# youmi-zym/TemporalStereo

Hardware: AMD Instinct MI355X
Metric: stereo pairs/sec, FlyingThings3D 540x960 D=192 (aggregation hot path) (higher is better)
Workload: dtype f32

## Files before the change

include/ts_hip.h:

```cpp
#ifndef TS_HIP_H
#define TS_HIP_H

#include <stddef.h>
#include <stdint.h>

#ifdef __cplusplus
extern "C" {
#endif

#define TS_OK 0
#define TS_ERR_NULL (-1)
#define TS_ERR_SHAPE (-2)
#define TS_ERR_UNSUPPORTED (-3)
#define TS_ERR_ALIGN (-4)

int ts_version(void);
const char* ts_last_error_string(void);

size_t ts_block_cost_workspace_bytes(int B, int C, int H, int W, int D, int scales);

int ts_block_cost_int_fwd(const float* left, const float* right, float* out, void* workspace,
                          int B, int C, int H, int W, int D, int scales, void* stream);

int ts_block_cost_sampled_fwd(const float* left, const float* right, const float* disp, float* out,
                              void* workspace, int B, int C, int H, int W, int D, int scales,
                              void* stream);

int ts_block_cost_sampled_warped_fwd(const float* left, const float* right, const float* disp, float* out,
                                     void* workspace, int B, int C, int H, int W, int D, int scales,
                                     void* stream);

int ts_block_cost_sampled_corr_fwd(const float* left, const float* right, const float* disp, float* out,
                                   void* workspace, int B, int C, int H, int W, int D, int scales,
                                   void* stream);

int ts_block_cost_corr_split_supported(int C, int Csplit);
int ts_block_cost_sampled_corr_split_fwd(const float* left, const float* left2, const float* right, const float* right2,
                                         const float* disp, float* out, void* workspace, int B, int C, int Csplit, int H, int W,
                                         int D, int scales, long long left_bstride, long long left2_bstride,
                                         long long right_bstride, long long right2_bstride, void* stream);
int ts_conv3d_hw_split_supported(int B, int Cin, int Csplit, int Cout, int D, int H, int W, int stride, int dilation,
                                 int transposed);
int ts_conv3d_hw_split_fwd(const float* x, const float* x2, const float* w_t, const float* scale, const float* shift, float* y,
                           int B, int Cin, int Csplit, int Cout, int D, int H, int W, int stride, int dilation,
                           int transposed, int act, float act_param,
                           long long in_bstride, long long in_cstride, long long in2_bstride, long long in2_cstride,
                           long long out_bstride, long long out_cstride, const float* addend, long long addend_bstride,
                           void* workspace, size_t workspace_bytes, void* stream);
int ts_conv3d_d_split_supported(int Cin, int Csplit);
int ts_conv3d_d_split_fwd(const float* x, const float* x2, const float* w_t, const float* scale, const float* shift, float* y,
                          int B, int Cin, int Csplit, int Cout, int Din, int H, int W, int k, int stride, int dilation,
                          int padding, int transposed, int act, float act_param,
                          long long in_bstride, long long in_cstride, long long in2_bstride, long long in2_cstride,
                          long long out_bstride, long long out_cstride, void* stream);
int ts_conv3d_hw_x6_split_supported(int Cin, int Csplit, int Cout, int W, int dilation);
int ts_conv3d_hw_x6_split_fwd(const float* x, const float* x2, const void* w6, const float* scale, const float* shift, float* y,
                              int B, int Cin, int Csplit, int Cout, int D, int H, int W, int dilation, int act, float act_param,
                              long long in_bstride, long long in_cstride, long long in2_bstride, long long in2_cstride,
                              long long out_bstride, long long out_cstride, const float* addend, long long addend_bstride,
                              void* workspace, size_t workspace_bytes, void* stream);

int ts_cat_fms_fwd(const float* left, const float* right, const float* disp, float* out, int B, int C, int H, int W, int D,
                   void* stream);
int ts_inverse_warp_3d_fwd(const float* img, const float* disp, float* out, int B, int C, int H, int W, int D, void* stream);
size_t ts_dif_fms_workspace_bytes(void);
int ts_dif_fms_fwd(const float* left, const float* right, const float* disp, float* out, void* workspace, int B, int C,
                   int H, int W, int D, void* stream);

int ts_correlation_fwd(const float* left, const float* right, float* out, int B, int C, int H, int W, int patch_h, int patch_w,
                       int keep, void* stream);
int ts_correlation_bwd(const float* left, const float* right, const float* out, const float* grad_out, float* grad_left,
                       float* grad_right, int B, int C, int H, int W, int patch_h, int patch_w, int keep, void* stream);

size_t ts_block_cost_bwd_workspace_bytes(int B, int C, int H, int W, int D, int scales);

int ts_block_cost_int_bwd(const float* left, const float* right, const float* grad_out,
                          float* grad_left, float* grad_right, void* workspace,
                          int B, int C, int H, int W, int D, int scales, void* stream);

int ts_block_cost_sampled_bwd(const float* left, const float* right, const float* disp,
                              const float* grad_out, float* grad_left, float* grad_right,
                              float* grad_disp, void* workspace,
                              int B, int C, int H, int W, int D, int scales, void* stream);
int ts_block_cost_sampled_warped_bwd(const float* left, const float* right, const float* disp,
                                     const float* grad_out, float* grad_left, float* grad_right,
                                     float* grad_disp, void* workspace,
                                     int B, int C, int H, int W, int D, int scales, void* stream);

size_t ts_bn_workspace_bytes(int B, int C, long long N);
int ts_bn_sync_merge(const float* gathered, int world, int C, float* mean, float* var, float* running_mean,
                     float* running_var, float momentum, float* inv_count, void* stream);
long long ts_bn_set_small_elems(long long n);
int ts_channel_sum_fwd(const float* x, float* out, void* workspace, int B, int C, long long N, long long bstride, long long cstride,
                       void* stream);
int ts_bn_train_fwd(const float* x, float* mean, float* var, float* running_mean, float* running_var, float momentum,
                    long long* num_batches_tracked, const float* gamma, const float* beta, float* out, void* workspace,
                    int B, int C, long long N, long long x_bstride, long long x_cstride, long long out_bstride,
                    long long out_cstride, float eps, int act, void* stream);
int ts_bn_train_bwd(const float* x, const float* dy, const float* mean, const float* var, const float* gamma, const float* beta,
                    float* sum_dz, float* sum_dz_xhat, float* dx, void* workspace, int B, int C, long long N,
                    long long x_bstride, long long x_cstride, long long dy_bstride, long long dy_cstride, float eps, int act,
                    float count, void* stream);
int ts_bn_stats_fwd(const float* x, float* mean, float* var, float* running_mean, float* running_var, float momentum,
                    long long* num_batches_tracked, void* workspace, int B, int C, long long N, long long bstride,
                    long long cstride, void* stream);
int ts_bn_apply_act_fwd(const float* x, const float* mean, const float* var, const float* gamma, const float* beta, float* out,
                        int B, int C, long long N, long long x_bstride, long long x_cstride, long long out_bstride,
                        long long out_cstride, float eps, int act, void* stream);
int ts_bn_act_bwd_reduce(const float* x, const float* dy, const float* mean, const float* var, const float* gamma,
                         const float* beta, float* sum_dz, float* sum_dz_xhat, void* workspace, int B, int C, long long N,
                         long long x_bstride, long long x_cstride, long long dy_bstride, long long dy_cstride, float eps, int act,
                         void* stream);
int ts_bn_act_bwd_apply(const float* x, const float* dy, const float* mean, const float* var, const float* gamma,
                        const float* beta, const float* sum_dz, const float* sum_dz_xhat, float* dx, int B, int C, long long N,
                        long long x_bstride, long long x_cstride, long long dy_bstride, long long dy_cstride, float eps, int act,
                        int train, float count, void* stream);

size_t ts_wasserstein_loss_workspace_bytes(int B, int H, int W);
int ts_wasserstein_loss_fwd(const float* cost, const float* offset, const float* sample, const float* gt, float* loss,
                            float* gt_scaled, void* workspace, int B, int D, int H, int W, int Hg, int Wg, float max_disp,
                            float start_disp, int sparse, void* stream);
int ts_wasserstein_loss_bwd(const float* cost, const float* offset, const float* sample, const float* gt_scaled,
                            const float* grad_loss, float* grad_cost, float* grad_offset, int B, int D, int H, int W, int Wg,
                            float max_disp, float start_disp, void* stream);
size_t ts_disp_smooth_l1_workspace_bytes(int B, int Hg, int Wg);
int ts_disp_smooth_l1_fwd(const float* est, const float* gt, float* loss_count, void* workspace, int B, int h, int w, int Hg,
                          int Wg, float max_disp, float start_disp, void* stream);
int ts_disp_smooth_l1_bwd(const float* est, const float* gt, const float* grad_loss, const float* loss_count, float* grad_est,
                          int B, int h, int w, int Hg, int Wg, float max_disp, float start_disp, void* stream);

size_t ts_disp_metrics_workspace_bytes(int B, int Hg, int Wg);
int ts_disp_metrics_fwd(const float* est0, const float* est1, const float* est2, const float* est3, int n_est, int h0, int w0,
                        int h1, int w1, int h2, int w2, int h3, int w3, const float* gt, const float* gt_right, int B, int Hg,
                        int Wg, float lb, float ub, int flags, float* out, void* workspace, void* stream);

#define TS_RENDER_EST_COLOR 1
#define TS_RENDER_GT_COLOR 2
#define TS_RENDER_ERR_CLASS 4
#define TS_RENDER_ERR_JET 8
#define TS_RENDER_U16 16
#define TS_RENDER_UINT8 32
#define TS_RENDER_CHW 64
#define TS_RENDER_BAR 128
#define TS_RENDER_CLIP 256
#define TS_RENDER_MAX_SHARED 512
#define TS_RENDER_MAX_GIVEN 1024
#define TS_RENDER_STATS_FLOATS 32
size_t ts_disp_render_workspace_bytes(int B, int Hg, int Wg);
int ts_disp_render_fwd(const float* est, const float* gt, const float* max_disp, const float* jet, int B, int h, int w, int Hg,
                       int Wg, int flags, float scale16, void* disp_color, void* err_class, void* err_jet, void* disp_u16,
                       float* stats, void* workspace, void* stream);

#define TS_FLOW_SPARSE 1
#define TS_FLOW_EST_HWC 2
#define TS_FLOW_GT_HWC 4
#define TS_FLOW_RENDER_EST_COLOR 1
#define TS_FLOW_RENDER_GT_COLOR 2
#define TS_FLOW_RENDER_ERR_CLASS 4
#define TS_FLOW_RENDER_STATS 8
#define TS_FLOW_RENDER_UINT8 16
#define TS_FLOW_RENDER_CHW 32
#define TS_FLOW_RENDER_MAX_SHARED 64
#define TS_FLOW_RENDER_MAX_GIVEN 128
#define TS_FLOW_RENDER_EST_HWC 256
#define TS_FLOW_RENDER_GT_HWC 512
#define TS_FLOW_STATS_FLOATS 16
#define TS_FLOW_U16_CHW 1
size_t ts_flow_metrics_workspace_bytes(int B, int Hg, int Wg);
int ts_flow_metrics_fwd(const float* est0, const float* est1, const float* est2, const float* est3, int n_est, int h0, int w0,
                        int h1, int w1, int h2, int w2, int h3, int w3, const float* gt, int B, int Hg, int Wg, float lb, float ub,
                        int flags, float* out, void* workspace, void* stream);
size_t ts_flow_render_workspace_bytes(int B, int Hg, int Wg);
int ts_flow_render_fwd(const float* est, const float* gt, const float* gt_val, const float* max_rad, const float* wheel, int B,
                       int h, int w, int Hg, int Wg, int flags, void* flow_color, void* err_class, float* stats, void* workspace,
                       void* stream);
int ts_flow_u16_decode_fwd(const void* raw, int B, int H, int W, int flags, float* flow, void* valid, void* stream);

#define TS_PREPARE_CHW 1
int ts_frames_prepare_fwd(const void* left, const void* right, int B, int Hs, int Ws, int flags, float mean0, float mean1,
                          float mean2, float std0, float std1, float std2, int H, int W, const int* crop, float* color_l,
                          float* color_r, long long color_stride, float* color_aug_l, float* color_aug_r,
                          long long color_aug_stride, void* stream);
int ts_intrinsics_pyramid_fwd(const void* K_norm, int is_fp64, int B, int kh, int kw, int S, float* K, float* inv_K, void* stream);
int ts_disp_u16_decode_fwd(const void* raw, int B, int H, int W, float scale, float* disp, void* valid, void* stream);

#define TS_AUGMENT_ROW_INTS 96
#define TS_AUGMENT_MAX_RECTS 4
#define TS_AUGMENT_GAMMA 1
size_t ts_frames_augment_workspace_bytes(int B, int Hs, int Ws);
int ts_frames_augment_fwd(const void* left, const void* right, int B, int Hs, int Ws, int flags, float mean0, float mean1,
                          float mean2, float std0, float std1, float std2, int H, int W, const int* table, float* color_l,
                          float* color_r, long long color_stride, float* color_aug_l, float* color_aug_r,
                          long long color_aug_stride, void* workspace, size_t workspace_bytes, void* stream);
int ts_disp_u16_window_fwd(const void* raw, int B, int Hs, int Ws, int H, int W, const int* table, float scale, float* disp,
                           void* valid, void* stream);

int ts_topk_softargmax_fwd(const float* cost, const float* sample, const float* offset, float* disp,
                           float* topk_disp, float* topk_cost, int* topk_index,
                           int B, int D, int H, int W, int k, void* stream);

int ts_topk_softargmax_bwd(const float* topk_disp, const float* topk_cost, const int* topk_index,
                           const float* disp, const float* grad_disp, const float* grad_topk_disp,
                           const float* grad_topk_cost, float* grad_cost, float* grad_sample,
                           int B, int D, int H, int W, int k, void* stream);

int ts_softargmin_fwd(const float* cost, const float* sample, float* disp, float temperature,
                      int normalize, int B, int D, int H, int W, void* stream);
// ... 255 lines not shown
```

temporalstereo_amd/_lib.py:

```python
import ctypes
import os
import threading

_HERE = os.path.dirname(os.path.abspath(__file__))
LIB_PATH = os.path.join(_HERE, "libts_hip.so")

_lock = threading.Lock()
_lib = None

c_f32p = ctypes.c_void_p
c_ptr = ctypes.c_void_p
c_int = ctypes.c_int
c_size = ctypes.c_size_t
c_float = ctypes.c_float

SIGNATURES = {
    "ts_version": (c_int, []),
    "ts_last_error_string": (ctypes.c_char_p, []),
    "ts_block_cost_workspace_bytes": (c_size, [c_int] * 6),
    "ts_block_cost_int_fwd": (c_int, [c_f32p, c_f32p, c_f32p, c_ptr] + [c_int] * 6 + [c_ptr]),
    "ts_block_cost_sampled_fwd": (c_int, [c_f32p, c_f32p, c_f32p, c_f32p, c_ptr] + [c_int] * 6 + [c_ptr]),
    "ts_block_cost_sampled_warped_fwd": (c_int, [c_f32p, c_f32p, c_f32p, c_f32p, c_ptr] + [c_int] * 6 + [c_ptr]),
    "ts_block_cost_sampled_corr_fwd": (c_int, [c_f32p, c_f32p, c_f32p, c_f32p, c_ptr] + [c_int] * 6 + [c_ptr]),
    "ts_block_cost_corr_split_supported": (c_int, [c_int] * 2),
    "ts_block_cost_sampled_corr_split_fwd": (c_int, [c_f32p] * 6 + [c_ptr] + [c_int] * 7 + [ctypes.c_longlong] * 4 + [c_ptr]),
    "ts_conv3d_hw_split_supported": (c_int, [c_int] * 10),
    "ts_conv3d_hw_split_fwd": (c_int, [c_f32p] * 6 + [c_int] * 11 + [c_float] + [ctypes.c_longlong] * 6 +
                               [c_f32p, ctypes.c_longlong, c_ptr, c_size, c_ptr]),
    "ts_conv3d_d_split_supported": (c_int, [c_int] * 2),
    "ts_conv3d_d_split_fwd": (c_int, [c_f32p] * 6 + [c_int] * 13 + [c_float] + [ctypes.c_longlong] * 6 + [c_ptr]),
    "ts_conv3d_hw_x6_split_supported": (c_int, [c_int] * 5),
    "ts_conv3d_hw_x6_split_fwd": (c_int, [c_f32p, c_f32p, c_ptr, c_f32p, c_f32p, c_f32p] + [c_int] * 9 + [c_float] + [ctypes.c_longlong] * 6 +
                                  [c_f32p, ctypes.c_longlong, c_ptr, c_size, c_ptr]),
    "ts_conv3d_hw_warp_workspace_bytes": (c_size, [c_int] * 5),
    "ts_conv3d_hw_warp_fwd": (c_int, [c_f32p] * 8 + [c_int] * 8 + [c_float] + [ctypes.c_longlong] * 5 + [c_ptr, c_size, c_ptr]),
    "ts_cat_fms_fwd": (c_int, [c_f32p] * 4 + [c_int] * 5 + [c_ptr]),
    "ts_inverse_warp_3d_fwd": (c_int, [c_f32p] * 3 + [c_int] * 5 + [c_ptr]),
    "ts_dif_fms_workspace_bytes": (c_size, []),
    "ts_dif_fms_fwd": (c_int, [c_f32p] * 4 + [c_ptr] + [c_int] * 5 + [c_ptr]),
    "ts_correlation_fwd": (c_int, [c_f32p] * 3 + [c_int] * 7 + [c_ptr]),
    "ts_correlation_bwd": (c_int, [c_f32p] * 6 + [c_int] * 7 + [c_ptr]),
    "ts_block_cost_bwd_workspace_bytes": (c_size, [c_int] * 6),
    "ts_block_cost_int_bwd": (c_int, [c_f32p] * 5 + [c_ptr] + [c_int] * 6 + [c_ptr]),
    "ts_block_cost_sampled_bwd": (c_int, [c_f32p] * 7 + [c_ptr] + [c_int] * 6 + [c_ptr]),
    "ts_block_cost_sampled_warped_bwd": (c_int, [c_f32p] * 7 + [c_ptr] + [c_int] * 6 + [c_ptr]),
    "ts_calib_stream": (c_int, [c_int, c_ptr, c_ptr, c_size, c_ptr]),
    "ts_candidates_in_range_fwd": (c_int, [c_f32p] * 3 + [c_int] * 5 + [c_ptr]),
    "ts_candidates_in_range_bwd": (c_int, [c_f32p] * 5 + [c_int] * 5 + [c_ptr]),
    "ts_offset_head_fwd": (c_int, [c_f32p] * 2 + [ctypes.c_longlong, c_float, c_ptr]),
    "ts_offset_head_bwd": (c_int, [c_f32p] * 3 + [ctypes.c_longlong, c_float, c_ptr]),
    "ts_space_to_depth2_fwd": (c_int, [c_f32p] * 2 + [c_int] * 4 + [c_ptr]),
    "ts_deconv2d_k4s2_weight_to_conv3": (c_int, [c_f32p] * 2 + [c_int] * 3 + [c_ptr]),
    "ts_deconv2d_k4s2_wgrad_from_conv3": (c_int, [c_f32p] * 2 + [c_int] * 2 + [c_ptr]),
    "ts_bn_fold_many": (c_int, [c_ptr, c_int, c_float, c_ptr]),
    "ts_clip_rmsprop_workspace_bytes": (c_size, [c_int]),
    "ts_clip_rmsprop_step": (c_int, [c_ptr, c_int] + [c_float] * 4 + [c_ptr, c_size, c_ptr]),
    "ts_topk_softargmax_fwd": (c_int, [c_f32p] * 7 + [c_int] * 5 + [c_ptr]),
    "ts_topk_softargmax_bwd": (c_int, [c_f32p] * 9 + [c_int] * 5 + [c_ptr]),
    "ts_softargmin_fwd": (c_int, [c_f32p] * 3 + [c_float, c_int] + [c_int] * 4 + [c_ptr]),
    "ts_softargmin_bwd": (c_int, [c_f32p] * 6 + [c_float, c_int] + [c_int] * 4 + [c_ptr]),
    "ts_argmax_select_fwd": (c_int, [c_f32p] * 4 + [c_int] * 4 + [c_ptr]),
    "ts_bn_workspace_bytes": (c_size, [c_int, c_int, ctypes.c_longlong]),
    "ts_channel_splice_fwd": (c_int, [c_f32p] * 3 + [c_int] * 3 + [ctypes.c_longlong] * 4 + [c_ptr]),
    "ts_bn_sync_merge": (c_int, [c_f32p, c_int, c_int] + [c_f32p] * 4 + [c_float, c_f32p, c_ptr]),
    "ts_bn_train_fwd": (c_int, [c_f32p] * 5 + [c_float, c_ptr] + [c_f32p] * 3 + [c_ptr, c_int, c_int] + [ctypes.c_longlong] * 5 +
                        [c_float, c_int, c_ptr]),
    "ts_bn_train_bwd": (c_int, [c_f32p] * 9 + [c_ptr, c_int, c_int] + [ctypes.c_longlong] * 5 + [c_float, c_int, c_float, c_ptr]),
    "ts_bn_stats_fwd": (c_int, [c_f32p] * 5 + [c_float, c_ptr, c_ptr, c_int, c_int] + [ctypes.c_longlong] * 3 + [c_ptr]),
    "ts_bn_apply_act_fwd": (c_int, [c_f32p] * 6 + [c_int, c_int] + [ctypes.c_longlong] * 5 + [c_float, c_int, c_ptr]),
    "ts_bn_act_bwd_reduce": (c_int, [c_f32p] * 8 + [c_ptr, c_int, c_int] + [ctypes.c_longlong] * 5 + [c_float, c_int, c_ptr]),
    "ts_bn_act_bwd_apply": (c_int, [c_f32p] * 9 + [c_int, c_int] + [ctypes.c_longlong] * 5 + [c_float, c_int, c_int, c_float, c_ptr]),
    "ts_wasserstein_loss_workspace_bytes": (c_size, [c_int] * 3),
    "ts_wasserstein_loss_fwd": (c_int, [c_f32p] * 6 + [c_ptr] + [c_int] * 6 + [c_float, c_float, c_int, c_ptr]),
    "ts_wasserstein_loss_bwd": (c_int, [c_f32p] * 7 + [c_int] * 5 + [c_float, c_float, c_ptr]),
    "ts_disp_smooth_l1_workspace_bytes": (c_size, [c_int] * 3),
    "ts_disp_smooth_l1_fwd": (c_int, [c_f32p] * 3 + [c_ptr] + [c_int] * 5 + [c_float, c_float, c_ptr]),
    "ts_disp_smooth_l1_bwd": (c_int, [c_f32p] * 5 + [c_int] * 5 + [c_float, c_float, c_ptr]),
    "ts_disp_metrics_workspace_bytes": (c_size, [c_int] * 3),
    "ts_disp_metrics_fwd": (c_int, [c_f32p] * 4 + [c_int] * 9 + [c_f32p] * 2 + [c_int] * 3 + [c_float, c_float, c_int, c_f32p, c_ptr, c_ptr]),
    "ts_disp_render_workspace_bytes": (c_size, [c_int] * 3),
    "ts_disp_render_fwd": (c_int, [c_f32p] * 4 + [c_int] * 6 + [c_float] + [c_ptr] * 4 + [c_f32p, c_ptr, c_ptr]),
    "ts_flow_metrics_workspace_bytes": (c_size, [c_int] * 3),
    "ts_flow_metrics_fwd": (c_int, [c_f32p] * 4 + [c_int] * 9 + [c_f32p] + [c_int] * 3 + [c_float, c_float, c_int, c_f32p, c_ptr, c_ptr]),
    "ts_flow_render_workspace_bytes": (c_size, [c_int] * 3),
    "ts_flow_render_fwd": (c_int, [c_f32p] * 5 + [c_int] * 6 + [c_ptr] * 2 + [c_f32p, c_ptr, c_ptr]),
    "ts_flow_u16_decode_fwd": (c_int, [c_ptr] + [c_int] * 4 + [c_f32p, c_ptr, c_ptr]),
    "ts_frames_prepare_fwd": (c_int, [c_ptr] * 2 + [c_int] * 4 + [c_float] * 6 + [c_int] * 2 + [c_ptr] + [c_f32p] * 2 +
                              [ctypes.c_longlong] + [c_f32p] * 2 + [ctypes.c_longlong, c_ptr]),
    "ts_intrinsics_pyramid_fwd": (c_int, [c_ptr] + [c_int] * 5 + [c_f32p] * 2 + [c_ptr]),
    "ts_disp_u16_decode_fwd": (c_int, [c_ptr] + [c_int] * 3 + [c_float, c_f32p, c_ptr, c_ptr]),
    "ts_frames_augment_workspace_bytes": (c_size, [c_int] * 3),
    "ts_frames_augment_fwd": (c_int, [c_ptr] * 2 + [c_int] * 4 + [c_float] * 6 + [c_int] * 2 + [c_ptr] + [c_f32p] * 2 +
                              [ctypes.c_longlong] + [c_f32p] * 2 + [ctypes.c_longlong, c_ptr, c_size, c_ptr]),
    "ts_disp_u16_window_fwd": (c_int, [c_ptr] + [c_int] * 5 + [c_ptr, c_float, c_f32p, c_ptr, c_ptr]),
    "ts_softsplat_sum_fwd": (c_int, [c_f32p] * 3 + [c_int] * 4 + [c_ptr]),
    "ts_softsplat_sum_fwd_deterministic": (c_int, [c_f32p] * 3 + [c_ptr] + [c_int] * 4 + [c_ptr]),
    "ts_softsplat_sum_bwd_input": (c_int, [c_f32p] * 3 + [c_int] * 4 + [c_ptr]),
    "ts_softsplat_sum_bwd_flow": (c_int, [c_f32p] * 4 + [c_int] * 4 + [c_ptr]),
    "ts_softsplat_softmax_workspace_bytes": (c_size, [c_int] * 4),
    "ts_softsplat_softmax_fwd": (c_int, [c_f32p] * 4 + [c_ptr] + [c_int] * 4 + [c_ptr]),
    "ts_conv_cout_pad": (c_int, [c_int]),
    "ts_peer_region_bytes": (c_size, []),
    "ts_peer_max_floats": (c_int, []),
    "ts_peer_max_ranks": (c_int, []),
    "ts_peer_alloc": (c_int, [ctypes.POINTER(c_ptr), c_ptr]),
    "ts_peer_open": (c_int, [c_ptr, ctypes.POINTER(c_ptr)]),
    "ts_peer_close": (c_int, [c_ptr]),
    "ts_peer_free": (c_int, [c_ptr]),
    "ts_peer_status": (c_int, [c_ptr, ctypes.POINTER(c_int), c_ptr]),
    "ts_bn_set_small_elems": (ctypes.c_longlong, [ctypes.c_longlong]),
    "ts_channel_sum_fwd": (c_int, [c_f32p, c_f32p, c_ptr, c_int, c_int, ctypes.c_longlong, ctypes.c_longlong, ctypes.c_longlong, c_ptr]),
    "ts_peer_status_async": (c_int, [c_ptr, c_ptr, c_ptr]),
    "ts_peer_set_timeout_ms": (ctypes.c_longlong, [ctypes.c_longlong]),
    "ts_peer_reset": (c_int, [c_ptr, c_ptr]),
    "ts_peer_all_gather": (c_int, [c_ptr, c_f32p, c_f32p, c_int, c_ptr]),
    "ts_peer_all_reduce_sum": (c_int, [c_ptr, c_f32p, c_int, c_f32p, c_ptr]),
    "ts_conv_weight_layout": (c_int, [c_f32p, c_f32p] + [c_int] * 4 + [ctypes.c_longlong] * 3 + [c_int, c_ptr]),
    "ts_conv_weight_layout_many": (c_int, [c_ptr, c_int, c_int, c_ptr]),
    "ts_conv_weight_layout_many2": (c_int, [c_ptr, c_int, c_int, c_ptr]),
    "ts_conv_wgrad_defer": (c_int, [c_int]),
    "ts_conv_wgrad_pending": (c_int, []),
    "ts_conv_wgrad_take": (c_int, [c_ptr, c_size, ctypes.POINTER(c_int), ctypes.POINTER(c_int)]),
    "ts_conv_wgrad_finish_many": (c_int, [c_ptr, c_int, c_int, c_ptr]),
    "ts_conv_set_chunk_cap": (c_int, [c_int]),
    "ts_conv3d_hw_x6_supported": (c_int, [c_int] * 6),
    "ts_conv3d_hw_x6_weight_bytes": (ctypes.c_size_t, [c_int] * 2),
    "ts_conv3d_hw_x6_weight_split": (c_int, [c_f32p, c_ptr, c_int, c_int, c_ptr]),
    "ts_conv3d_hw_x6_weight_split_from": (c_int, [c_f32p, c_ptr, c_int, c_int] + [ctypes.c_longlong] * 3 + [c_int, c_ptr]),
    "ts_conv3d_hw_x6_workspace_bytes": (c_size, [c_int] * 6),
    "ts_conv3d_hw_x6s_supported": (c_int, [c_int] * 5),
    "ts_conv3d_hw_x6s_weight_bytes": (c_size, [c_int] * 3),
    "ts_conv3d_hw_x6s_weight_split": (c_int, [c_f32p, c_ptr, c_int, c_int, c_int, c_int, c_ptr]),
    "ts_conv3d_hw_x6s_fwd": (c_int, [c_f32p, c_ptr, c_f32p, c_f32p, c_f32p] + [c_int] * 8 + [c_float] + [ctypes.c_longlong] * 4 + [c_ptr]),
    "ts_conv3d_hw_x6_fwd": (c_int, [c_f32p, c_ptr, c_f32p, c_f32p, c_f32p] + [c_int] * 8 + [c_float] + [ctypes.c_longlong] * 4 +
                            [c_f32p, ctypes.c_longlong, c_ptr, c_size, c_ptr]),
    "ts_conv3d_hw_fwd": (c_int, [c_f32p] * 5 + [c_int] * 10 + [c_float] + [ctypes.c_longlong] * 4 +
                         [c_f32p, ctypes.c_longlong, c_ptr, c_size, c_ptr]),
    "ts_conv3d_hw_workspace_bytes": (c_size, [c_int] * 8),
    "ts_conv3d_hw_bwd_data": (c_int, [c_f32p] * 3 + [c_int] * 9 + [ctypes.c_longlong] * 4 + [c_ptr]),
    "ts_conv3d_bwd_weight_workspace_bytes": (ctypes.c_size_t, [c_int] * 3),
    "ts_conv3d_hw_bwd_weight": (c_int, [c_f32p] * 3 + [c_int] * 8 + [ctypes.c_longlong] * 4 + [c_ptr, ctypes.c_size_t, c_ptr]),
    "ts_conv3d_d_bwd_data": (c_int, [c_f32p] * 3 + [c_int] * 11 + [ctypes.c_longlong] * 4 + [c_ptr]),
    "ts_conv3d_d_bwd_weight": (c_int, [c_f32p] * 3 + [c_int] * 10 + [ctypes.c_longlong] * 4 + [c_ptr, ctypes.c_size_t, c_ptr]),
    "ts_conv3d_d_fwd": (c_int, [c_f32p] * 5 + [c_int] * 12 + [c_float] + [ctypes.c_longlong] * 4 + [c_ptr]),
    "ts_resize3d_add_act_fwd": (c_int, [c_f32p] * 3 + [c_int] * 9 + [ctypes.c_longlong] * 6 + [c_ptr]),
    "ts_pool3d5_avgmax_fwd": (c_int, [c_f32p] * 3 + [c_int] * 5 + [ctypes.c_longlong] * 6 + [c_ptr]),
    "ts_merge_candidates_fwd": (c_int, [c_f32p] * 9 + [c_int] * 6 + [ctypes.c_longlong] * 4 + [c_ptr]),
    "ts_convex_upsample_fwd": (c_int, [c_f32p] * 3 + [c_int] * 4 + [c_float, c_ptr]),
    "ts_convex_upsample_candidates_fwd": (c_int, [c_f32p] * 6 + [c_int] * 4 + [c_float, c_float, c_int, c_int, c_ptr]),
    "ts_unet_upsample_fwd": (c_int, [c_f32p] * 3 + [c_int] * 5 + [c_ptr]),
    "ts_convex_upsample_bwd": (c_int, [c_f32p] * 5 + [c_int] * 4 + [c_float, c_ptr]),
    "ts_unet_upsample_bwd": (c_int, [c_f32p] * 5 + [c_ptr] + [c_int] * 5 + [c_ptr]),
    "ts_deconv2d_k4s2_fwd": (c_int, [c_f32p] * 5 + [c_int] * 6 + [ctypes.c_longlong, c_ptr]),
    "ts_resize_bilinear_fwd": (c_int, [c_f32p] * 2 + [c_int] * 6 + [c_float, ctypes.c_longlong, c_ptr]),
    "ts_resize_bilinear_pair_fwd": (c_int, [c_f32p] * 4 + [c_int] * 6 + [c_float, c_float, c_ptr]),
    "ts_range_candidates_fwd": (c_int, [c_f32p] * 4 + [c_int] * 3 + [c_float, c_int, c_int, c_ptr]),
    "ts_project_to_3d_fwd": (c_int, [c_f32p] * 7 + [c_int] * 6 + [c_float, c_ptr]),
    "ts_inverse_warp_fwd": (c_int, [c_f32p] * 9 + [c_ptr, c_f32p] + [c_int] * 11 + [c_float, c_ptr]),
    "ts_inverse_warp_bwd": (c_int, [c_f32p] * 8 + [c_int] * 11 + [c_float, c_ptr]),
    "ts_raft_corr_pyramid_fwd": (c_int, [c_f32p] * 3 + [c_int] * 5 + [c_ptr]),
    "ts_raft_corr_lookup_fwd": (c_int, [c_f32p] * 3 + [c_int] * 5 + [c_ptr]),
    "ts_raft_corr_lookup_bwd": (c_int, [c_f32p] * 5 + [c_int] * 6 + [c_ptr]),
    "ts_raft_corr_pyramid_bwd": (c_int, [c_f32p] * 5 + [c_int] * 5 + [c_ptr]),
    "ts_flow_corr_pyramid_fwd": (c_int, [c_f32p] * 3 + [c_int] * 5 + [c_ptr]),
    "ts_flow_corr_lookup_fwd": (c_int, [c_f32p] * 3 + [c_int] * 5 + [c_ptr]),
    "ts_flow_corr_lookup_bwd": (c_int, [c_f32p] * 5 + [c_int] * 6 + [c_ptr]),
    "ts_flow_corr_pyramid_bwd": (c_int, [c_f32p] * 5 + [c_int] * 5 + [c_ptr]),
    "ts_spp3d_pool_fwd": (c_int, [c_f32p] * 2 + [c_int] * 10 + [ctypes.c_longlong] * 2 + [c_ptr]),
    "ts_spp3d_pool_bwd": (c_int, [c_f32p] * 6 +[c_int] * 10 + [ctypes.c_longlong] * 4 + [c_ptr]),
    "ts_spp3d_expand_fwd": (c_int, [c_f32p] * 6 + [c_int] * 11 + [ctypes.c_longlong] * 2 + [c_ptr]),
    "ts_spp3d_expand_bwd": (c_int, [c_f32p] * 5 + [c_int] * 11 + [ctypes.c_longlong] * 2 + [c_ptr]),
    "ts_depth_sum3_fwd": (c_int, [c_f32p] * 6 + [c_int] * 6 + [ctypes.c_longlong] * 8 + [c_ptr]),
    "ts_bn_small_train_bwd": (c_int, [c_f32p] * 7 + [c_int] * 3 + [ctypes.c_longlong] * 6 + [c_float, c_int, c_ptr]),
    "ts_reproject_memory_workspace_bytes": (c_size, [c_int] * 5),
    "ts_reproject_memory_fwd": (c_int, [c_f32p, ctypes.c_longlong, c_int, c_int, c_f32p, c_f32p, c_int, c_f32p, c_int, c_int,
                                        c_f32p, c_int, c_f32p, c_f32p, c_f32p, c_float, c_float, c_f32p, c_f32p, c_f32p,
                                        c_ptr, c_int, c_int, c_int, c_ptr]),
    "ts_resize3d_add_act_bwd": (c_int, [c_f32p] * 5 + [c_int] * 9 + [c_ptr]),
    "ts_pool3d5_avgmax_bwd": (c_int, [c_f32p] * 4 + [c_int] * 5 + [c_ptr]),
    "ts_merge_candidates_bwd": (c_int, [c_f32p] * 5 + [c_int] * 5 + [c_ptr]),
    "ts_copy_rows_fwd": (c_int, [c_f32p] * 2 + [ctypes.c_longlong] * 4 + [c_ptr]),
    "ts_plan_create": (c_ptr, []),
    "ts_plan_destroy": (None, [c_ptr]),
    "ts_plan_length": (c_int, [c_ptr]),
    "ts_plan_add_call": (c_int, [c_ptr, ctypes.c_char_p, ctypes.POINTER(ctypes.c_ulonglong), c_int]),
    "ts_plan_run": (c_int, [c_ptr]),
    "ts_stream_fork": (c_int, [c_ptr, c_ptr]),
    "ts_event_record": (c_int, [c_int, c_ptr]),
    "ts_event_wait": (c_int, [c_int, c_ptr]),
}

_QUERIES = frozenset(n for n in SIGNATURES if n.endswith("_bytes") or n.startswith("ts_plan_") or
                     n.endswith("_split_supported") or
                     n in ("ts_version", "ts_last_error_string", "ts_conv_cout_pad", "ts_conv3d_hw_x6_supported", "ts_conv3d_hw_x6s_supported", "ts_peer_max_floats", "ts_peer_max_ranks",
                           "ts_peer_alloc", "ts_peer_open", "ts_peer_close", "ts_peer_free", "ts_peer_status", "ts_peer_status_async",
                           "ts_peer_set_timeout_ms", "ts_peer_reset", "ts_bn_set_small_elems",
                           "ts_conv_wgrad_defer", "ts_conv_wgrad_pending", "ts_conv_wgrad_take"))


def lib():
    rec = getattr(_tls, "recorder", None)
    if rec is not None:
        return rec.proxy
    return _real_lib()


def _real_lib():
    global _lib
    if _lib is None:
        with _lock:
            if _lib is None:
                if not os.path.exists(LIB_PATH):
                    raise RuntimeError(
                        "temporalstereo_amd: %s is missing -- build it with "
                        "`python -m temporalstereo_amd.build` (there is no fallback path)" % LIB_PATH)
                handle = ctypes.CDLL(LIB_PATH)
                for name, (res, args) in SIGNATURES.items():
                    fn = getattr(handle, name, None)
                    if fn is None:
                        raise RuntimeError("libts_hip.so does not export %s (stale build?)" % name)
                    fn.restype = res
                    fn.argtypes = args
                _lib = handle
    return _lib


_tls = threading.local()


def _word(argtype, value):
    if isinstance(value, ctypes._SimpleCData):
        value = value.value
    if argtype is c_float:
        import struct
        return struct.unpack("<I", struct.pack("<f", float(value)))[0]
    if value is None:
        return 0
    return int(value) & 0xFFFFFFFFFFFFFFFF


class _RecordingProxy:
    def __init__(self, recorder):
        self._rec = recorder

    def __getattr__(self, name):
        real = getattr(_real_lib(), name)
        if name in _QUERIES:
            return real
        argtypes = SIGNATURES[name][1]
        rec = self._rec

        def call(*args):
            rc = real(*args)
            if rc == 0:
                words = (ctypes.c_ulonglong * len(args))(*[_word(t, a) for t, a in zip(argtypes, args)])
                rec.log.append((name, int(words[len(args) - 1]) if len(args) else 0))
                rc2 = _real_lib().ts_plan_add_call(rec.plan, name.encode(), words, len(args))
                if rc2 != 0:
                    check(rc2, "ts_plan_add_call(%s)" % name)
            return rc
        return call


class Recorder:

    def __init__(self):
        self.plan = _real_lib().ts_plan_create()
        if not self.plan:
            raise RuntimeError("ts_plan_create failed")
        self.keep = []
        self.log = []
        self.proxy = _RecordingProxy(self)

    def __enter__(self):
        if getattr(_tls, "recorder", None) is not None:
            raise RuntimeError("plan recording does not nest")
        _tls.recorder = self
        return self

    def __exit__(self, *exc):
        _tls.recorder = None
        return False

    def __len__(self):
        return int(_real_lib().ts_plan_length(self.plan))

    def run(self):
        rc = _real_lib().ts_plan_run(self.plan)
        if rc != 0:
            check(rc, "ts_plan_run")

    def __del__(self):
        try:
            if self.plan:
                _real_lib().ts_plan_destroy(self.plan)
                self.plan = None
        except Exception:
            pass


def recording():
    return getattr(_tls, "recorder", None) is not None


def check(rc, what):
    if rc != 0:
        msg = _real_lib().ts_last_error_string().decode("utf-8", "replace")
        kind = "argument error" if rc < 0 else "hipError_t"
        raise RuntimeError("%s failed (%s %d): %s" % (what, kind, rc, msg))


def ptr(t):
    if t is None:
        return None
    rec = getattr(_tls, "recorder", None)
    if rec is not None:
        rec.keep.append(t)
    return t.data_ptr()


def current_stream_handle():
    import torch
    return torch._C._cuda_getCurrentRawStream(torch.cuda.current_device())


def contiguous(t):
    if t.is_contiguous():
        return t
    if recording():
        raise RuntimeError("plan recording needs contiguous tensors (a .contiguous() copy would not be replayed)")
    return t.contiguous()
```

temporalstereo_amd/aggregation/native.py:

```python
import os
import time

import torch
import torch.nn as nn

from .. import _lib
from .. import functional as TF

ACT_NONE, ACT_SILU, ACT_RELU, ACT_TANH_OFFSET, ACT_HEAD_PAIR = 0, 1, 2, 3, 4


def _stream():
    return _lib.current_stream_handle()


_PAR = {"on": False, "aux": None, "kinds": frozenset(__import__("os").environ.get("TS_BRANCHES", "hourglass").split(","))}


def _aux_stream():
    return _PAR["aux"]


_STAGE_CAP = int(os.environ.get("TS_STAGE_CHUNK_CAP", "8"))


def _chunk_cap(cap):
    if cap == 8:
        cap = _STAGE_CAP
    _lib.check(_lib.lib().ts_conv_set_chunk_cap(int(cap)), "ts_conv_set_chunk_cap")


_QUALIFIED = {}
_ROUND_TRIP_SLACK = 1.6


def _round_trip_us(main, s, n=20):
    L = _lib._real_lib()
    buf = torch.zeros(2, 256, device=s.device)
    pm, ps = _lib.ctypes.c_void_p(main.cuda_stream), _lib.ctypes.c_void_p(s.cuda_stream)
    a, b = _lib.ctypes.c_void_p(buf[0].data_ptr()), _lib.ctypes.c_void_p(buf[1].data_ptr())

    def lap(k):
        for _ in range(k):
            for st, other in ((pm, ps), (ps, pm)):
                _lib.check(L.ts_copy_rows_fwd(a, b, 1, 256, 256, 256, st), "ts_copy_rows_fwd")
                _lib.check(L.ts_stream_fork(st, other), "ts_stream_fork")
    lap(5)
    best = None
    for _ in range(3):
        torch.cuda.synchronize(s.device)
        t0 = time.perf_counter()
        lap(n)
        torch.cuda.synchronize(s.device)
        us = (time.perf_counter() - t0) / n * 1e6
        best = us if best is None else min(best, us)
    return best


def qualified_streams(dev, count, private=False):
    with torch.cuda.device(dev):
        pool = _QUALIFIED.setdefault(torch.cuda.current_device(), {"shared": [], "floor": None})
        main = torch.cuda.current_stream()
        if pool["floor"] is None:
            pool["floor"] = _round_trip_us(main, torch.cuda.Stream(device=dev))

        def draw():
            best = None
            for _ in range(8):
                s = torch.cuda.Stream(device=dev, priority=-1)
                us = _round_trip_us(main, s)
                if us <= _ROUND_TRIP_SLACK * pool["floor"]:
                    return s
                if best is None or us < best[0]:
                    best = (us, s)
            return best[1]
        if private:
            return [draw() for _ in range(count)]
        while len(pool["shared"]) < count:
            pool["shared"].append(draw())
        return pool["shared"][:count]


def _edge(src, dst):
    rc = _lib.lib().ts_stream_fork(_lib.ctypes.c_void_p(src.cuda_stream), _lib.ctypes.c_void_p(dst.cuda_stream))
    _lib.check(rc, "ts_stream_fork")


class Branch:

    def __init__(self, kind):
        self.on = _PAR["on"] and kind in _PAR["kinds"]
        if self.on:
            self.cur, self.aux = torch.cuda.current_stream(), _aux_stream()

    def __enter__(self):
        if self.on:
            _edge(self.cur, self.aux)
            self.ctx = torch.cuda.stream(self.aux)
            self.ctx.__enter__()
        return self

    def __exit__(self, *exc):
        if self.on:
            self.ctx.__exit__(*exc)
        return False

    def join(self):
        if self.on:
            _edge(self.aux, self.cur)


def _act_code(mod):
    if mod is None:
        return ACT_NONE
    if isinstance(mod, nn.SiLU):
        return ACT_SILU
    if isinstance(mod, nn.ReLU):
        return ACT_RELU
    raise NotImplementedError("activation %r has no fused kernel epilogue" % (mod,))


class Tape:

    def __init__(self):
        self.layouts = []
        self.folds = []
        self.splits = []
        self.eps = None
        self.unsupported = []
        self._tables = None

    def __enter__(self):
        global _TAPE
        self._outer, _TAPE = _TAPE, self
        return self

    def __exit__(self, *exc):
        global _TAPE
        _TAPE = self._outer
        return False

    def layout(self, out, weight, transposed, rows=None, col0=0, out_st=None, src_cin0=0, cout_sel=None):
        w = weight
        d0, d1 = w.shape[0], w.shape[1]
        T = w[0, 0].numel()
        cout, cin = (d1, d0) if transposed else (d0, d1)
        s_ci, s_co = ((d1 * T, T) if transposed else (T, d1 * T))
        c0, nci = rows if rows is not None else (0, cin)
        o0, nco = cout_sel if cout_sel is not None else (0, cout)
        self.layouts.append(dict(out=out, w=w, A=nci, T=T, nb=nco, col0=col0, sa=s_ci, sb=s_co, st=1, src_off=(c0 + src_cin0) * s_ci + o0 * s_co,
                                 out_sa=out.stride(0), out_st=out.stride(1) if out_st is None else out_st))
        self._tables = None

    def fold(self, scale, shift, bias, bn, cout):
        if bn is not None:
            if self.eps is not None and float(bn.eps) != self.eps:
                self.unsupported.append("BatchNorm layers with different eps")
            self.eps = float(bn.eps)
        self.folds.append(dict(scale=scale, shift=shift, bias=bias, bn=bn, C=cout))
        self._tables = None

    def _upload(self, dev):
        import numpy as np
        lay = np.zeros(len(self.layouts), dtype=np.dtype([("w", "<u8"), ("out", "<u8"), ("A", "<i4"), ("T", "<i4"), ("nb", "<i4"), ("col0", "<i4"),
                                                          ("sa", "<i8"), ("sb", "<i8"), ("st", "<i8"), ("osa", "<i8"), ("ost", "<i8"),
                                                          ("flip", "<i4"), ("reserved", "<i4")]))
        most = 1
        for i, e in enumerate(self.layouts):
            w = e["w"]
            if not w.is_contiguous():
                raise RuntimeError("Tape: a source weight is not contiguous")
            lay[i] = (w.data_ptr() + 4 * e["src_off"], e["out"].data_ptr(), e["A"], e["T"], e["nb"], e["col0"], e["sa"], e["sb"], e["st"],
                      e["out_sa"], e["out_st"], 0, 0)
            most = max(most, e["A"] * e["T"] * e["nb"])
        fo = np.zeros(len(self.folds), dtype=np.dtype([("gamma", "<u8"), ("beta", "<u8"), ("mean", "<u8"), ("var", "<u8"), ("bias", "<u8"),
                                                       ("scale", "<u8"), ("shift", "<u8"), ("C", "<i4"), ("pad", "<i4")]))
        P = lambda t: t.data_ptr() if t is not None else 0
        for i, e in enumerate(self.folds):
            bn = e["bn"]
            if bn is not None:
                g, b = (bn.weight, bn.bias) if bn.affine else (None, None)
                fo[i] = (P(g), P(b), P(bn.running_mean), P(bn.running_var), P(e["bias"]), P(e["scale"]), P(e["shift"]), e["C"], e["C"])
            else:
                fo[i] = (0, 0, 0, 0, P(e["bias"]), P(e["scale"]), P(e["shift"]), e["C"], e["C"])
        up = lambda a: torch.from_numpy(a.view(np.uint8).reshape(-1).copy()).to(dev)
        self._tables = (up(lay), up(fo), min(64, (most + 255) // 256))

    def refresh(self, dev):
        if self.unsupported:
            raise RuntimeError("Tape.refresh: %s -- rebuild the aggregator instead" % "; ".join(self.unsupported))
        L = _lib.lib()
        if self._tables is None:
            self._upload(dev)
        lay, fo, blocks = self._tables
        if self.layouts:
            _lib.check(L.ts_conv_weight_layout_many2(_lib.ptr(lay), len(self.layouts), blocks, _stream()), "ts_conv_weight_layout_many2")
        if self.folds:
            _lib.check(L.ts_bn_fold_many(_lib.ptr(fo), len(self.folds), self.eps if self.eps is not None else 1e-5, _stream()), "ts_bn_fold_many")
        for f, kind, mode in self.splits:
            if kind == "x6":
                _lib.check(L.ts_conv3d_hw_x6_weight_split(f.w.data_ptr(), f.w6.data_ptr(), f.cin, f.cout, _stream()), "ts_conv3d_hw_x6_weight_split")
            else:
                _lib.check(L.ts_conv3d_hw_x6s_weight_split(f.w.data_ptr(), f.w6s.data_ptr(), f.cin, f.cout, f.w.shape[2], mode, _stream()),
                           "ts_conv3d_hw_x6s_weight_split")


_TAPE = None


class Folded:

    def __init__(self, weight, bias, bn, act, transposed, kind):
        self._tape = _TAPE
        self.src = (weight, bias, bn, transposed)
        w = weight.detach().float()
        if transposed:
            w = w.transpose(0, 1)
        cout, cin = w.shape[0], w.shape[1]
        taps = w.shape[2:].numel()
        self.cin, self.cout, self.kind, self.act = cin, cout, kind, act
        self.kshape = tuple(w.shape[2:])
        pad = int(_lib.lib().ts_conv_cout_pad(cout))
        if pad < cout:
            raise NotImplementedError("Cout=%d has no kernel bucket" % cout)
        wt = torch.zeros(cin, taps, pad, device=w.device, dtype=torch.float32)
        wt[:, :, :cout] = w.reshape(cout, cin, taps).permute(1, 2, 0)
        self.w = wt.contiguous()
        scale = torch.ones(pad, device=w.device)
        shift = torch.zeros(pad, device=w.device)
        b = bias.detach().float() if bias is not None else torch.zeros(cout, device=w.device)
        if bn is not None:
            if not isinstance(bn, nn.modules.batchnorm._BatchNorm) or bn.running_mean is None:
                raise NotImplementedError("only BatchNorm with running statistics can be folded, got %r" % (bn,))
            gamma = bn.weight.detach().float() if bn.affine else torch.ones(cout, device=w.device)
            beta = bn.bias.detach().float() if bn.affine else torch.zeros(cout, device=w.device)
            s = gamma / torch.sqrt(bn.running_var.detach().float() + bn.eps)
            scale[:cout] = s
            shift[:cout] = beta + (b - bn.running_mean.detach().float()) * s
        else:
            shift[:cout] = b
        self.scale, self.shift = scale.contiguous(), shift.contiguous()
        if _TAPE is not None:
            if weight.dtype != torch.float32:
                _TAPE.unsupported.append("non-fp32 weights")
            _TAPE.layout(self.w, weight.detach(), transposed)
            _TAPE.fold(self.scale, self.shift, bias, bn, cout)


def fold_split_input(f, n):
    head, rest = object.__new__(Folded), object.__new__(Folded)
    for g, lo, hi in ((head, 0, n), (rest, n, f.cin)):
        g.cin, g.cout, g.kind, g.kshape = hi - lo, f.cout, f.kind, f.kshape
        g._tape = getattr(f, "_tape", None)
        g.w = f.w[lo:hi].contiguous()
        assert g.w.data_ptr() == f.w[lo:hi].data_ptr()
    head.act, rest.act = ACT_NONE, f.act
    head.scale, head.shift = torch.ones_like(f.scale), torch.zeros_like(f.shift)
    rest.scale, rest.shift = f.scale, f.shift
    return head, rest


def fold_concat(a, b):
    if (a.cin, a.kind, a.act, a.kshape) != (b.cin, b.kind, b.act, b.kshape):
        raise ValueError("fold_concat: layers differ in more than their output channels")
    f = object.__new__(Folded)
    f.cin, f.cout, f.kind, f.act, f.kshape = a.cin, a.cout + b.cout, a.kind, a.act, a.kshape
    pad = int(_lib.lib().ts_conv_cout_pad(f.cout))
    if pad < f.cout:
        raise NotImplementedError("Cout=%d has no kernel bucket" % f.cout)
    taps = a.w.shape[1]
    f.w = torch.zeros(a.cin, taps, pad, device=a.w.device, dtype=torch.float32)
    f.w[:, :, :a.cout] = a.w[:, :, :a.cout]
    f.w[:, :, a.cout:f.cout] = b.w[:, :, :b.cout]
    f.scale = torch.ones(pad, device=a.w.device)
    f.shift = torch.zeros(pad, device=a.w.device)
    f.scale[:a.cout] = a.scale[:a.cout]; f.scale[a.cout:f.cout] = b.scale[:b.cout]
    f.shift[:a.cout] = a.shift[:a.cout]; f.shift[a.cout:f.cout] = b.shift[:b.cout]
    f._tape = getattr(a, "_tape", None)
    if f._tape is not None:
        col = 0
        for g in (a, b):
            src = getattr(g, "src", None)
            if src is None:
                f._tape.unsupported.append("concatenation of derived layers")
                break
            weight, bias, bn, transposed = src
            f._tape.layout(f.w, weight.detach(), transposed, col0=col)
            f._tape.fold(f.scale[col:col + g.cout], f.shift[col:col + g.cout], bias, bn, g.cout)
            col += g.cout
    return f


def fold_wrapper(m, kind, transposed=False):
    return Folded(m.weight, m.bias, getattr(m, "norm", None), _act_code(getattr(m, "activation", None)), transposed, kind)


def _strides5(t):
    if t.stride(4) != 1 or t.stride(3) != t.shape[4] or t.stride(2) != t.shape[3] * t.shape[4]:
        raise ValueError("tensor planes must be dense (channel-sliced views of contiguous buffers are fine)")
    return t.stride(0), t.stride(1)


Split = TF.Split


X6 = os.environ.get("TS_CONV_X6", "1") != "0"
_X6_MIN_GRID = int(os.environ.get("TS_CONV_X6_MIN_GRID", "128"))
_X6_MIN_GRID_UNSPLIT = int(os.environ.get("TS_CONV_X6_MIN_GRID_UNSPLIT", "64"))


def x6_weights(f):
    w6 = getattr(f, "w6", None)
    if w6 is None:
        L = _lib._real_lib()
        w6 = torch.empty(int(L.ts_conv3d_hw_x6_weight_bytes(f.cin, f.cout)), device=f.w.device, dtype=torch.uint8)
        _lib.check(L.ts_conv3d_hw_x6_weight_split(f.w.data_ptr(), w6.data_ptr(), f.cin, f.cout, _stream()), "ts_conv3d_hw_x6_weight_split")
        f.w6 = w6
        if getattr(f, "_tape", None) is not None:
            f._tape.splits.append((f, "x6", 0))
    return w6


X6S = os.environ.get("TS_CONV_X6S", "1") != "0"
_X6S_MIN_GRID = int(os.environ.get("TS_CONV_X6S_MIN_GRID", "256"))
_X6S_MIN_GRID_T3 = int(os.environ.get("TS_CONV_X6S_MIN_GRID_T3", "400"))
X6S_S2, X6S_T3, X6S_T4 = 0, 1, 2


def x6s_weights(f, mode):
    w6 = getattr(f, "w6s", None)
    if w6 is None:
        L = _lib._real_lib()
        w6 = torch.empty(int(L.ts_conv3d_hw_x6s_weight_bytes(f.cin, f.cout, mode)), device=f.w.device, dtype=torch.uint8)
        _lib.check(L.ts_conv3d_hw_x6s_weight_split(f.w.data_ptr(), w6.data_ptr(), f.cin, f.cout, f.w.shape[2], mode, _stream()),
                   "ts_conv3d_hw_x6s_weight_split")
        f.w6s = w6
        f.w6s_mode = mode
        if getattr(f, "_tape", None) is not None:
            f._tape.splits.append((f, "x6s", mode))
    elif getattr(f, "w6s_mode", mode) != mode:
        raise RuntimeError("x6s_weights: this layer's weights were split for mode %d, asked for mode %d" % (f.w6s_mode, mode))
    return w6


def x6s_grid(B, cout, D, H, W, mode):
    if mode == X6S_S2:
        return ((((H - 1) // 2 + 1) + 3) // 4) * ((((W - 1) // 2 + 1) + 31) // 32) * D * B * ((cout + 31) // 32)
    return ((H + 7) // 8) * ((W + 31) // 32) * D * B * ((cout + 15) // 16)


def conv_hw(x, f, stride=1, dilation=1, transposed=False, out=None, act=None, act_param=0.0, addend=None, second=None,
            out_second=None):
    split = None
    if isinstance(x, Split):
        if second is not None or transposed or stride != 1:
            raise ValueError("conv_hw(Split): stride-1, not transposed, no `second`")
        x, split = x.a, x.b
# ... 71 lines not shown
    return out


def conv_d(x, f, k, stride=1, dilation=1, padding=0, transposed=False, out=None, act=None, act_param=0.0):
    split = None
    if isinstance(x, Split):
        x, split = x.a, x.b
    B, Cin, Din, H, W = x.shape
    if split is not None:
        Cs, Cin = Cin, Cin + split.shape[1]
        i2b, i2c = _strides5(split)
    assert Cin == f.cin, (Cin, f.cin)
    Dout = 2 * Din if transposed else (Din + 2 * padding - dilation * (k - 1) - 1) // stride + 1
    if out is None:
        out = torch.empty((B, f.cout, Dout, H, W), device=x.device, dtype=torch.float32)
    ib, ic = _strides5(x)
    ob, oc = _strides5(out)
    if split is not None:
        rc = _lib.lib().ts_conv3d_d_split_fwd(_lib.ptr(x), _lib.ptr(split), _lib.ptr(f.w), _lib.ptr(f.scale), _lib.ptr(f.shift),
                                              _lib.ptr(out), B, Cin, Cs, f.cout, Din, H, W, k, stride, dilation, padding,
                                              int(transposed), f.act if act is None else act, float(act_param),
                                              ib, ic, i2b, i2c, ob, oc, _stream())
        _lib.check(rc, "ts_conv3d_d_split_fwd")
        return out
    rc = _lib.lib().ts_conv3d_d_fwd(_lib.ptr(x), _lib.ptr(f.w), _lib.ptr(f.scale), _lib.ptr(f.shift), _lib.ptr(out),
                                    B, Cin, f.cout, Din, H, W, k, stride, dilation, padding, int(transposed),
                                    f.act if act is None else act, float(act_param), ib, ic, ob, oc, _stream())
    _lib.check(rc, "ts_conv3d_d_fwd")
    return out


FUSED_K1 = os.environ.get("TS_FUSED_K1", "1") != "0"
SPLIT_INPUT = os.environ.get("TS_SPLIT_INPUT", "1") != "0"


def block_cost_corr(left, right, disp, scales):
    return TF.block_cost_corr(left, right, disp, scales)


def conv_hw_warp(corr, f, q, disp, base, dilation=1):
    B, Cc, D, H, W = corr.shape
    assert Cc == f.cin, (Cc, f.cin)
    out = torch.empty((B, f.cout, D, H, W), device=corr.device, dtype=torch.float32)
    ib, ic = _strides5(corr)
    ob, oc = _strides5(out)
    wsb = TF._q("ts_conv3d_hw_warp_workspace_bytes", B, f.cout, D, H, W)
    ws = torch.empty(wsb, device=corr.device, dtype=torch.uint8)
    rc = _lib.lib().ts_conv3d_hw_warp_fwd(_lib.ptr(corr), _lib.ptr(f.w), _lib.ptr(f.scale), _lib.ptr(f.shift), _lib.ptr(out),
                                          _lib.ptr(q), _lib.ptr(disp), _lib.ptr(base), B, Cc, f.cout, D, H, W, dilation, f.act, 0.0,
                                          ib, ic, ob, oc, base.stride(0) if base is not None else 0, _lib.ptr(ws), wsb, _stream())
    _lib.check(rc, "ts_conv3d_hw_warp_fwd")
    return out


def resize_add_act(a, add, size, act=ACT_SILU):
    B, C, Da, Ha, Wa = a.shape
    D, H, W = size
    out = torch.empty((B, C, D, H, W), device=a.device, dtype=torch.float32)
    ab, ac = _strides5(a)
    bb, bc = _strides5(add) if add is not None else (0, 0)
    ob, oc = _strides5(out)
    rc = _lib.lib().ts_resize3d_add_act_fwd(_lib.ptr(a), _lib.ptr(add), _lib.ptr(out), B, C, Da, Ha, Wa, D, H, W, act,
                                            ab, ac, bb, bc, ob, oc, _stream())
    _lib.check(rc, "ts_resize3d_add_act_fwd")
    return out


def pool5(x, out_avg, out_max):
    B, C, D, H, W = x.shape
    xb, xc = _strides5(x); ab, ac = _strides5(out_avg); mb, mc = _strides5(out_max)
    rc = _lib.lib().ts_pool3d5_avgmax_fwd(_lib.ptr(x), _lib.ptr(out_avg), _lib.ptr(out_max), B, C, D, H, W,
                                          xb, xc, ab, ac, mb, mc, _stream())
    _lib.check(rc, "ts_pool3d5_avgmax_fwd")


def resize_bilinear(x, size, value_scale=1.0, out=None):
    B, C, h, w = x.shape
    if out is None:
        out = torch.empty((B, C, size[0], size[1]), device=x.device, dtype=torch.float32)
    x = _lib.contiguous(x)
    rc = _lib.lib().ts_resize_bilinear_fwd(_lib.ptr(x), _lib.ptr(out), B, C, h, w, size[0], size[1],
                                           float(value_scale), out.stride(0), _stream())
    _lib.check(rc, "ts_resize_bilinear_fwd")
    return out


def resize_bilinear_pair(x0, x1, size, scale0, scale1):
    B, C, h, w = x0.shape
    if x1.shape != x0.shape:
        raise RuntimeError("resize_bilinear_pair: shapes differ")
    o0 = torch.empty((B, C, size[0], size[1]), device=x0.device, dtype=torch.float32)
    o1 = torch.empty_like(o0)
    x0, x1 = _lib.contiguous(x0), _lib.contiguous(x1)
    rc = _lib.lib().ts_resize_bilinear_pair_fwd(_lib.ptr(x0), _lib.ptr(x1), _lib.ptr(o0), _lib.ptr(o1),
                                                B, C, h, w, size[0], size[1], float(scale0), float(scale1), _stream())
    _lib.check(rc, "ts_resize_bilinear_pair_fwd")
    return o0, o1


def copy_rows(src, dst):
    B = src.shape[0]
    n = src[0].numel()
    src = _lib.contiguous(src)
    rc = _lib.lib().ts_copy_rows_fwd(_lib.ptr(src), _lib.ptr(dst), B, n, n, dst.stride(0), _stream())
    _lib.check(rc, "ts_copy_rows_fwd")


def range_candidates(disp, rng, extra_front=0):
    B, _, H, W = disp.shape
    low = torch.empty_like(disp)
    high = torch.empty_like(disp)
    cand = torch.empty((B, extra_front + 5, H, W), device=disp.device, dtype=torch.float32)
    rc = _lib.lib().ts_range_candidates_fwd(_lib.ptr(disp), _lib.ptr(low), _lib.ptr(high), _lib.ptr(cand), B, H, W,
                                            float(rng), extra_front, extra_front + 5, _stream())
    _lib.check(rc, "ts_range_candidates_fwd")
    return low, high, cand


def split_sampled_first_layer(f0, scales):
    C = f0.cin * 8 // (16 + scales)
    if 2 * C + scales * (C // 8) != f0.cin or f0.kshape != (1, 3, 3):
        raise NotImplementedError("first aggregation layer is not a (1,3,3) conv over [left | warped | corr]")
    left, rest = fold_split_input(f0, C)
    _, corr = fold_split_input(rest, C)
    q = object.__new__(Folded)
    q.cin, q.cout, q.kind, q.act, q.kshape = C, 9 * rest.cout, "d", ACT_NONE, (1, 1, 1)
    pad = int(_lib.lib().ts_conv_cout_pad(q.cout))
    q.w = torch.zeros(C, 1, pad, device=rest.w.device, dtype=torch.float32)
    q.w[:, 0, :q.cout] = rest.w[:C, :, :rest.cout].reshape(C, 9 * rest.cout)
    q.scale, q.shift = torch.ones(pad, device=q.w.device), torch.zeros(pad, device=q.w.device)
    q._tape = getattr(f0, "_tape", None)
    if q._tape is not None:
        src = getattr(f0, "src", None)
        if src is None or src[3]:
            q._tape.unsupported.append("first layer of a sampled level is itself derived")
        else:
            q._tape.layout(q.w, src[0].detach(), False, rows=(C, C), out_st=rest.cout)
    return left, rest, corr, q


class SepConv:

    def __init__(self, mod, transposed=False):
        c0, c1 = mod.conv[0], mod.conv[1]
        self.transposed = transposed
        self.f0 = fold_wrapper(c0, "hw", transposed)
        self.f1 = fold_wrapper(c1, "d", transposed)
        self.k = c1.kernel_size[0]
        self.stride, self.dil = c0.stride[1], c0.dilation[1]
        self.pad_d = c1.padding[0]
        if c0.kernel_size != (1, 3, 3) or c0.padding[1] != self.dil or c1.stride[0] != self.stride:
            raise NotImplementedError("separable conv outside the (1,3,3)+(k,1,1) family: %r" % (mod,))

    def __call__(self, x, out=None, addend=None):
        y = conv_hw(x, self.f0, self.stride, self.dil, self.transposed, addend=addend)
        return conv_d(y, self.f1, self.k, self.stride, self.dil, self.pad_d, self.transposed, out=out)


class Hourglass:

    def __init__(self, mod):
        self.c1, self.c2, self.c3, self.c4 = (SepConv(getattr(mod, n)) for n in ("conv1", "conv2", "conv3", "conv4"))
        self.c5, self.c6 = SepConv(mod.conv5, True), SepConv(mod.conv6, True)
        self.s5, self.s6 = SepConv(mod.shortcut5), SepConv(mod.shortcut6)
        self.c4.f1.act = ACT_SILU

    def __call__(self, x):
        pre = self.c2(self.c1(x))
        br = Branch("hourglass")
        with br:
            s6 = self.s6(x)
            s5 = self.s5(pre)
        out = self.c5(self.c4(self.c3(pre)))
        br.join()
        out = resize_add_act(out, s5, pre.shape[-3:])
        return resize_add_act(self.c6(out), s6, x.shape[-3:])


class Heads:

    def __init__(self, mod):
        self.delta = float(mod.delta)
        c0, self.c1 = fold_wrapper(mod.cost_head[0], "d"), fold_wrapper(mod.cost_head[1], "hw")
        o0, self.o1 = fold_wrapper(mod.off_head[0], "d"), fold_wrapper(mod.off_head[1], "hw")
        self.C = C = c0.cout
        self.co0 = fold_concat(c0, o0)
        f = object.__new__(Folded)
        f.cin, f.cout, f.kind, f.act, f.kshape = 2 * C, 2, "hw", ACT_HEAD_PAIR, self.c1.kshape
        pad = int(_lib.lib().ts_conv_cout_pad(2))
        f.w = torch.zeros(2 * C, self.c1.w.shape[1], pad, device=self.c1.w.device, dtype=torch.float32)
        f.w[:C, :, 0] = self.c1.w[:, :, 0]
        f.w[C:, :, 1] = self.o1.w[:, :, 0]
        f.scale = torch.ones(pad, device=f.w.device); f.shift = torch.zeros(pad, device=f.w.device)
        f.scale[0], f.scale[1] = self.c1.scale[0], self.o1.scale[0]
        f.shift[0], f.shift[1] = self.c1.shift[0], self.o1.shift[0]
        f._tape = _TAPE
        if _TAPE is not None:
            for k, (m, g) in enumerate(((mod.cost_head[1], self.c1), (mod.off_head[1], self.o1))):
                _TAPE.layout(f.w[k * C:(k + 1) * C], m.weight.detach(), False, col0=k)
                _TAPE.fold(f.scale[k:k + 1], f.shift[k:k + 1], m.bias, getattr(m, "norm", None), 1)
        self.pair = f

    def __call__(self, x):
        y = conv_d(x, self.co0, 3, 1, 1, 1)
        B, _, D, H, W = y.shape
        both = torch.empty((2, B, D, H, W), device=y.device, dtype=torch.float32)
        conv_hw(y, self.pair, out=both.permute(1, 0, 2, 3, 4), act_param=self.delta)
        return both[0], both[1]


class ConvexUp:

    def __init__(self, mod):
        self.r, self.k = mod.upscale_factor, mod.window_size
        if self.k != 3:
            raise NotImplementedError("window_size != 3")
        self.m0 = Folded(mod.mask[0].weight.unsqueeze(2), mod.mask[0].bias, mod.mask[1], ACT_SILU, False, "hw")
        w3 = mod.mask[3].weight
        self.m3 = Folded(w3.reshape(w3.shape[0], w3.shape[1], 1, 1, 1), mod.mask[3].bias, None, ACT_NONE, False, "d")

    def mask(self, feat):
        return conv_d(conv_hw(feat.unsqueeze(2), self.m0), self.m3, 1)

    def with_candidates(self, feat, disp, m, rng, extra_front=0):
        B, _, H, W = disp.shape
        if m is None:
            m = self.mask(feat)
        Ho, Wo = H * self.r, W * self.r
        out = torch.empty((B, 1, Ho, Wo), device=disp.device, dtype=torch.float32)
        low, high = torch.empty_like(out), torch.empty_like(out)
        cand = torch.empty((B, extra_front + 5, Ho, Wo), device=disp.device, dtype=torch.float32)
        disp = _lib.contiguous(disp)
        rc = _lib.lib().ts_convex_upsample_candidates_fwd(_lib.ptr(m), _lib.ptr(disp), _lib.ptr(out), _lib.ptr(low),
                                                          _lib.ptr(high), _lib.ptr(cand), B, H, W, self.r, float(self.r), float(rng),
                                                          extra_front, extra_front + 5, _stream())
        _lib.check(rc, "ts_convex_upsample_candidates_fwd")
        return out, low, high, cand

    def __call__(self, feat, disp, m=None):
        B, _, H, W = disp.shape
        if m is None:
            m = self.mask(feat)
        out = torch.empty((B, 1, H * self.r, W * self.r), device=disp.device, dtype=torch.float32)
        disp = _lib.contiguous(disp)
        rc = _lib.lib().ts_convex_upsample_fwd(_lib.ptr(m), _lib.ptr(disp), _lib.ptr(out), B, H, W, self.r,
                                               float(self.r), _stream())
        _lib.check(rc, "ts_convex_upsample_fwd")
        return out


class _LevelBase:
    def __init__(self, mod):
        self.mod = mod
        self.C, self.topk, self.scales = mod.C, mod.topk, mod.block_cost_scale
        self.init0, self.hg, self.init2 = SepConv(mod.init3d[0]), Hourglass(mod.init3d[1]), SepConv(mod.init3d[2])
        self.heads = Heads(mod.pred_heads)

    def init3d(self, raw, addend=None):
        return self.init2(self.hg(self.init0(raw, addend=addend)))

    def split_reference_half(self):
        if self.init0.stride != 1 or self.init0.transposed:
            raise NotImplementedError("first aggregation layer is not a stride-1 conv over [left | warped | corr]")
        self.init0_left, self.init0.f0, self.init0_corr, self.init0_q = split_sampled_first_layer(self.init0.f0, self.scales)

    def left_term(self, left):
        return conv_hw(left.unsqueeze(2), self.init0_left, 1, self.init0.dil)

    def right_term(self, right):
        return conv_d(right.unsqueeze(2), self.init0_q, 1).squeeze(2)

    def first_layer_fused(self, left, right, ds, lterm, rterm):
        corr = block_cost_corr(left, right, ds, self.scales)
        i0 = self.init0
        y = conv_hw_warp(corr, self.init0_corr, rterm, ds, lterm.squeeze(2) if lterm.dim() == 5 else lterm, i0.dil)
        return conv_d(y, i0.f1, i0.k, i0.stride, i0.dil, i0.pad_d, i0.transposed)

    def init3d_from(self, first):
        return self.init2(self.hg(first))

    def feature_terms(self, left, right):
        return self.left_term(left), (self.right_term(right) if FUSED_K1 else None)


class _MergingLevel(_LevelBase):
    def __init__(self, mod):
        super().__init__(mod)
        pc = mod.past_conv
        f = fold_wrapper(pc, "d")
        self.past_w = f.w.reshape(-1)[:self.C].contiguous()
        self.past_scale, self.past_shift = f.scale[:self.C].contiguous(), f.shift[:self.C].contiguous()
        self.fusion = mod.spatial_fusion
        if self.fusion:
            self.conv5 = fold_wrapper(mod.fuse.conv_5x5, "d")
            self.fuse_conv = SepConv(mod.fuse.conv_fuse)
        self.up = ConvexUp(mod.convex_upsample)

    def merge(self, vol, samples, prev_info, resize_memory):
        B, C, D0, H, W = vol.shape
        K = self.topk
        memory = prev_info.get('cost_memory', None)
        mem_s = mem_c = None
        if memory is not None and prev_info.get('use_past_cost', False):
            mem_s, mem_c = memory['disp_sample'], memory['cost_volume']
            if resize_memory:
                mem_s, mem_c = resize_bilinear_pair(mem_s, mem_c, (H, W), W / mem_s.shape[-1], 1.0)
            mem_s, mem_c = _lib.contiguous(mem_s), _lib.contiguous(mem_c)
        Dm = D0 + K
        nch = 4 * C if self.fusion else C
        cat4 = torch.empty((B, nch, Dm, H, W), device=vol.device, dtype=torch.float32)
        samp = torch.empty((B, Dm, H, W), device=vol.device, dtype=torch.float32)
        x0 = cat4[:, :C]
        vb, vc = _strides5(vol); ob, oc = _strides5(x0)
        rc = _lib.lib().ts_merge_candidates_fwd(_lib.ptr(vol), _lib.ptr(samples), _lib.ptr(mem_s), _lib.ptr(mem_c),
                                                _lib.ptr(self.past_w), _lib.ptr(self.past_scale), _lib.ptr(self.past_shift),
                                                _lib.ptr(samp), _lib.ptr(x0), B, C, D0, K, H, W, vb, vc, ob, oc, _stream())
        _lib.check(rc, "ts_merge_candidates_fwd")
        return cat4, samp

    def fuse(self, cat4):
        C = self.C
        x0 = cat4[:, :C]
        if not self.fusion:
            return x0
        br = Branch("pool")
        with br:
            pool5(x0, cat4[:, 2 * C:3 * C], cat4[:, 3 * C:])
        conv_d(x0, self.conv5, 5, 1, 1, 2, out=cat4[:, C:2 * C])
        br.join()
# ... 393 lines not shown
```

temporalstereo_amd/csrc/conv3d.hip:

```cpp
#include <cstdlib>
#include <mutex>
#include <type_traits>
#include <vector>

#include "conv_common.hpp"
#include "conv_x6p.hpp"
#include "warp.hpp"

namespace {




template <int MODE, int KT, int ST, int DL, int TP = 256>
struct Geom {
  static constexpr int NTR = (MODE == MODE_D) ? KT : 1;
  static constexpr int TRW = (TP == 64) ? 4 : 8, TCW = (TP == 64) ? 16 : 32;
  static constexpr int in_rows = (MODE == MODE_HW) ? (TRW - 1) * ST + 2 * DL + 1 : ((MODE == MODE_HWT) ? ((KT == 16) ? TRW + 2 : TRW + 1) : 1);
  static constexpr int in_cols = (MODE == MODE_HW) ? (TCW - 1) * ST + 2 * DL + 1 : ((MODE == MODE_HWT) ? ((KT == 16) ? TCW + 2 : TCW + 1) : TP);
  static constexpr int pitch = (MODE == MODE_D) ? TP : (in_cols | 1);
  static constexpr int RQ_HW = (in_rows * in_cols + 255) / 256;
  static constexpr int chan_raw = (MODE == MODE_D) ? NTR * TP : in_rows * pitch;
  static constexpr int pad0 = (16 - (chan_raw & 31)) & 31;
  static constexpr int chan_elems = chan_raw + (pad0 ? pad0 : 32);
};


template <int CB, int MODE, int KT, int ST, int DL, int NC, int PR = 0, int PF = 0, int TP = 256>
__global__ void __launch_bounds__(256)
ig_conv_kernel(const float* __restrict__ x, const float* __restrict__ w, const float* __restrict__ scale,
               const float* __restrict__ shift, float* __restrict__ y, const IG p) {
  extern __shared__ __attribute__((aligned(16))) float lds[];
  static_assert(!PR || (MODE == MODE_HW && KT == 9 && ST == 1 && CB == 1 && NC >= 8), "row pairing: stride-1 (1,3,3), Cout <= 8");
  static_assert(TP == 256 || (TP == 64 && (MODE == MODE_D || MODE == MODE_HWT || (MODE == MODE_HW && !PR))), "64-pixel tiles: not the row-paired form");
  using G = Geom<MODE, KT, ST, DL, TP>;
  constexpr int WP = (CB * 16) | 16;
  constexpr int NTR = G::NTR, RQ = (MODE == MODE_D) ? NTR : G::RQ_HW;
  constexpr int in_rows = G::in_rows, in_cols = G::in_cols, pitch = G::pitch, chan_elems = G::chan_elems;
  constexpr int KTW = PR ? 12 : KT;
  constexpr int NPB = PR ? 2 : TP / 64;
  constexpr int WV = KTW * NC * CB * 4;
  constexpr int RWN = (WV + 255) / 256;

  const int wave = threadIdx.x >> 6, lane = threadIdx.x & 63;
  const int j = lane & 15, kq = lane >> 4;
  unsigned lin = blockIdx.x + gridDim.x * (blockIdx.y + gridDim.y * blockIdx.z);
  if (p.xcd) {
    const unsigned per = (gridDim.x * gridDim.y * gridDim.z) / 8;
    if (lin < per * 8) lin = (lin % 8) * per + lin / 8;
  }
  const int bx = lin % gridDim.x, by = (lin / gridDim.x) % gridDim.y, bz = lin / (gridDim.x * gridDim.y);
  const int cog = bz % p.co_groups;
  const int ks = (bz / p.co_groups) % p.ksplit, b = bz / (p.co_groups * p.ksplit);
  const int kbeg = ks * p.kspan, kend = min(p.Cin, kbeg + p.kspan);
  const int co0 = cog * CB * 16;
  const int od = by;

  int tile = bx, pa = 0, pbit = 0;
  if (MODE == MODE_HWT) { pa = (tile & 3) >> 1; pbit = tile & 1; tile >>= 2; }
  int iy0 = 0, ix0 = 0, ty0 = 0, tx0 = 0;
  if (MODE == MODE_HW) {
    ty0 = (tile / p.tiles_x) * G::TRW; tx0 = (tile % p.tiles_x) * G::TCW;
    iy0 = ty0 * ST - DL; ix0 = tx0 * ST - DL;
  } else if (MODE == MODE_HWT) {
    ty0 = (tile / p.tiles_x) * G::TRW; tx0 = (tile % p.tiles_x) * G::TCW;
    iy0 = ty0 - ((KT == 16) ? 1 : 0); ix0 = tx0 - ((KT == 16) ? 1 : 0);
  }
  float* in_tile = lds;
  float* w_tile = lds + NC * chan_elems;
  const unsigned HW = static_cast<unsigned>(p.H) * p.W;

  int plane_id[NTR], plane_wt[NTR], ntaps = KT;
  if (MODE == MODE_D) {
    if (p.transposed) {
      ntaps = 0;
      if ((od & 1) == 0) { plane_id[0] = od >> 1; plane_wt[0] = 1; ntaps = 1; }
      else {
        plane_id[0] = (od - 1) >> 1; plane_wt[0] = 2; ntaps = 1;
        if (NTR > 1 && ((od + 1) >> 1) < p.D) { plane_id[1] = (od + 1) >> 1; plane_wt[1] = 0; ntaps = 2; }
      }
#pragma unroll
      for (int t = 0; t < NTR; ++t) if (t >= ntaps) { plane_id[t] = -1; plane_wt[t] = 0; }
    } else {
#pragma unroll
      for (int t = 0; t < NTR; ++t) {
        const int id = od * p.stride + t * p.dil - p.pad;
        plane_id[t] = (id >= 0 && id < p.D) ? id : -1;
        plane_wt[t] = t;
      }
    }
  }
  const int px0 = (MODE == MODE_D) ? bx * TP : 0;

  unsigned goff[RQ];
  int loff[RQ];
  if (MODE == MODE_D) {
#pragma unroll
    for (int t = 0; t < NTR; ++t) {
      const unsigned px = px0 + 4u * (threadIdx.x & 63u);
      goff[t] = (plane_id[t] >= 0 && px < HW) ? (static_cast<unsigned>(plane_id[t]) * HW + px) * 4u : kOOB;
      loff[t] = t * 256 + 4 * static_cast<int>(threadIdx.x & 63u);
    }
  } else {
#pragma unroll
    for (int q = 0; q < RQ; ++q) {
      const int e = static_cast<int>(threadIdx.x) + 256 * q;
      const bool slot = e < in_rows * in_cols;
      const int cy = e / in_cols, cx = e - cy * in_cols;
      const int gy = iy0 + cy, gx = ix0 + cx;
      const bool live = slot && gy >= 0 && gy < p.H && gx >= 0 && gx < p.W;
      goff[q] = live ? (static_cast<unsigned>(od) * HW + static_cast<unsigned>(gy) * p.W + gx) * 4u : kOOB;
      loff[q] = slot ? cy * pitch + cx : G::chan_raw;
    }
  }
  constexpr int NI64 = (MODE == MODE_D && TP == 64) ? (NC * NTR + 15) / 16 : 1;
  unsigned go64[NI64];
  int lo64[NI64], ch64[NI64];
  if constexpr (MODE == MODE_D && TP == 64) {
#pragma unroll
    for (int i = 0; i < NI64; ++i) {
      const int r = static_cast<int>(threadIdx.x >> 4) + 16 * i;
      const bool ok = r < NC * NTR;
      const int c = r / NTR, t = r - c * NTR;
      int pid = -1;
#pragma unroll
      for (int u = 0; u < NTR; ++u) pid = (u == t) ? plane_id[u] : pid;
      const unsigned px = px0 + 4u * (threadIdx.x & 15u);
      go64[i] = (ok && pid >= 0 && px < HW) ? (static_cast<unsigned>(pid) * HW + px) * 4u : kOOB;
      ch64[i] = ok ? c : 0;
      lo64[i] = ok ? c * chan_elems + t * TP + 4 * static_cast<int>(threadIdx.x & 15u) : G::chan_raw;
    }
  }
  unsigned woff[RWN];
  int wci[RWN], wl[RWN];
#pragma unroll
  for (int q = 0; q < RWN; ++q) {
    const int v = threadIdx.x + 256 * q;
    const int co4 = v % (CB * 4), r = v / (CB * 4);
    const int ci = r % NC, tap = r / NC;
    if constexpr (PR) {
      const int rho = tap / 3, kx = tap % 3, ky = rho - ((co4 >> 1) ? 0 : 1);
      const bool ok = v < WV && ky >= 0 && ky <= 2;
      woff[q] = ok ? static_cast<unsigned>((ci * KT + ky * 3 + kx) * p.coutp + (co4 & 1) * 4) * 4u : kOOB;
    } else {
      const bool ok = v < WV && co0 + co4 * 4 < p.coutp;
      woff[q] = ok ? static_cast<unsigned>((ci * KT + tap) * p.coutp + co0 + co4 * 4) * 4u : kOOB;
    }
    wci[q] = ci;
    wl[q] = v < WV ? r * WP + co4 * 4 : KTW * NC * WP;
  }
  const __amdgpu_buffer_rsrc_t xr = ig_rsrc(x + static_cast<long long>(b) * p.in_bstride, p.in_bytes);
  const __amdgpu_buffer_rsrc_t xr2 = ig_rsrc(p.x2 + static_cast<long long>(b) * p.in2_bstride, p.in2_bytes);
  const __amdgpu_buffer_rsrc_t wr = ig_rsrc(w, p.w_bytes);
  const unsigned cstride_b = static_cast<unsigned>(p.in_cstride) * 4u, cstride2_b = static_cast<unsigned>(p.in2_cstride) * 4u;
  const unsigned wstride_b = static_cast<unsigned>(KT * p.coutp) * 4u;

  int boff[4];
#pragma unroll
  for (int pb = 0; pb < 4; ++pb) {
    if (MODE == MODE_D) boff[pb] = kq * chan_elems + wave * (TP / 4) + pb * 16 + j;
    else if (PR) {
      const int base = (DL == 1) ? wave * 2 : (wave & 1) + 4 * (wave >> 1);
      boff[pb] = kq * chan_elems + base * pitch + (pb & 1) * 16 + j;
    } else {
      const int row = (TP == 64) ? wave : wave * 2 + (pb >> 1), col = (TP == 64) ? j : (pb & 1) * 16 + j;
      constexpr int st = (MODE == MODE_HW) ? ST : 1;
      boff[pb] = kq * chan_elems + row * st * pitch + col * st;
    }
  }
  const int aoff = kq * WP + j;

  v4f acc[CB][4];
#pragma unroll
  for (int cb = 0; cb < CB; ++cb)
#pragma unroll
    for (int pb = 0; pb < 4; ++pb) acc[cb][pb] = v4f{0.f, 0.f, 0.f, 0.f};
  float esc[CB][4], esh[CB][4];
#pragma unroll
  for (int cb = 0; cb < CB; ++cb)
#pragma unroll
    for (int r = 0; r < 4; ++r) {
      const int co = min(PR ? (kq & 1) * 4 + r : co0 + cb * 16 + kq * 4 + r, p.coutp - 1);
      esc[cb][r] = scale ? scale[co] : 1.f;
      esh[cb][r] = shift ? shift[co] : 0.f;
    }

  constexpr int NSET = PF ? 2 : 1;
  constexpr bool VD = (MODE == MODE_D);
  constexpr int NCQ = VD ? NC / 4 : 1;
  float rin[NSET][VD ? 1 : NC][VD ? 1 : RQ];
  constexpr bool VD64 = VD && TP == 64;
  u32x4 rin4[NSET][VD64 ? 1 : NCQ][(VD && !VD64) ? NTR : 1];
  u32x4 rin64[NSET][NI64];
  u32x4 rw[NSET][RWN];
  const int wave_u = __builtin_amdgcn_readfirstlane(static_cast<int>(threadIdx.x >> 6));
  auto fetch = [&](auto set, int c0) {
    constexpr int S = decltype(set)::value;
    const ChunkBase cbs = chunk_base(c0, p.csplit, xr, xr2, cstride_b, cstride2_b);
    if constexpr (VD64) {
#pragma unroll
      for (int i = 0; i < NI64; ++i) {
        const unsigned chb = static_cast<unsigned>(min(c0 + ch64[i], p.Cin - 1) - cbs.c_first) * cbs.cstride_b;
        rin64[S][i] = __builtin_amdgcn_raw_buffer_load_b128(cbs.rsrc, go64[i] == kOOB ? kOOB : go64[i] + chb, 0, 0);
      }
    } else if constexpr (VD) {
#pragma unroll
      for (int ic = 0; ic < NCQ; ++ic) {
        const unsigned so = static_cast<unsigned>(min(c0 + wave_u + 4 * ic, p.Cin - 1) - cbs.c_first) * cbs.cstride_b;
#pragma unroll
        for (int t = 0; t < NTR; ++t) rin4[S][ic][t] = __builtin_amdgcn_raw_buffer_load_b128(cbs.rsrc, goff[t], so, 0);
      }
    } else {
#pragma unroll
    for (int c = 0; c < NC; ++c) {
      const unsigned so = static_cast<unsigned>(min(c0 + c, p.Cin - 1) - cbs.c_first) * cbs.cstride_b;
#pragma unroll
      for (int i = 0; i < RQ; ++i) rin[S][c][i] = __uint_as_float(__builtin_amdgcn_raw_buffer_load_b32(cbs.rsrc, goff[i], so, 0));
    }
    }
    const unsigned wso = static_cast<unsigned>(c0) * wstride_b;
#pragma unroll
    for (int q = 0; q < RWN; ++q)
      rw[S][q] = __builtin_amdgcn_raw_buffer_load_b128(wr, (wci[q] < kend - c0) ? woff[q] + wso : kOOB, 0, 0);
  };
  auto commit = [&](auto set) {
    constexpr int S = decltype(set)::value;
    if constexpr (VD64) {
#pragma unroll
      for (int i = 0; i < NI64; ++i) *reinterpret_cast<u32x4*>(in_tile + lo64[i]) = rin64[S][i];
    } else if constexpr (VD) {
#pragma unroll
      for (int ic = 0; ic < NCQ; ++ic)
#pragma unroll
        for (int t = 0; t < NTR; ++t)
          *reinterpret_cast<u32x4*>(in_tile + (wave_u + 4 * ic) * chan_elems + loff[t]) = rin4[S][ic][t];
    } else {
#pragma unroll
    for (int c = 0; c < NC; ++c)
#pragma unroll
      for (int i = 0; i < RQ; ++i) in_tile[c * chan_elems + loff[i]] = rin[S][c][i];
    }
#pragma unroll
    for (int q = 0; q < RWN; ++q) *reinterpret_cast<u32x4*>(w_tile + wl[q]) = rw[S][q];
  };
  auto mma = [&]() {
#pragma unroll 1
  for (int c8 = 0; c8 < (NC >= 8 ? NC / 8 : 1); ++c8) {
    const float* it = in_tile + c8 * 8 * chan_elems;
    const float* wt0 = w_tile + c8 * 8 * WP + aoff;
    if (MODE == MODE_HW) {
      constexpr int NS = (NC == 4) ? 9 : 2 * KTW;
      float a[2][CB], bv[2][4];
      auto frag = [&](int s, int slot) {
        const int tap = (NC == 4) ? s : (s >> 1), cq = (NC == 4) ? 0 : (s & 1);
        const int toff = (tap / 3) * DL * pitch + (tap % 3) * DL;
#pragma unroll
        for (int cb = 0; cb < CB; ++cb) a[slot][cb] = wt0[(tap * NC + cq * 4) * WP + cb * 16];
#pragma unroll
        for (int pb = 0; pb < NPB; ++pb) bv[slot][pb] = it[boff[pb] + cq * 4 * chan_elems + toff];
      };
      frag(0, 0);
#pragma unroll
      for (int s = 0; s < NS; ++s) {
        if (s + 1 < NS) frag(s + 1, (s + 1) & 1);
#pragma unroll
        for (int cb = 0; cb < CB; ++cb)
#pragma unroll
          for (int pb = 0; pb < NPB; ++pb)
            acc[cb][pb] = __builtin_amdgcn_mfma_f32_16x16x4f32(a[s & 1][cb], bv[s & 1][pb], acc[cb][pb], 0, 0, 0);
      }
    } else if (MODE == MODE_HWT) {
      constexpr int KS = (KT == 16) ? 4 : 3, ORG = (KT == 16) ? 1 : 0;
#pragma unroll
      for (int ta = 0; ta < 2; ++ta) {
        int ky, dy;
        if (pa) { ky = ta ? 0 : 2; dy = ta ? 1 : 0; }
        else { if (ta && KT != 16) continue; ky = ta ? 3 : 1; dy = ta ? -1 : 0; }
#pragma unroll
        for (int tb = 0; tb < 2; ++tb) {
          int kx, dx;
          if (pbit) { kx = tb ? 0 : 2; dx = tb ? 1 : 0; }
          else { if (tb && KT != 16) continue; kx = tb ? 3 : 1; dx = tb ? -1 : 0; }
          const int toff = (dy + ORG) * pitch + dx + ORG;
          const float* wt = wt0 + ((ky * KS + kx) * NC) * WP;
#pragma unroll
          for (int cq = 0; cq < 2; ++cq) {
            float a[CB], bv[4];
#pragma unroll
            for (int cb = 0; cb < CB; ++cb) a[cb] = wt[cq * 4 * WP + cb * 16];
#pragma unroll
            for (int pb = 0; pb < NPB; ++pb) bv[pb] = it[boff[pb] + cq * 4 * chan_elems + toff];
#pragma unroll
            for (int cb = 0; cb < CB; ++cb)
#pragma unroll
              for (int pb = 0; pb < NPB; ++pb)
                acc[cb][pb] = __builtin_amdgcn_mfma_f32_16x16x4f32(a[cb], bv[pb], acc[cb][pb], 0, 0, 0);
          }
        }
      }
    } else {
#pragma unroll
      for (int t = 0; t < NTR; ++t) {
        if (t >= ntaps) continue;
        const float* wt = wt0 + (plane_wt[t] * NC) * WP;
#pragma unroll
        for (int cq = 0; cq < 2; ++cq) {
          float a[CB], bv[4];
#pragma unroll
          for (int cb = 0; cb < CB; ++cb) a[cb] = wt[cq * 4 * WP + cb * 16];
#pragma unroll
          for (int pb = 0; pb < NPB; ++pb) bv[pb] = it[boff[pb] + cq * 4 * chan_elems + t * TP];
#pragma unroll
          for (int cb = 0; cb < CB; ++cb)
#pragma unroll
            for (int pb = 0; pb < NPB; ++pb)
              acc[cb][pb] = __builtin_amdgcn_mfma_f32_16x16x4f32(a[cb], bv[pb], acc[cb][pb], 0, 0, 0);
        }
      }
    }
  }
  };
  using S0 = std::integral_constant<int, 0>;
  using S1 = std::integral_constant<int, NSET - 1>;
  fetch(S0{}, kbeg);
  if constexpr (NSET == 2) {
    if (kbeg + NC < kend) fetch(S1{}, kbeg + NC);
    for (int c0 = kbeg; c0 < kend; c0 += 2 * NC) {
      __syncthreads();
      commit(S0{});
      __syncthreads();
      if (c0 + 2 * NC < kend) fetch(S0{}, c0 + 2 * NC);
      mma();
      if (c0 + NC < kend) {
        __syncthreads();
        commit(S1{});
        __syncthreads();
        if (c0 + 3 * NC < kend) fetch(S1{}, c0 + 3 * NC);
        mma();
      }
    }
  } else {
    for (int c0 = kbeg; c0 < kend; c0 += NC) {
      __syncthreads();
      commit(S0{});
      __syncthreads();
      if (c0 + NC < kend) fetch(S0{}, c0 + NC);
      mma();
    }
  }

  const size_t hw_o = static_cast<size_t>(p.Ho) * p.Wo;
  const unsigned oplane = static_cast<unsigned>(p.Do) * static_cast<unsigned>(hw_o);
  const bool split = p.ksplit > 1;
  const __amdgpu_buffer_rsrc_t yr = split
      ? ig_rsrc(p.partial + (static_cast<size_t>(ks) * p.B + b) * p.Cout * oplane, p.part_bytes)
      : ig_rsrc(y + static_cast<long long>(b) * p.out_bstride, p.out_bytes);
  const unsigned ocs = split ? oplane * 4u : static_cast<unsigned>(p.out_cstride) * 4u;
  const float* ab = (MODE == MODE_HW && p.addend) ? p.addend + static_cast<size_t>(b) * p.add_bstride : nullptr;
#pragma unroll
  for (int pb = 0; pb < NPB; ++pb) {
    unsigned opix, ppix = 0;
    bool inside;
    if (PR) {
      const int base = (DL == 1) ? wave * 2 : (wave & 1) + 4 * (wave >> 1);
      const int oy = ty0 + base + ((kq < 2) ? DL : 0), ox = tx0 + (pb & 1) * 16 + j;
      inside = oy < p.Ho && ox < p.Wo;
      ppix = static_cast<unsigned>(oy) * p.Wo + ox;
      opix = static_cast<unsigned>(od) * static_cast<unsigned>(hw_o) + ppix;
    } else if (MODE == MODE_D) {
      const unsigned px = px0 + wave * (TP / 4) + pb * 16 + j;
      inside = px < HW;
      opix = static_cast<unsigned>(od) * HW + px;
    } else {
      int oy = (TP == 64) ? ty0 + wave : ty0 + wave * 2 + (pb >> 1), ox = (TP == 64) ? tx0 + j : tx0 + (pb & 1) * 16 + j;
      if (MODE == MODE_HWT) {
        inside = oy < p.H && ox < p.W;
        oy = 2 * oy + pa; ox = 2 * ox + pbit;
        inside = inside && oy < p.Ho && ox < p.Wo;
      } else inside = oy < p.Ho && ox < p.Wo;
      ppix = static_cast<unsigned>(oy) * p.Wo + ox;
      opix = static_cast<unsigned>(od) * static_cast<unsigned>(hw_o) + ppix;
    }
#pragma unroll
    for (int cb = 0; cb < CB; ++cb)
#pragma unroll
      for (int r = 0; r < 4; ++r) {
        const int co = PR ? (kq & 1) * 4 + r : co0 + cb * 16 + kq * 4 + r;
        const unsigned off = (inside && co < p.Cout) ? opix * 4u + static_cast<unsigned>(co) * ocs : kOOB;
        float v = acc[cb][pb][r];
        if (!split) {
          if (MODE == MODE_HW && ab) v += ab[static_cast<size_t>(min(co, p.Cout - 1)) * p.add_cstride + static_cast<size_t>(od) * p.add_dstride + (inside ? ppix : 0u)];
          v = apply_act(v * esc[cb][r] + esh[cb][r], p.act, p.act_param, co);
        }
        __builtin_amdgcn_raw_buffer_store_b32(__float_as_uint(v), yr, off, 0, 0);
      }
  }
}



constexpr int kEpiPitch = 272;
template <int NCB, int NPB = 4>
__device__ __forceinline__ void epilogue_stage(float* epi, const float (&v)[NCB][NPB][4], int wave, int kq, int j) {
#pragma unroll
  for (int cb = 0; cb < NCB; ++cb)
#pragma unroll
    for (int pb = 0; pb < NPB; ++pb)
#pragma unroll
      for (int r = 0; r < 4; ++r) epi[(cb * 16 + kq * 4 + r) * kEpiPitch + wave * (NPB * 16) + pb * 16 + j] = v[cb][pb][r];
}
template <int NCB, int NT = 256, int QPC = 64, class QuadOffset>
__device__ __forceinline__ void epilogue_flush(const float* epi, __amdgpu_buffer_rsrc_t yr, unsigned ocs, int co_base, int Cout,
                                               QuadOffset quad_offset) {
#pragma unroll
  for (int it = 0; it < NCB * 16 * QPC / NT; ++it) {
    const int idx = static_cast<int>(threadIdx.x) + NT * it;
    const int col = idx / QPC, q = idx % QPC;
    const u32x4 val = *reinterpret_cast<const u32x4*>(epi + col * kEpiPitch + q * 4);
    const unsigned po = quad_offset(q);
    const int co = co_base + col;
    const unsigned off = (po != kOOB && co < Cout) ? po + static_cast<unsigned>(co) * ocs : kOOB;
    __builtin_amdgcn_raw_buffer_store_b128(val, yr, off, 0, 0);
  }
}

constexpr int X6_NC = 16, X6_SLOTS = 10;

__global__ void __launch_bounds__(256)
weight_split6_kernel(const float* __restrict__ w_t, u32x4* __restrict__ w6, int Cin, int coutp, int nchunk, int Cout, long long sci,
                     long long sco, long long st, int flip) {
  const int n = nchunk * X6_SLOTS * 2 * coutp;
  for (int i = blockIdx.x * blockDim.x + threadIdx.x; i < n; i += gridDim.x * blockDim.x) {
    const int co = i % coutp;
    int r = i / coutp;
    const int g = r & 1; r >>= 1;
    const int slot = r % X6_SLOTS, chunk = r / X6_SLOTS;
    float v[8];
#pragma unroll
    for (int e = 0; e < 8; ++e) {
      const int ci = chunk * X6_NC + g * 8 + e;
      if (Cout > 0) v[e] = (slot < 9 && ci < Cin && co < Cout) ? w_t[ci * sci + co * sco + (flip ? 8 - slot : slot) * st] : 0.f;
      else v[e] = (slot < 9 && ci < Cin) ? w_t[(static_cast<size_t>(ci) * 9 + slot) * coutp + co] : 0.f;
    }
    unsigned part[3][4];
#pragma unroll
    for (int e = 0; e < 4; ++e) split6(v[2 * e], v[2 * e + 1], part[0][e], part[1][e], part[2][e]);
#pragma unroll
    for (int pt = 0; pt < 3; ++pt)
      w6[(((static_cast<size_t>(chunk) * 3 + pt) * X6_SLOTS + slot) * 2 + g) * coutp + co] =
          u32x4{part[pt][0], part[pt][1], part[pt][2], part[pt][3]};
  }
}

template <int CB, int DL, int TR = 8>
__global__ void __launch_bounds__(256, TR == 8 ? 2 : 3)
ig_conv_x6_kernel(const float* __restrict__ x, const u32x4* __restrict__ w6, const float* __restrict__ scale,
                  const float* __restrict__ shift, float* __restrict__ y, const IG p) {
  extern __shared__ __attribute__((aligned(16))) u32x4 lds6[];
  static_assert(TR == 8 || DL == 1, "4-row tiles: dilation 1");
  constexpr int NPB = TR / 2;
  constexpr int SPC = TR == 8 ? 2 : 4;
  constexpr int in_rows = TR + 2 * DL, QPR = 10, LCOLS = 4 * QPR, NPIX = in_rows * LCOLS;
  constexpr int NPIXP = NPIX;
  static_assert(NPIXP % 16 == 0, "block pitch");
  constexpr int SLOTS = in_rows * QPR;
  static_assert(SPC * SLOTS <= 256, "staging slots");
  constexpr int COB = CB * 16;
  constexpr int WV = 3 * X6_SLOTS * 2 * COB;
  constexpr int RWN = (WV + 255) / 256;
  u32x4* in6 = lds6;
  u32x4* w6s = lds6 + 3 * 2 * NPIXP;

  const int wave = threadIdx.x >> 6, lane = threadIdx.x & 63;
  const int j = lane & 15, kq = lane >> 4;
  unsigned lin = blockIdx.x + gridDim.x * (blockIdx.y + gridDim.y * blockIdx.z);
  {
    const unsigned total = gridDim.x * gridDim.y * gridDim.z, per = total / 8;
    if (p.xcd && lin < per * 8) lin = (lin % 8) * per + lin / 8;
  }
  const int tile = lin % gridDim.x;
  const int od = (lin / gridDim.x) % gridDim.y;
  const int bz = lin / (gridDim.x * gridDim.y);
  const int cog = bz % p.co_groups;
  const int ks = (bz / p.co_groups) % p.ksplit, b = bz / (p.co_groups * p.ksplit);
  const int kbeg = ks * p.kspan, kend = min(p.Cin, kbeg + p.kspan);
  const int co0 = cog * COB;
  const int ty0 = (tile / p.tiles_x) * TR, tx0 = (tile % p.tiles_x) * 32;
  const unsigned HW = static_cast<unsigned>(p.H) * p.W;
  const unsigned cstride_b = static_cast<unsigned>(p.in_cstride) * 4u, cstride2_b = static_cast<unsigned>(p.in2_cstride) * 4u;

  const bool stager = threadIdx.x < SPC * SLOTS;
  const int spart = static_cast<int>(threadIdx.x) / SLOTS;
  const int sg = TR == 8 ? spart : (spart >> 1), shalf = spart & 1;
  const int sslot = static_cast<int>(threadIdx.x) - spart * SLOTS;
  const int srow = sslot / QPR, squad = sslot - srow * QPR;
  unsigned goff = kOOB;
  {
    const int gy = ty0 - DL + srow, gx = tx0 - 4 + 4 * squad;
    if (stager && gy >= 0 && gy < p.H && gx >= 0 && gx < p.W)
// ... 36 lines not shown
      const int co = min(co0 + cb * 16 + kq * 4 + r, p.coutp - 1);
      esc[cb][r] = scale ? scale[co] : 1.f;
      esh[cb][r] = shift ? shift[co] : 0.f;
    }

  constexpr int NCH = 16 / SPC;
  v4f rin[NCH];
  u32x4 rw[RWN];
  auto fetch = [&](int c0) {
    const ChunkBase cbs = chunk_base(c0, p.csplit, xr, xr2, cstride_b, cstride2_b);
#pragma unroll
    for (int c = 0; c < NCH; ++c) {
      const unsigned co = static_cast<unsigned>(min(c0 + spart * NCH + c, p.Cin - 1) - cbs.c_first) * cbs.cstride_b;
      rin[c] = __builtin_bit_cast(v4f, __builtin_amdgcn_raw_buffer_load_b128(cbs.rsrc, goff == kOOB ? kOOB : goff + co, 0, 0));
    }
    const unsigned wso = static_cast<unsigned>(c0 / X6_NC) * wchunk_b;
#pragma unroll
    for (int q = 0; q < RWN; ++q) rw[q] = __builtin_amdgcn_raw_buffer_load_b128(wr, woff[q], wso, 0);
  };
  auto commit = [&]() {
    if (stager) {
#pragma unroll
      for (int i = 0; i < 4; ++i) {
        unsigned part[3][NCH / 2];
#pragma unroll
        for (int e = 0; e < NCH / 2; ++e) split6(rin[2 * e][i], rin[2 * e + 1][i], part[0][e], part[1][e], part[2][e]);
#pragma unroll
        for (int pt = 0; pt < 3; ++pt) {
          if constexpr (TR == 8) in6[pt * 2 * NPIXP + lpix + i] = u32x4{part[pt][0], part[pt][1], part[pt][2], part[pt][3]};
          else reinterpret_cast<u32x2*>(in6 + pt * 2 * NPIXP + lpix + i)[shalf] = u32x2{part[pt][0], part[pt][1]};
        }
      }
    }
#pragma unroll
    for (int q = 0; q < RWN; ++q) w6s[wl[q]] = rw[q];
  };

  fetch(kbeg);
  for (int c0 = kbeg; c0 < kend; c0 += X6_NC) {
    __syncthreads();
    commit();
    __syncthreads();
    if (c0 + X6_NC < kend) fetch(c0 + X6_NC);
    v4f part[CB][NPB];
#pragma unroll
    for (int cb = 0; cb < CB; ++cb)
#pragma unroll
      for (int pb = 0; pb < NPB; ++pb) part[cb][pb] = v4f{0.f, 0.f, 0.f, 0.f};
    bf16x8 a[2][3][CB], bv[2][3][2];
    auto load_a = [&](int s, int buf) {
      const int slot = 2 * s + tsel;
#pragma unroll
      for (int pt = 0; pt < 3; ++pt)
#pragma unroll
        for (int cb = 0; cb < CB; ++cb)
          a[buf][pt][cb] = __builtin_bit_cast(bf16x8, w6s[((pt * X6_SLOTS + slot) * 2) * COB + aoff + cb * 16]);
    };
    auto load_b = [&](int s, int h, int buf) {
      const int slot = 2 * s + tsel;
      const int tap = slot < 9 ? slot : 8;
      const int toff = (tap / 3) * DL * LCOLS + (tap % 3) * DL;
#pragma unroll
      for (int pt = 0; pt < 3; ++pt)
#pragma unroll
        for (int k = 0; k < 2; ++k) bv[buf][pt][k] = __builtin_bit_cast(bf16x8, in6[pt * 2 * NPIXP + boff[2 * h + k] + toff]);
    };
    constexpr int NH = NPB / 2;
    load_a(0, 0);
    load_b(0, 0, 0);
#pragma unroll
    for (int u = 0; u < 5 * NH; ++u) {
      const int s = u / NH, h = u % NH;
      if (u + 1 < 5 * NH) {
        load_b((u + 1) / NH, (u + 1) % NH, (u + 1) & 1);
        if (h == NH - 1) load_a(s + 1, (s + 1) & 1);
      }
      constexpr int PA[6] = {0, 2, 1, 0, 1, 0}, PB[6] = {2, 0, 1, 1, 0, 0};
#pragma unroll
      for (int t = 0; t < 6; ++t)
#pragma unroll
        for (int cb = 0; cb < CB; ++cb)
#pragma unroll
          for (int k = 0; k < 2; ++k)
            part[cb][2 * h + k] = __builtin_amdgcn_mfma_f32_16x16x32_bf16(a[s & 1][PA[t]][cb], bv[u & 1][PB[t]][k], part[cb][2 * h + k], 0, 0, 0);
    }
#pragma unroll
    for (int cb = 0; cb < CB; ++cb)
#pragma unroll
      for (int pb = 0; pb < NPB; ++pb) acc[cb][pb] += part[cb][pb];
  }

  const size_t hw_o = static_cast<size_t>(p.Ho) * p.Wo;
  const bool split = p.ksplit > 1;
  const unsigned oplane = static_cast<unsigned>(p.Do) * static_cast<unsigned>(hw_o);
  const __amdgpu_buffer_rsrc_t yr = split
      ? ig_rsrc(p.partial + (static_cast<size_t>(ks) * p.B + b) * p.Cout * oplane, p.part_bytes)
      : ig_rsrc(y + static_cast<long long>(b) * p.out_bstride, p.out_bytes);
  const unsigned ocs = split ? oplane * 4u : static_cast<unsigned>(p.out_cstride) * 4u;
  const float* ab = (p.addend && !split) ? p.addend + static_cast<size_t>(b) * p.add_bstride : nullptr;
  float outv[CB][NPB][4];
#pragma unroll
  for (int pb = 0; pb < NPB; ++pb) {
    const int oy = ty0 + (TR == 8 ? wave * 2 + (pb >> 1) : wave), ox = tx0 + (pb & 1) * 16 + j;
    const bool inside = oy < p.Ho && ox < p.Wo;
    const unsigned ppix = static_cast<unsigned>(oy) * p.Wo + ox;
#pragma unroll
    for (int cb = 0; cb < CB; ++cb)
#pragma unroll
      for (int r = 0; r < 4; ++r) {
        const int co = co0 + cb * 16 + kq * 4 + r;
        float v = acc[cb][pb][r];
        if (ab) v += ab[static_cast<size_t>(min(co, p.Cout - 1)) * p.add_cstride + static_cast<size_t>(od) * p.add_dstride + (inside ? ppix : 0u)];
        outv[cb][pb][r] = split ? v : apply_act(v * esc[cb][r] + esh[cb][r], p.act, p.act_param, co);
      }
  }
  __syncthreads();
  float* epi = reinterpret_cast<float*>(lds6);
  epilogue_stage<CB, NPB>(epi, outv, wave, kq, j);
  __syncthreads();
  const unsigned obase = static_cast<unsigned>(od) * static_cast<unsigned>(hw_o);
  epilogue_flush<CB, 256, TR * 8>(epi, yr, ocs, co0, p.Cout, [&](int q) {
    const int oy = ty0 + (q >> 3), ox = tx0 + (q & 7) * 4;
    return (oy < p.Ho && ox < p.Wo) ? (obase + static_cast<unsigned>(oy) * p.Wo + ox) * 4u : kOOB;
  });
}

__global__ void __launch_bounds__(256)
conv_splitk_finish(const float* __restrict__ partial, const float* __restrict__ scale, const float* __restrict__ shift,
                   float* __restrict__ y, int B, int Cout, long long plane, int ksplit, int act, float act_param,
                   long long out_bstride, long long out_cstride, const float* __restrict__ addend, long long add_bstride,
                   long long hw_o) {
  const int bc = blockIdx.y;
  const int co = bc % Cout, b = bc / Cout;
  const long long n = static_cast<long long>(B) * Cout * plane;
  const float* pp = partial + static_cast<long long>(bc) * plane;
  float* yp = y + b * out_bstride + co * out_cstride;
  const float* ap = addend ? addend + b * add_bstride + co * hw_o : nullptr;
  const float sc = scale ? scale[co] : 1.f, sh = shift ? shift[co] : 0.f;
  const unsigned uplane = static_cast<unsigned>(plane), uhw = static_cast<unsigned>(hw_o);
  for (unsigned px = blockIdx.x * blockDim.x + threadIdx.x; px < uplane; px += gridDim.x * blockDim.x) {
    float v = 0.f;
    for (int k = 0; k < ksplit; ++k) v += pp[k * n + px];
    if (ap) v += ap[px % uhw];
    yp[px] = apply_act(v * sc + sh, act, act_param, co);
  }
}

thread_local int g_chunk_cap = 32;
const long long g_pf_max_wgs = ts::env_ll("TS_CONV_PF_MAX_WGS", 512);
const long long g_small_hw = ts::env_ll("TS_CONV_HW_SMALL_WGS", 256);
const bool g_small_over_pairing = ts::env_ll("TS_CONV_SMALL_OVER_PAIRING", 1) != 0;
const bool g_row_pairing = ts::env_not_zero("TS_CONV_ROW_PAIRING");

template <int CB, int MODE, int KT, int ST, int DL, int NC, int PR = 0, int PF = 0, int TP = 256>
int launch_one(const float* x, const float* w, const float* scale, const float* shift, float* y, const IG& p,
               dim3 grid, hipStream_t st) {
  using G = Geom<MODE, KT, ST, DL, TP>;
  constexpr int WP = (CB * 16) | 16;
  constexpr int KTW = PR ? 12 : KT;
  constexpr size_t lds = (static_cast<size_t>(NC) * G::chan_elems + static_cast<size_t>(KTW) * NC * WP + 4) * sizeof(float);
  static_assert(lds <= 160 * 1024, "ig_conv_kernel: tile does not fit the LDS");
  auto kern = &ig_conv_kernel<CB, MODE, KT, ST, DL, NC, PR, PF, TP>;
  if (lds > 64 * 1024) {
    static bool raised = false;
    if (!raised) {
      (void)hipFuncSetAttribute(reinterpret_cast<const void*>(kern), hipFuncAttributeMaxDynamicSharedMemorySize, static_cast<int>(lds));
      raised = true;
    }
  }
  hipLaunchKernelGGL(kern, grid, dim3(256), lds, st, x, w, scale, shift, y, p);
  return ts::launched("ig_conv_kernel");
}

template <int CB, int MODE, int KT, int ST, int DL, int TP = 256>
int launch_nc(long long wgs, const float* x, const float* w, const float* scale, const float* shift, float* y, const IG& p,
              dim3 grid, hipStream_t st) {
  using G = Geom<MODE, KT, ST, DL, TP>;
  constexpr int WP = (CB * 16) | 16;
  constexpr size_t per_ch = (static_cast<size_t>(G::chan_elems) + static_cast<size_t>(KT) * WP) * sizeof(float);
  constexpr size_t lds_cu = 160 * 1024;
  const size_t per_cu = static_cast<size_t>((wgs + ts::kNumCU - 1) / ts::kNumCU);
  if constexpr (MODE == MODE_HW && TP == 256) {
    if (p.Cin <= 4 && p.ksplit == 1) return launch_one<CB, MODE, KT, ST, DL, 4>(x, w, scale, shift, y, p, grid, st);
  }
  const int max_nc = g_chunk_cap;
  if constexpr (MODE == MODE_HW && KT == 9 && ST == 1 && CB == 1 && TP == 256) {
    if (p.Cout <= 8 && g_row_pairing) {
      constexpr size_t per_ch2 = (static_cast<size_t>(G::chan_elems) + 12 * WP) * sizeof(float);
      auto fits2 = [&](int nc) { return nc <= max_nc && (nc * per_ch2 + 16) * per_cu <= lds_cu && p.kspan >= nc; };
      if (fits2(32)) return launch_one<CB, MODE, KT, ST, DL, 32, 1>(x, w, scale, shift, y, p, grid, st);
      if (fits2(16)) return launch_one<CB, MODE, KT, ST, DL, 16, 1>(x, w, scale, shift, y, p, grid, st);
      return launch_one<CB, MODE, KT, ST, DL, 8, 1>(x, w, scale, shift, y, p, grid, st);
    }
  }
  auto fits = [&](int nc) { return nc <= max_nc && (nc * per_ch + 16) * per_cu <= lds_cu && p.kspan >= nc; };
  if constexpr (32 * per_ch + 16 <= lds_cu) { if (fits(32)) return launch_one<CB, MODE, KT, ST, DL, 32, 0, 0, TP>(x, w, scale, shift, y, p, grid, st); }
  if constexpr (16 * per_ch + 16 <= lds_cu) { if (fits(16)) return launch_one<CB, MODE, KT, ST, DL, 16, 0, 0, TP>(x, w, scale, shift, y, p, grid, st); }
  if constexpr (CB <= 2) {
    if (wgs < g_pf_max_wgs && p.kspan > 8) return launch_one<CB, MODE, KT, ST, DL, 8, 0, 1, TP>(x, w, scale, shift, y, p, grid, st);
  }
  return launch_one<CB, MODE, KT, ST, DL, 8, 0, 0, TP>(x, w, scale, shift, y, p, grid, st);
}

template <int MODE, int KT, int ST, int DL>
int launch_ig(const float* x, const float* w, const float* scale, const float* shift, float* y, IG p, int B,
              int grid_x, int grid_y, hipStream_t st) {
  {
    const unsigned long long plane = static_cast<unsigned long long>(p.Do) * p.Ho * p.Wo;
    const unsigned long long out_b = (static_cast<unsigned long long>(p.Cout - 1) * p.out_cstride + plane) * 4ull;
    const unsigned long long part_b = static_cast<unsigned long long>(p.Cout) * plane * 4ull;
    TS_REQUIRE(out_b < 0x7fffffffull && part_b < 0x7fffffffull && p.out_cstride >= 0, TS_ERR_UNSUPPORTED,
               "conv: a batch element of y spans 2 GiB or more");
    p.out_bytes = static_cast<unsigned>(out_b); p.part_bytes = static_cast<unsigned>(part_b);
  }
  const int need = (p.Cout + 15) / 16;
  int cb = need >= 4 ? 4 : (need >= 2 ? 2 : 1);
  auto groups = [&](int c) { return (need + c - 1) / c; };
  const long long tiles = static_cast<long long>(grid_x) * grid_y * B * p.ksplit;
  while (cb > 1 && tiles * groups(cb) < ts::kNumCU + ts::kNumCU / 2) cb >>= 1;
  p.co_groups = groups(cb);
  p.B = B;
  static const int xcd = ts::env_not_zero("TS_CONV_XCD") ? 1 : 0;
  p.xcd = xcd;
  const long long wgs = tiles * p.co_groups;
  if constexpr (MODE == MODE_D) {
    static const long long small = ts::env_ll("TS_CONV_D_SMALL_WGS", 256);
    if (wgs <= small && cb == 1) {
      const int gx64 = (p.H * p.W + 63) / 64;
      const dim3 grid64(gx64, grid_y, B * p.co_groups * p.ksplit);
      return launch_nc<1, MODE, KT, ST, DL, 64>(4 * wgs, x, w, scale, shift, y, p, grid64, st);
    }
  }
  if constexpr (MODE == MODE_HW) {
    if (wgs <= g_small_hw && cb == 1 && p.Cin > 4 && !(p.Cout <= 8 && ST == 1 && g_row_pairing && !(g_small_over_pairing && p.Cin >= 64))) {
      p.tiles_x = (p.Wo + 15) / 16;
      const int gx64 = ((p.Ho + 3) / 4) * p.tiles_x;
      const dim3 grid64(gx64, grid_y, B * p.co_groups * p.ksplit);
      return launch_nc<1, MODE, KT, ST, DL, 64>(4 * wgs, x, w, scale, shift, y, p, grid64, st);
    }
  }
  if constexpr (MODE == MODE_HWT) {
    if (wgs <= g_small_hw && cb == 1) {
      p.tiles_x = (p.W + 15) / 16;
      const int gx64 = ((p.H + 3) / 4) * p.tiles_x * 4;
      const dim3 grid64(gx64, grid_y, B * p.co_groups * p.ksplit);
      return launch_nc<1, MODE, KT, ST, DL, 64>(4 * wgs, x, w, scale, shift, y, p, grid64, st);
    }
  }
  const dim3 grid(grid_x, grid_y, B * p.co_groups * p.ksplit);
  if (cb == 4) return launch_nc<4, MODE, KT, ST, DL>(wgs, x, w, scale, shift, y, p, grid, st);
  if (cb == 2) return launch_nc<2, MODE, KT, ST, DL>(wgs, x, w, scale, shift, y, p, grid, st);
  return launch_nc<1, MODE, KT, ST, DL>(wgs, x, w, scale, shift, y, p, grid, st);
}

__global__ void __launch_bounds__(256)
weight_layout_kernel(const float* __restrict__ w, float* __restrict__ out, int A, int T, int nb, int bpad, long long sa, long long sb,
                     long long st, int flip) {
  const unsigned n = static_cast<unsigned>(A) * static_cast<unsigned>(T) * static_cast<unsigned>(bpad);
  for (unsigned i = blockIdx.x * blockDim.x + threadIdx.x; i < n; i += gridDim.x * blockDim.x) {
    const unsigned r = i / static_cast<unsigned>(bpad);
    const int b = static_cast<int>(i - r * static_cast<unsigned>(bpad));
    const unsigned a = r / static_cast<unsigned>(T);
    const int t = static_cast<int>(r - a * static_cast<unsigned>(T));
    out[i] = b < nb ? w[static_cast<long long>(a) * sa + b * sb + (flip ? T - 1 - t : t) * st] : 0.f;
  }
}

struct WeightLayoutDesc {
  const float* w; float* out;
  int A, T, nb, bpad;
  long long sa, sb, st;
  int flip, reserved;
};
static_assert(sizeof(WeightLayoutDesc) == 64, "table entry layout");

__global__ void __launch_bounds__(256)
weight_layout_many_kernel(const WeightLayoutDesc* __restrict__ table) {
  const WeightLayoutDesc d = table[blockIdx.y];
  const long long n = static_cast<long long>(d.A) * d.T * d.bpad;
  for (long long i = static_cast<long long>(blockIdx.x) * blockDim.x + threadIdx.x; i < n;
       i += static_cast<long long>(gridDim.x) * blockDim.x) {
    const int b = static_cast<int>(i % d.bpad);
    const long long r = i / d.bpad;
    const int t = static_cast<int>(r % d.T), a = static_cast<int>(r / d.T);
    d.out[i] = b < d.nb ? d.w[a * d.sa + b * d.sb + (d.flip ? d.T - 1 - t : t) * d.st] : 0.f;
  }
}

struct WeightLayoutDesc2 {
  const float* w; float* out;
  int A, T, nb, col0;
  long long sa, sb, st;
  long long out_sa, out_st;
  int flip, reserved;
};
static_assert(sizeof(WeightLayoutDesc2) == 80, "table entry layout");

__global__ void __launch_bounds__(256)
weight_layout_many2_kernel(const WeightLayoutDesc2* __restrict__ table) {
  const WeightLayoutDesc2 d = table[blockIdx.y];
  const long long n = static_cast<long long>(d.A) * d.T * d.nb;
  for (long long i = static_cast<long long>(blockIdx.x) * blockDim.x + threadIdx.x; i < n;
       i += static_cast<long long>(gridDim.x) * blockDim.x) {
    const int b = static_cast<int>(i % d.nb);
    const long long r = i / d.nb;
    const int t = static_cast<int>(r % d.T), a = static_cast<int>(r / d.T);
    d.out[a * d.out_sa + t * d.out_st + d.col0 + b] = d.w[a * d.sa + b * d.sb + (d.flip ? d.T - 1 - t : t) * d.st];
  }
}

bool ig_extent(IG& p, int KT) {
  const unsigned long long in_b = (static_cast<unsigned long long>(p.Cin - 1) * p.in_cstride + static_cast<unsigned long long>(p.D) * p.H * p.W) * 4ull;
  const unsigned long long w_b = static_cast<unsigned long long>(p.Cin) * KT * p.coutp * 4ull;
  if (in_b >= 0x7fffffffull || w_b >= 0x7fffffffull || p.in_cstride < 0) return false;
  p.in_bytes = static_cast<unsigned>(in_b); p.w_bytes = static_cast<unsigned>(w_b);
  p.out_bytes = p.part_bytes = 0;
  p.x2 = nullptr; p.csplit = 0x7fffffff; p.in2_bstride = p.in2_cstride = 0; p.in2_bytes = 0;
  return true;
}

struct SplitIn {
  const float* x2;
  int csplit;
  long long bstride, cstride;
};
bool split_point_ok(int Cin, int Csplit) { return Csplit > 0 && Csplit < Cin && Csplit % 32 == 0; }
bool ig_split(IG& p, const SplitIn& sp) {
  const unsigned long long plane = static_cast<unsigned long long>(p.D) * p.H * p.W;
  const unsigned long long b1 = (static_cast<unsigned long long>(sp.csplit - 1) * p.in_cstride + plane) * 4ull;
  const unsigned long long b2 = (static_cast<unsigned long long>(p.Cin - sp.csplit - 1) * sp.cstride + plane) * 4ull;
  if (b1 >= 0x7fffffffull || b2 >= 0x7fffffffull || sp.cstride < 0) return false;
  p.in_bytes = static_cast<unsigned>(b1);
  p.x2 = sp.x2; p.csplit = sp.csplit; p.in2_bstride = sp.bstride; p.in2_cstride = sp.cstride; p.in2_bytes = static_cast<unsigned>(b2);
  return true;
}

struct WG {
  int B, Cin, Cout, D, H, W, Do, Ho, Wo;
  int stride, dil, pad, k;
  int tiles_x, tiles_per_plane, ntiles;
  int cop;
  int vec;
  long long x_bstride, x_cstride, dy_bstride, dy_cstride;
  unsigned x_bytes, dy_bytes;
};

template <int MODE, int KT, int ST, int DL>
__global__ void __launch_bounds__(256)
wgrad_kernel(const float* __restrict__ x, const float* __restrict__ dy, float* __restrict__ part, const WG p) {
  extern __shared__ __attribute__((aligned(16))) float lds[];
  constexpr int CIP = 17;
  constexpr int TRW = (MODE == MODE_HW) ? (ST == 2 ? 4 : 8) : 8;
  constexpr int NPX = (MODE == MODE_HW) ? TRW * 32 : 256;
  constexpr int in_rows = (MODE == MODE_HW) ? (TRW - 1) * ST + 2 * DL + 1 : 1;
  constexpr int in_cols = (MODE == MODE_HW) ? 31 * ST + 2 * DL + 1 : 256;
  constexpr int NIN = (MODE == MODE_HW) ? in_rows * in_cols : KT * 256;
  constexpr int RQ = (NIN + 255) / 256;
  float* xs = lds;
  float* dys = lds + NIN * CIP;
  const int wave = threadIdx.x >> 6, lane = threadIdx.x & 63;
  const int j = lane & 15, kq = lane >> 4;
  const int ci0 = blockIdx.y * 16;
  const int cob = (p.Cout + 15) / 16, nitems = KT * cob;
  const unsigned HW = static_cast<unsigned>(p.H) * p.W, HWo = static_cast<unsigned>(p.Ho) * p.Wo;

  const int cbsplit = cob >= 3 ? 4 : cob, pxsplit = 4 / cbsplit;
  const int cb = wave % cbsplit, part_px = wave / cbsplit;
  const bool working = cb < cob;
  v4f acc[KT];
#pragma unroll
  for (int i = 0; i < KT; ++i) acc[i] = v4f{0.f, 0.f, 0.f, 0.f};

  for (int tile = blockIdx.x; tile < p.ntiles; tile += gridDim.x) {
    const int sp = tile % p.tiles_per_plane;
    const int od = (tile / p.tiles_per_plane) % p.Do, b = tile / (p.tiles_per_plane * p.Do);
    const __amdgpu_buffer_rsrc_t xr = ig_rsrc(x + static_cast<size_t>(b) * p.x_bstride, p.x_bytes);
    const __amdgpu_buffer_rsrc_t yr = ig_rsrc(dy + static_cast<size_t>(b) * p.dy_bstride, p.dy_bytes);
    int ty0 = 0, tx0 = 0;
    if (MODE == MODE_HW) { ty0 = (sp / p.tiles_x) * TRW; tx0 = (sp % p.tiles_x) * 32; }
    __syncthreads();
    if constexpr (MODE == MODE_HW) {
      if (p.vec) {
        constexpr int QPR = (in_cols + 4 - DL + 3) / 4;
        constexpr int SL = in_rows * QPR;
        constexpr int CPT = (SL <= 128) ? 8 : 16;
        const int slot = (SL <= 128) ? static_cast<int>(threadIdx.x & 127) : static_cast<int>(threadIdx.x);
        const int cfirst = (SL <= 128) ? static_cast<int>(threadIdx.x >> 7) * 8 : 0;
        if (slot < SL) {
          const int cy = slot / QPR, qx = slot - cy * QPR;
          const int gy = ty0 * ST - DL + cy, gx4 = tx0 * ST - 4 + 4 * qx;
          const bool rowok = gy >= 0 && gy < p.H && gx4 >= 0 && gx4 < p.W;
          const unsigned off = rowok ? (static_cast<unsigned>(od) * HW + static_cast<unsigned>(gy) * p.W + gx4) * 4u : kOOB;
          u32x4 v[CPT];
#pragma unroll
          for (int c = 0; c < CPT; ++c) {
            const int ch = ci0 + cfirst + c;
            const unsigned so = static_cast<unsigned>(min(ch, p.Cin - 1)) * static_cast<unsigned>(p.x_cstride) * 4u;
            v[c] = __builtin_amdgcn_raw_buffer_load_b128(xr, (ch < p.Cin) ? off : kOOB, so, 0);
          }
          const int cx0 = 4 * qx - (4 - DL);
#pragma unroll
          for (int e = 0; e < 4; ++e) {
            const int cx = cx0 + e;
            if (cx >= 0 && cx < in_cols) {
#pragma unroll
              for (int c = 0; c < CPT; ++c) xs[(cy * in_cols + cx) * CIP + cfirst + c] = __uint_as_float(v[c][e]);
            }
          }
        }
      }
    }
    if (MODE != MODE_HW || !p.vec) {
#pragma unroll
    for (int q = 0; q < RQ; ++q) {
      const int i = threadIdx.x + 256 * q;
      unsigned off = kOOB;
      if (i < NIN) {
        if (MODE == MODE_HW) {
          const int cy = i / in_cols, cx = i - cy * in_cols;
          const int gy = ty0 * ST - DL + cy, gx = tx0 * ST - DL + cx;
          if (gy >= 0 && gy < p.H && gx >= 0 && gx < p.W) off = (static_cast<unsigned>(od) * HW + static_cast<unsigned>(gy) * p.W + gx) * 4u;
        } else {
          const int t = i >> 8, px = sp * 256 + (i & 255);
          const int id = od * p.stride + t * p.dil - p.pad;
          if (id >= 0 && id < p.D && px < static_cast<int>(HW)) off = (static_cast<unsigned>(id) * HW + px) * 4u;
        }
      }
      float v[16];
#pragma unroll
      for (int c = 0; c < 16; ++c) {
        const unsigned so = static_cast<unsigned>(min(ci0 + c, p.Cin - 1)) * static_cast<unsigned>(p.x_cstride) * 4u;
        v[c] = __uint_as_float(__builtin_amdgcn_raw_buffer_load_b32(xr, (ci0 + c < p.Cin) ? off : kOOB, so, 0));
      }
      if (i < NIN) {
#pragma unroll
        for (int c = 0; c < 16; ++c) xs[i * CIP + c] = v[c];
      }
    }
    }
    for (int i = threadIdx.x; i < NPX; i += 256) {
      unsigned off = kOOB;
      if (MODE == MODE_HW) {
        const int oy = ty0 + i / 32, ox = tx0 + (i & 31);
        if (oy < p.Ho && ox < p.Wo) off = (static_cast<unsigned>(od) * HWo + static_cast<unsigned>(oy) * p.Wo + ox) * 4u;
      } else {
        const int px = sp * 256 + i;
        if (px < static_cast<int>(HWo)) off = (static_cast<unsigned>(od) * HWo + px) * 4u;
      }
      for (int c0 = 0; c0 < cob * 16; c0 += 16) {
        float v[16];
#pragma unroll
        for (int c = 0; c < 16; ++c) {
          const unsigned so = static_cast<unsigned>(min(c0 + c, p.Cout - 1)) * static_cast<unsigned>(p.dy_cstride) * 4u;
          v[c] = __uint_as_float(__builtin_amdgcn_raw_buffer_load_b32(yr, (c0 + c < p.Cout) ? off : kOOB, so, 0));
        }
#pragma unroll
        for (int c = 0; c < 16; ++c) dys[i * p.cop + c0 + c] = v[c];
      }
    }
    __syncthreads();
    if (working) {
      const int nstep = (NPX / 4) / pxsplit, s0 = part_px * nstep;
      const float* ap = dys + kq * p.cop + cb * 16 + j;
      const float* bp = xs + (MODE == MODE_HW ? kq * ST : kq) * CIP + j;
#pragma unroll 2
      for (int step = s0; step < s0 + nstep; ++step) {
        int xo;
        if (MODE == MODE_HW) xo = ((step >> 3) * ST * in_cols + (step & 7) * 4 * ST) * CIP;
        else xo = step * 4 * CIP;
        const float a = ap[step * 4 * p.cop];
// ... 543 lines not shown
extern "C" int ts_conv3d_hw_split_supported(int B, int Cin, int Csplit, int Cout, int D, int H, int W, int stride, int dilation,
                                            int transposed) {
  if (B <= 0 || Cout <= 0 || D <= 0 || H <= 0 || W <= 0 || transposed || !split_point_ok(Cin, Csplit)) return 0;
  if (!(stride == 1 || stride == 2) || !(dilation == 1 || dilation == 2) || (stride == 2 && dilation == 2)) return 0;
  const int ks = conv_hw_ksplit(B, Cin, Cout, D, (H - 1) / stride + 1, (W - 1) / stride + 1, stride);
  return ks == 1 || (((Cin + ks - 1) / ks + 7) / 8 * 8) % 32 == 0;
}

extern "C" int ts_conv3d_hw_split_fwd(const float* x, const float* x2, const float* w_t, const float* scale, const float* shift, float* y,
                                      int B, int Cin, int Csplit, int Cout, int D, int H, int W, int stride, int dilation,
                                      int transposed, int act, float act_param,
                                      long long in_bstride, long long in_cstride, long long in2_bstride, long long in2_cstride,
                                      long long out_bstride, long long out_cstride, const float* addend, long long addend_bstride,
                                      void* workspace, size_t workspace_bytes, void* stream) {
  const SplitIn sp{x2, Csplit, in2_bstride, in2_cstride};
  return conv_hw_impl(x, w_t, scale, shift, y, B, Cin, Cout, D, H, W, stride, dilation, transposed, act, act_param,
                      in_bstride, in_cstride, out_bstride, out_cstride, addend, addend_bstride, workspace, workspace_bytes,
                      0, 0, stream, 0, 0, &sp);
}

extern "C" size_t ts_conv3d_hw_warp_workspace_bytes(int B, int Cout, int D, int H, int W) {
  if (B <= 0 || Cout <= 0 || D <= 0 || H <= 0 || W <= 0) return 0;
  return ts::round_up(static_cast<size_t>(B) * Cout * D * H * W * sizeof(float), 256);
}

extern "C" int ts_conv3d_hw_warp_fwd(const float* corr, const float* w_t, const float* scale, const float* shift, float* y,
                                     const float* q, const float* disp, const float* base,
                                     int B, int Cc, int Cout, int D, int H, int W, int dilation, int act, float act_param,
                                     long long in_bstride, long long in_cstride, long long out_bstride, long long out_cstride,
                                     long long base_bstride, void* workspace, size_t workspace_bytes, void* stream) {
  TS_REQUIRE(B > 0 && Cc > 0 && Cout > 0 && D > 0 && H > 0 && W >= 2, TS_ERR_SHAPE, "conv3d_hw_warp: bad size");
  TS_REQUIRE(dilation == 1 || dilation == 2, TS_ERR_UNSUPPORTED, "conv3d_hw_warp: dilation must be 1 or 2");
  TS_REQUIRE(D <= 65535 && static_cast<long long>(B) * ((Cout + 7) / 8) <= 65535, TS_ERR_UNSUPPORTED, "conv3d_hw_warp: grid too large");
  TS_REQUIRE_PTR(corr); TS_REQUIRE_PTR(w_t); TS_REQUIRE_PTR(y); TS_REQUIRE_PTR(q); TS_REQUIRE_PTR(disp); TS_REQUIRE_PTR(workspace);
  TS_REQUIRE(workspace_bytes >= ts_conv3d_hw_warp_workspace_bytes(B, Cout, D, H, W), TS_ERR_SHAPE, "conv3d_hw_warp: workspace too small");
  TS_REQUIRE(9ull * Cout * H * W * 4ull < 0x7fffffffull, TS_ERR_UNSUPPORTED, "conv3d_hw_warp: a batch element of q spans 2 GiB or more");
  hipStream_t st = ts::as_stream(stream);
  float* T = reinterpret_cast<float*>(workspace);
  const long long HW = static_cast<long long>(H) * W;
  const long long wgs = ((HW + 255) / 256) * D * B * ((Cout + 7) / 8);
  TS_REQUIRE(wgs < (1ll << 31), TS_ERR_UNSUPPORTED, "conv3d_hw_warp: grid too large");
  const dim3 grid(static_cast<unsigned>(wgs));
  if (dilation == 1) hipLaunchKernelGGL(warp_gather_kernel<1>, grid, dim3(256), 0, st, q, disp, base, T, Cout, D, H, W, base_bstride);
  else hipLaunchKernelGGL(warp_gather_kernel<2>, grid, dim3(256), 0, st, q, disp, base, T, Cout, D, H, W, base_bstride);
  if (int rc = ts::launched("warp_gather_kernel")) return rc;
  return conv_hw_impl(corr, w_t, scale, shift, y, B, Cc, Cout, D, H, W, 1, dilation, 0, act, act_param, in_bstride, in_cstride,
                      out_bstride, out_cstride, T, static_cast<long long>(Cout) * D * HW, nullptr, 0, 0, 0, stream,
                      static_cast<long long>(D) * HW, HW);
}

extern "C" int ts_conv3d_hw_bwd_data(const float* dy, const float* w_b, float* dx, int B, int Cin, int Cout, int D, int H,
                                     int W, int stride, int dilation, int transposed, long long dy_bstride,
                                     long long dy_cstride, long long dx_bstride, long long dx_cstride, void* stream) {
  TS_REQUIRE(B > 0 && Cin > 0 && Cout > 0 && D > 0 && H > 0 && W > 0, TS_ERR_SHAPE, "conv3d_hw_bwd_data: non-positive size");
  TS_REQUIRE(stride == 1 || stride == 2, TS_ERR_UNSUPPORTED, "conv3d_hw_bwd_data: stride must be 1 or 2");
  if (transposed)
    return conv_hw_impl(dy, w_b, nullptr, nullptr, dx, B, Cout, Cin, D, 2 * H, 2 * W, 2, 1, 0, ACT_NONE, 0.f, dy_bstride,
                        dy_cstride, dx_bstride, dx_cstride, nullptr, 0, nullptr, 0, 0, 0, stream);
  const int Ho = (H - 1) / stride + 1, Wo = (W - 1) / stride + 1;
  if (stride == 2)
    return conv_hw_impl(dy, w_b, nullptr, nullptr, dx, B, Cout, Cin, D, Ho, Wo, 2, 1, 1, ACT_NONE, 0.f, dy_bstride,
                        dy_cstride, dx_bstride, dx_cstride, nullptr, 0, nullptr, 0, H, W, stream);
  return conv_hw_impl(dy, w_b, nullptr, nullptr, dx, B, Cout, Cin, D, Ho, Wo, 1, dilation, 0, ACT_NONE, 0.f, dy_bstride,
                      dy_cstride, dx_bstride, dx_cstride, nullptr, 0, nullptr, 0, 0, 0, stream);
}

extern "C" size_t ts_conv3d_bwd_weight_workspace_bytes(int Cin, int Cout, int taps) {
  if (Cin <= 0 || Cout <= 0 || taps <= 0) return 0;
  const int ciblocks = (Cin + 15) / 16, cob = (Cout + 15) / 16;
  return static_cast<size_t>(wgrad_groups_max(ciblocks)) * ciblocks * taps * cob * 256 * sizeof(float);
}

extern "C" int ts_conv3d_hw_bwd_weight(const float* x, const float* dy, float* dw, int B, int Cin, int Cout, int D, int H,
                                       int W, int stride, int dilation, long long x_bstride, long long x_cstride,
                                       long long dy_bstride, long long dy_cstride, void* workspace,
                                       size_t workspace_bytes, void* stream) {
  TS_REQUIRE(B > 0 && Cin > 0 && Cout > 0 && D > 0 && H > 0 && W > 0, TS_ERR_SHAPE, "conv3d_hw_bwd_weight: non-positive size");
  TS_REQUIRE(Cout <= 64, TS_ERR_UNSUPPORTED, "conv3d_hw_bwd_weight: Cout=%d > 64", Cout);
  TS_REQUIRE((stride == 1 && (dilation == 1 || dilation == 2)) || (stride == 2 && dilation == 1), TS_ERR_UNSUPPORTED,
             "conv3d_hw_bwd_weight: stride/dilation outside {1/1, 1/2, 2/1}");
  TS_REQUIRE_PTR(x); TS_REQUIRE_PTR(dy); TS_REQUIRE_PTR(dw);
  WG p;
  p.B = B; p.Cin = Cin; p.Cout = Cout; p.D = D; p.H = H; p.W = W; p.Do = D;
  p.Ho = (H - 1) / stride + 1; p.Wo = (W - 1) / stride + 1;
  p.stride = stride; p.dil = dilation; p.pad = dilation; p.k = 3;
  p.x_bstride = x_bstride; p.x_cstride = x_cstride; p.dy_bstride = dy_bstride; p.dy_cstride = dy_cstride;
  TS_REQUIRE(wg_extent(p), TS_ERR_UNSUPPORTED, "conv3d_hw_bwd_weight: a batch element spans 2 GiB or more");
  hipStream_t st = ts::as_stream(stream);
  if (stride == 2) return launch_wgrad<MODE_HW, 9, 2, 1>(x, dy, dw, p, workspace, workspace_bytes, st);
  if (dilation == 2) return launch_wgrad<MODE_HW, 9, 1, 2>(x, dy, dw, p, workspace, workspace_bytes, st);
  return launch_wgrad<MODE_HW, 9, 1, 1>(x, dy, dw, p, workspace, workspace_bytes, st);
}

namespace {
int conv_d_impl(const float* x, const float* w_t, const float* scale, const float* shift, float* y,
                int B, int Cin, int Cout, int Din, int H, int W, int k, int stride, int dilation,
                int padding, int transposed, int act, float act_param,
                long long in_bstride, long long in_cstride, long long out_bstride,
                long long out_cstride, int out_d, void* stream, const SplitIn* sp = nullptr) {
  TS_REQUIRE(B > 0 && Cin > 0 && Cout > 0 && Din > 0 && H > 0 && W > 0, TS_ERR_SHAPE, "conv3d_d: non-positive size");
  TS_REQUIRE(k == 1 || k == 3 || k == 5, TS_ERR_UNSUPPORTED, "conv3d_d: k must be 1, 3 or 5");
  TS_REQUIRE(stride >= 1 && stride <= 2 && dilation >= 1 && padding >= 0, TS_ERR_UNSUPPORTED, "conv3d_d: bad stride/dilation/padding");
  TS_REQUIRE(!transposed || (k == 3 && stride == 2 && dilation == 1 && padding == 1), TS_ERR_UNSUPPORTED,
             "conv3d_d: transposed form is k=3, stride 2, padding 1");
  TS_REQUIRE(act >= 0 && act <= 3, TS_ERR_SHAPE, "conv3d_d: unknown activation");
  TS_REQUIRE_PTR(x); TS_REQUIRE_PTR(w_t); TS_REQUIRE_PTR(y);
  const int bucket = cout_bucket(Cout);
  const int Dout = transposed ? (out_d ? out_d : 2 * Din) : (Din + 2 * padding - dilation * (k - 1) - 1) / stride + 1;
  TS_REQUIRE(Dout > 0 && Dout <= 65535, TS_ERR_SHAPE, "conv3d_d: bad output depth");
  TS_REQUIRE(!transposed || (Dout >= 2 * Din - 1 && Dout <= 2 * Din), TS_ERR_SHAPE, "conv3d_d: transposed depth %d is not 2D-1 | 2D", Dout);
  hipStream_t st = ts::as_stream(stream);
  IG p;
  p.Cin = Cin; p.Cout = Cout; p.coutp = bucket; p.D = Din; p.H = H; p.W = W; p.Do = Dout; p.Ho = H; p.Wo = W;
  p.stride = stride; p.dil = dilation; p.pad = padding; p.k = k; p.transposed = transposed;
  p.act = act; p.act_param = act_param;
  p.in_bstride = in_bstride; p.in_cstride = in_cstride; p.out_bstride = out_bstride; p.out_cstride = out_cstride;
  p.tiles_x = 1; p.co_groups = 1; p.ksplit = 1; p.kspan = Cin; p.partial = nullptr;
  p.addend = nullptr; p.add_bstride = 0; p.add_cstride = 0; p.add_dstride = 0;
  TS_REQUIRE(ig_extent(p, k), TS_ERR_UNSUPPORTED, "conv3d_d: a batch element of x spans 2 GiB or more");
  if (sp) {
    TS_REQUIRE_PTR(sp->x2);
    TS_REQUIRE(split_point_ok(Cin, sp->csplit), TS_ERR_UNSUPPORTED, "conv3d_d_split: Csplit=%d must be a multiple of 32 inside (0, Cin=%d)",
               sp->csplit, Cin);
    TS_REQUIRE(ig_split(p, *sp), TS_ERR_UNSUPPORTED, "conv3d_d_split: a batch element of x2 spans 2 GiB or more");
  }
  const int tiles = (H * W + 255) / 256;
  if (k == 1) return launch_ig<MODE_D, 1, 1, 1>(x, w_t, scale, shift, y, p, B, tiles, Dout, st);
  if (k == 3) return launch_ig<MODE_D, 3, 1, 1>(x, w_t, scale, shift, y, p, B, tiles, Dout, st);
  return launch_ig<MODE_D, 5, 1, 1>(x, w_t, scale, shift, y, p, B, tiles, Dout, st);
}
}

extern "C" int ts_conv3d_d_fwd(const float* x, const float* w_t, const float* scale, const float* shift, float* y,
                               int B, int Cin, int Cout, int Din, int H, int W, int k, int stride, int dilation,
                               int padding, int transposed, int act, float act_param,
                               long long in_bstride, long long in_cstride, long long out_bstride,
                               long long out_cstride, void* stream) {
  return conv_d_impl(x, w_t, scale, shift, y, B, Cin, Cout, Din, H, W, k, stride, dilation, padding, transposed, act,
                     act_param, in_bstride, in_cstride, out_bstride, out_cstride, 0, stream);
}

extern "C" int ts_conv3d_d_split_supported(int Cin, int Csplit) { return split_point_ok(Cin, Csplit); }

extern "C" int ts_conv3d_d_split_fwd(const float* x, const float* x2, const float* w_t, const float* scale, const float* shift, float* y,
                                     int B, int Cin, int Csplit, int Cout, int Din, int H, int W, int k, int stride, int dilation,
                                     int padding, int transposed, int act, float act_param,
                                     long long in_bstride, long long in_cstride, long long in2_bstride, long long in2_cstride,
                                     long long out_bstride, long long out_cstride, void* stream) {
  const SplitIn sp{x2, Csplit, in2_bstride, in2_cstride};
  return conv_d_impl(x, w_t, scale, shift, y, B, Cin, Cout, Din, H, W, k, stride, dilation, padding, transposed, act,
                     act_param, in_bstride, in_cstride, out_bstride, out_cstride, 0, stream, &sp);
}

extern "C" int ts_conv3d_d_bwd_data(const float* dy, const float* w_b, float* dx, int B, int Cin, int Cout, int Din, int H,
                                    int W, int k, int stride, int dilation, int padding, int transposed,
                                    long long dy_bstride, long long dy_cstride, long long dx_bstride, long long dx_cstride,
                                    void* stream) {
  TS_REQUIRE(B > 0 && Cin > 0 && Cout > 0 && Din > 0 && H > 0 && W > 0, TS_ERR_SHAPE, "conv3d_d_bwd_data: non-positive size");
  if (transposed)
    return conv_d_impl(dy, w_b, nullptr, nullptr, dx, B, Cout, Cin, 2 * Din, H, W, 3, 2, 1, 1, 0, ACT_NONE, 0.f, dy_bstride,
                       dy_cstride, dx_bstride, dx_cstride, 0, stream);
  const int Dout = (Din + 2 * padding - dilation * (k - 1) - 1) / stride + 1;
  TS_REQUIRE(Dout > 0, TS_ERR_SHAPE, "conv3d_d_bwd_data: bad forward geometry");
  if (stride == 2) {
    TS_REQUIRE(k == 3 && dilation == 1 && padding == 1, TS_ERR_UNSUPPORTED, "conv3d_d_bwd_data: stride 2 needs k=3, padding 1");
    return conv_d_impl(dy, w_b, nullptr, nullptr, dx, B, Cout, Cin, Dout, H, W, 3, 2, 1, 1, 1, ACT_NONE, 0.f, dy_bstride,
                       dy_cstride, dx_bstride, dx_cstride, Din, stream);
  }
  TS_REQUIRE(stride == 1, TS_ERR_UNSUPPORTED, "conv3d_d_bwd_data: stride must be 1 or 2");
  return conv_d_impl(dy, w_b, nullptr, nullptr, dx, B, Cout, Cin, Dout, H, W, k, 1, dilation, dilation * (k - 1) - padding, 0,
                     ACT_NONE, 0.f, dy_bstride, dy_cstride, dx_bstride, dx_cstride, 0, stream);
}

extern "C" int ts_conv3d_d_bwd_weight(const float* x, const float* dy, float* dw, int B, int Cin, int Cout, int Din, int H,
                                      int W, int k, int stride, int dilation, int padding, long long x_bstride,
                                      long long x_cstride, long long dy_bstride, long long dy_cstride, void* workspace,
                                      size_t workspace_bytes, void* stream) {
  TS_REQUIRE(B > 0 && Cin > 0 && Cout > 0 && Din > 0 && H > 0 && W > 0, TS_ERR_SHAPE, "conv3d_d_bwd_weight: non-positive size");
  TS_REQUIRE(Cout <= 64, TS_ERR_UNSUPPORTED, "conv3d_d_bwd_weight: Cout=%d > 64", Cout);
  TS_REQUIRE(k == 1 || k == 3 || k == 5, TS_ERR_UNSUPPORTED, "conv3d_d_bwd_weight: k must be 1, 3 or 5");
  TS_REQUIRE(stride >= 1 && stride <= 2 && dilation >= 1 && padding >= 0, TS_ERR_UNSUPPORTED, "conv3d_d_bwd_weight: bad stride/dilation/padding");
  TS_REQUIRE_PTR(x); TS_REQUIRE_PTR(dy); TS_REQUIRE_PTR(dw);
  WG p;
  p.B = B; p.Cin = Cin; p.Cout = Cout; p.D = Din; p.H = H; p.W = W; p.Ho = H; p.Wo = W;
  p.Do = (Din + 2 * padding - dilation * (k - 1) - 1) / stride + 1;
  TS_REQUIRE(p.Do > 0, TS_ERR_SHAPE, "conv3d_d_bwd_weight: bad output depth");
  p.stride = stride; p.dil = dilation; p.pad = padding; p.k = k;
  p.x_bstride = x_bstride; p.x_cstride = x_cstride; p.dy_bstride = dy_bstride; p.dy_cstride = dy_cstride;
  TS_REQUIRE(wg_extent(p), TS_ERR_UNSUPPORTED, "conv3d_d_bwd_weight: a batch element spans 2 GiB or more");
  hipStream_t st = ts::as_stream(stream);
  if (k == 1) return launch_wgrad<MODE_D, 1, 1, 1>(x, dy, dw, p, workspace, workspace_bytes, st);
  if (k == 3) return launch_wgrad<MODE_D, 3, 1, 1>(x, dy, dw, p, workspace, workspace_bytes, st);
  return launch_wgrad<MODE_D, 5, 1, 1>(x, dy, dw, p, workspace, workspace_bytes, st);
}

extern "C" int ts_deconv2d_k4s2_fwd(const float* x, const float* w_t, const float* scale, const float* shift, float* y,
                                    int B, int Cin, int Cout, int H, int W, int act, long long out_bstride, void* stream) {
  TS_REQUIRE(B > 0 && Cin > 0 && Cout > 0 && H > 0 && W > 0, TS_ERR_SHAPE, "deconv2d: non-positive size");
  TS_REQUIRE(Cout <= 32, TS_ERR_UNSUPPORTED, "deconv2d: Cout=%d > 32", Cout);
  TS_REQUIRE(act >= 0 && act <= 2, TS_ERR_SHAPE, "deconv2d: unknown activation");
  TS_REQUIRE_PTR(x); TS_REQUIRE_PTR(w_t); TS_REQUIRE_PTR(scale); TS_REQUIRE_PTR(shift); TS_REQUIRE_PTR(y);
  IG p;
  p.Cin = Cin; p.Cout = Cout; p.coutp = cout_bucket(Cout); p.D = 1; p.H = H; p.W = W; p.Do = 1; p.Ho = 2 * H; p.Wo = 2 * W;
  p.stride = 2; p.dil = 1; p.pad = 1; p.k = 4; p.transposed = 1; p.act = act; p.act_param = 0.f;
  p.in_bstride = static_cast<long long>(Cin) * H * W; p.in_cstride = static_cast<long long>(H) * W;
  p.out_bstride = out_bstride; p.out_cstride = 4ll * H * W;
  p.tiles_x = (W + 31) / 32; p.co_groups = 1; p.ksplit = 1; p.kspan = Cin; p.partial = nullptr;
  p.addend = nullptr; p.add_bstride = 0; p.add_cstride = 0; p.add_dstride = 0;
  TS_REQUIRE(ig_extent(p, 16), TS_ERR_UNSUPPORTED, "deconv2d: a batch element of x spans 2 GiB or more");
  const int tiles = ((H + 7) / 8) * p.tiles_x;
  return launch_ig<MODE_HWT, 16, 1, 1>(x, w_t, scale, shift, y, p, B, tiles * 4, 1, ts::as_stream(stream));
}

extern "C" int ts_conv_cout_pad(int cout) { return cout_bucket(cout); }

extern "C" int ts_conv_wgrad_defer(int on) {
  const int was = g_wgrad_defer ? 1 : 0;
  g_wgrad_defer = on != 0;
  return was;
}
extern "C" int ts_conv_wgrad_pending(void) {
  std::lock_guard<std::mutex> lock(g_wgrad_mutex);
  return static_cast<int>(g_wgrad_pending.size());
}
extern "C" int ts_conv_wgrad_take(void* host_table, size_t capacity_bytes, int* n, int* total_blocks) {
  TS_REQUIRE_PTR(host_table); TS_REQUIRE_PTR(n); TS_REQUIRE_PTR(total_blocks);
  std::lock_guard<std::mutex> lock(g_wgrad_mutex);
  const size_t cnt = g_wgrad_pending.size();
  TS_REQUIRE(cnt * sizeof(WgradFinishDesc) <= capacity_bytes, TS_ERR_SHAPE, "conv_wgrad_take: %zu entries do not fit %zu bytes", cnt, capacity_bytes);
  int blocks = 0;
  WgradFinishDesc* out = static_cast<WgradFinishDesc*>(host_table);
  for (size_t i = 0; i < cnt; ++i) {
    out[i] = g_wgrad_pending[i];
    out[i].block0 = blocks;
    blocks += out[i].nitems * 4 * out[i].ciblocks;
  }
  *n = static_cast<int>(cnt);
  *total_blocks = blocks;
  g_wgrad_pending.clear();
  return TS_OK;
}
extern "C" int ts_conv_wgrad_finish_many(const void* table, int n, int total_blocks, void* stream) {
  TS_REQUIRE(n > 0 && total_blocks > 0, TS_ERR_SHAPE, "conv_wgrad_finish_many: empty table");
  TS_REQUIRE_PTR(table);
  hipLaunchKernelGGL(wgrad_finish_many, dim3(static_cast<unsigned>(total_blocks)), dim3(256), 0, ts::as_stream(stream),
                     static_cast<const WgradFinishDesc*>(table), n);
  return ts::launched("wgrad_finish_many");
}

extern "C" int ts_conv_set_chunk_cap(int cap) {
  TS_REQUIRE(cap == 8 || cap == 16 || cap == 32, TS_ERR_SHAPE, "conv_set_chunk_cap: %d is not 8, 16 or 32", cap);
  g_chunk_cap = cap;
  return TS_OK;
}

extern "C" size_t ts_conv3d_hw_workspace_bytes(int B, int Cin, int Cout, int D, int H, int W, int stride, int transposed) {
  if (transposed || B <= 0 || Cin <= 0 || Cout <= 0 || D <= 0 || H <= 0 || W <= 0) return 0;
  const int Ho = (H - 1) / stride + 1, Wo = (W - 1) / stride + 1;
  const int ks = conv_hw_ksplit(B, Cin, Cout, D, Ho, Wo, stride);
  return ks > 1 ? static_cast<size_t>(ks) * B * Cout * D * Ho * Wo * sizeof(float) : 0;
}

extern "C" int ts_conv_weight_layout(const float* w, float* out, int A, int T, int nb, int bpad, long long stride_a,
                                     long long stride_b, long long stride_t, int flip, void* stream) {
  TS_REQUIRE(A > 0 && T > 0 && nb > 0 && bpad >= nb, TS_ERR_SHAPE, "conv_weight_layout: bad size");
  TS_REQUIRE_PTR(w); TS_REQUIRE_PTR(out);
  const long long n = static_cast<long long>(A) * T * bpad;
  TS_REQUIRE(n < (1ll << 31), TS_ERR_UNSUPPORTED, "conv_weight_layout: 2^31 elements or more");
  long long blocks = (n + 255) / 256;
  if (blocks > 1024) blocks = 1024;
  hipLaunchKernelGGL(weight_layout_kernel, dim3(static_cast<unsigned>(blocks)), dim3(256), 0, ts::as_stream(stream), w, out, A, T, nb,
                     bpad, stride_a, stride_b, stride_t, flip);
  return ts::launched("weight_layout_kernel");
}

extern "C" int ts_conv_weight_layout_many2(const void* table, int n, int blocks_x, void* stream) {
  TS_REQUIRE(n > 0 && n <= 65535 && blocks_x > 0 && blocks_x <= 4096, TS_ERR_SHAPE, "conv_weight_layout_many2: bad table size");
  TS_REQUIRE_PTR(table);
  hipLaunchKernelGGL(weight_layout_many2_kernel, dim3(static_cast<unsigned>(blocks_x), static_cast<unsigned>(n)), dim3(256), 0,
                     ts::as_stream(stream), static_cast<const WeightLayoutDesc2*>(table));
  return ts::launched("weight_layout_many2_kernel");
}

extern "C" int ts_conv_weight_layout_many(const void* table, int n, int blocks_x, void* stream) {
  TS_REQUIRE(n > 0 && n <= 65535 && blocks_x > 0 && blocks_x <= 4096, TS_ERR_SHAPE, "conv_weight_layout_many: bad table size");
  TS_REQUIRE_PTR(table);
  hipLaunchKernelGGL(weight_layout_many_kernel, dim3(static_cast<unsigned>(blocks_x), static_cast<unsigned>(n)), dim3(256), 0,
                     ts::as_stream(stream), static_cast<const WeightLayoutDesc*>(table));
  return ts::launched("weight_layout_many_kernel");
}
```

temporalstereo_amd/csrc/conv_common.hpp:

```cpp
#pragma once
#include "ts_common.hpp"

namespace {

enum Act { ACT_NONE = 0, ACT_SILU = 1, ACT_RELU = 2, ACT_TANH_OFFSET = 3, ACT_HEAD_PAIR = 4 };

__device__ __forceinline__ float silu_fast(float v) {
#ifdef TS_EXACT_SILU
  return v / (1.f + expf(-v));
#else
  const float d = 1.f + __builtin_amdgcn_exp2f(v * -1.4426950408889634f);
  const float r = __builtin_amdgcn_rcpf(d);
  const float rn = fmaf(fmaf(-d, r, 1.f), r, r);
  return v * (d < 3.0e38f ? rn : r);
#endif
}

__device__ __forceinline__ float apply_act(float v, int act, float p, int co = 0) {
  if (act == ACT_HEAD_PAIR) act = co == 0 ? ACT_NONE : ACT_TANH_OFFSET;
  switch (act) {
    case ACT_SILU: return silu_fast(v);
    case ACT_RELU: return fmaxf(v, 0.f);
    case ACT_TANH_OFFSET: return fminf(fmaxf(tanhf(v / 100.f), -1.f), 1.f) * p;
    default: return v;
  }
}

typedef float v4f __attribute__((ext_vector_type(4)));
typedef unsigned u32x4 __attribute__((ext_vector_type(4)));
typedef unsigned u32x2 __attribute__((ext_vector_type(2)));
enum { MODE_HW = 0, MODE_HWT = 1, MODE_D = 2 };
constexpr unsigned kOOB = 0x80000000u;

struct IG {
  int Cin, Cout, coutp;
  int D, H, W;
  int Do, Ho, Wo;
  int stride, dil, pad, k, transposed;
  int act;
  float act_param;
  long long in_bstride, in_cstride, out_bstride, out_cstride;
  unsigned in_bytes, w_bytes;
  unsigned out_bytes, part_bytes;
  int tiles_x, co_groups;
  int ksplit, kspan;
  float* partial;
  int B;
  const float* addend;
  long long add_bstride;
  long long add_cstride, add_dstride;
  int xcd;
  const float* x2;
  int csplit;
  long long in2_bstride, in2_cstride;
  unsigned in2_bytes;
};

struct ChunkBase {
  __amdgpu_buffer_rsrc_t rsrc;
  unsigned cstride_b;
  int c_first;
};
__device__ __forceinline__ ChunkBase chunk_base(int c0, int csplit, __amdgpu_buffer_rsrc_t r1, __amdgpu_buffer_rsrc_t r2, unsigned cs1,
                                                unsigned cs2) {
  const bool second = c0 >= csplit;
  return ChunkBase{second ? r2 : r1, second ? cs2 : cs1, second ? csplit : 0};
}

__device__ __forceinline__ __amdgpu_buffer_rsrc_t ig_rsrc(const void* base, unsigned bytes) {
  return __builtin_amdgcn_make_buffer_rsrc(const_cast<void*>(base), 0, bytes, 0x00020000);
}

typedef __bf16 bf16x8 __attribute__((ext_vector_type(8)));
typedef float f32x2 __attribute__((ext_vector_type(2)));
typedef __bf16 bf16x2 __attribute__((ext_vector_type(2)));

__device__ __forceinline__ unsigned pack_bf16(float a, float b) {
  return __builtin_bit_cast(unsigned, __builtin_convertvector(f32x2{a, b}, bf16x2));
}
__device__ __forceinline__ void split6(float a, float b, unsigned& hi, unsigned& mid, unsigned& lo) {
  hi = pack_bf16(a, b);
  a -= __uint_as_float(hi << 16); b -= __uint_as_float(hi & 0xffff0000u);
  mid = pack_bf16(a, b);
  a -= __uint_as_float(mid << 16); b -= __uint_as_float(mid & 0xffff0000u);
  lo = pack_bf16(a, b);
}

}
```

temporalstereo_amd/csrc/plan.hip:

```cpp
#include <cstdint>
#include <cstring>
#include <mutex>
#include <string>
#include <utility>
#include <vector>

#include "ts_common.hpp"

namespace {

constexpr int kMaxWords = 32;

template <class T>
T unpack(unsigned long long w) {
  static_assert(sizeof(T) <= sizeof(unsigned long long), "argument wider than a plan word");
  T v;
  std::memcpy(&v, &w, sizeof(T));
  return v;
}

template <class... A, size_t... I>
int call_with(int (*f)(A...), const unsigned long long* w, std::index_sequence<I...>) {
  return f(unpack<A>(w[I])...);
}
template <class... A>
int call_with(int (*f)(A...), const unsigned long long* w) {
  return call_with(f, w, std::index_sequence_for<A...>{});
}
template <class... A>
constexpr int arity(int (*)(A...)) { return static_cast<int>(sizeof...(A)); }

struct Entry {
  const char* name;
  int (*thunk)(const unsigned long long*);
  int nargs;
};

#define TS_PLAN_OP(fn) Entry{#fn, [](const unsigned long long* w) { return call_with(&fn, w); }, arity(&fn)}

const Entry kTable[] = {
    TS_PLAN_OP(ts_block_cost_int_fwd),      TS_PLAN_OP(ts_block_cost_sampled_fwd),
    TS_PLAN_OP(ts_block_cost_sampled_warped_fwd),
    TS_PLAN_OP(ts_block_cost_sampled_corr_fwd), TS_PLAN_OP(ts_conv3d_hw_warp_fwd),
    TS_PLAN_OP(ts_cat_fms_fwd),             TS_PLAN_OP(ts_dif_fms_fwd),             TS_PLAN_OP(ts_inverse_warp_3d_fwd),
    TS_PLAN_OP(ts_block_cost_int_bwd),      TS_PLAN_OP(ts_block_cost_sampled_bwd),
    TS_PLAN_OP(ts_topk_softargmax_fwd),     TS_PLAN_OP(ts_topk_softargmax_bwd),
    TS_PLAN_OP(ts_softargmin_fwd),          TS_PLAN_OP(ts_softargmin_bwd),
    TS_PLAN_OP(ts_argmax_select_fwd),       TS_PLAN_OP(ts_softsplat_sum_fwd),
    TS_PLAN_OP(ts_softsplat_sum_fwd_deterministic), TS_PLAN_OP(ts_softsplat_sum_bwd_input), TS_PLAN_OP(ts_softsplat_sum_bwd_flow),
    TS_PLAN_OP(ts_softsplat_softmax_fwd),   TS_PLAN_OP(ts_project_to_3d_fwd),
    TS_PLAN_OP(ts_conv3d_hw_fwd),           TS_PLAN_OP(ts_conv3d_d_fwd),
    TS_PLAN_OP(ts_conv3d_hw_bwd_data),      TS_PLAN_OP(ts_conv3d_hw_bwd_weight),
    TS_PLAN_OP(ts_conv3d_d_bwd_data),       TS_PLAN_OP(ts_conv3d_d_bwd_weight),
    TS_PLAN_OP(ts_resize3d_add_act_fwd),    TS_PLAN_OP(ts_pool3d5_avgmax_fwd),
    TS_PLAN_OP(ts_merge_candidates_fwd),    TS_PLAN_OP(ts_convex_upsample_fwd),
    TS_PLAN_OP(ts_convex_upsample_candidates_fwd),
    TS_PLAN_OP(ts_unet_upsample_fwd),       TS_PLAN_OP(ts_deconv2d_k4s2_fwd),
    TS_PLAN_OP(ts_resize_bilinear_fwd),     TS_PLAN_OP(ts_range_candidates_fwd),
    TS_PLAN_OP(ts_copy_rows_fwd),           TS_PLAN_OP(ts_stream_fork),
    TS_PLAN_OP(ts_event_record),            TS_PLAN_OP(ts_event_wait),
    TS_PLAN_OP(ts_resize3d_add_act_bwd),    TS_PLAN_OP(ts_pool3d5_avgmax_bwd),
    TS_PLAN_OP(ts_merge_candidates_bwd),
    TS_PLAN_OP(ts_reproject_memory_fwd),
    TS_PLAN_OP(ts_resize_bilinear_pair_fwd),
    TS_PLAN_OP(ts_calib_stream),             TS_PLAN_OP(ts_conv_set_chunk_cap),
    TS_PLAN_OP(ts_wasserstein_loss_fwd),     TS_PLAN_OP(ts_wasserstein_loss_bwd),
    TS_PLAN_OP(ts_disp_smooth_l1_fwd),       TS_PLAN_OP(ts_disp_smooth_l1_bwd),
    TS_PLAN_OP(ts_disp_metrics_fwd),         TS_PLAN_OP(ts_disp_render_fwd),
    TS_PLAN_OP(ts_correlation_fwd),          TS_PLAN_OP(ts_correlation_bwd),
    TS_PLAN_OP(ts_bn_stats_fwd),             TS_PLAN_OP(ts_bn_apply_act_fwd),
    TS_PLAN_OP(ts_bn_act_bwd_reduce),        TS_PLAN_OP(ts_bn_act_bwd_apply),
    TS_PLAN_OP(ts_convex_upsample_bwd),      TS_PLAN_OP(ts_unet_upsample_bwd),
    TS_PLAN_OP(ts_conv_weight_layout),      TS_PLAN_OP(ts_conv_weight_layout_many),
    TS_PLAN_OP(ts_conv3d_hw_x6_fwd),        TS_PLAN_OP(ts_conv3d_hw_x6_weight_split), TS_PLAN_OP(ts_conv3d_hw_x6_weight_split_from),
    TS_PLAN_OP(ts_conv3d_hw_x6s_fwd),       TS_PLAN_OP(ts_conv3d_hw_x6s_weight_split),
    TS_PLAN_OP(ts_peer_all_gather),         TS_PLAN_OP(ts_peer_all_reduce_sum),
    TS_PLAN_OP(ts_bn_train_fwd),            TS_PLAN_OP(ts_bn_train_bwd),
    TS_PLAN_OP(ts_channel_splice_fwd),
    TS_PLAN_OP(ts_candidates_in_range_fwd), TS_PLAN_OP(ts_candidates_in_range_bwd),
    TS_PLAN_OP(ts_offset_head_fwd),         TS_PLAN_OP(ts_offset_head_bwd),
    TS_PLAN_OP(ts_space_to_depth2_fwd),
    TS_PLAN_OP(ts_deconv2d_k4s2_weight_to_conv3), TS_PLAN_OP(ts_deconv2d_k4s2_wgrad_from_conv3),
    TS_PLAN_OP(ts_clip_rmsprop_step),       TS_PLAN_OP(ts_bn_sync_merge),
    TS_PLAN_OP(ts_bn_fold_many),
    TS_PLAN_OP(ts_conv_weight_layout_many2), TS_PLAN_OP(ts_conv_wgrad_finish_many), TS_PLAN_OP(ts_channel_sum_fwd),
    TS_PLAN_OP(ts_block_cost_sampled_warped_bwd),
    TS_PLAN_OP(ts_frames_prepare_fwd),      TS_PLAN_OP(ts_intrinsics_pyramid_fwd),  TS_PLAN_OP(ts_disp_u16_decode_fwd),
    TS_PLAN_OP(ts_frames_augment_fwd),      TS_PLAN_OP(ts_disp_u16_window_fwd),
    TS_PLAN_OP(ts_block_cost_sampled_corr_split_fwd), TS_PLAN_OP(ts_conv3d_hw_split_fwd),
    TS_PLAN_OP(ts_conv3d_d_split_fwd),      TS_PLAN_OP(ts_conv3d_hw_x6_split_fwd),
    TS_PLAN_OP(ts_inverse_warp_fwd),        TS_PLAN_OP(ts_inverse_warp_bwd),
    TS_PLAN_OP(ts_raft_corr_pyramid_fwd),   TS_PLAN_OP(ts_raft_corr_lookup_fwd),
    TS_PLAN_OP(ts_raft_corr_lookup_bwd),    TS_PLAN_OP(ts_raft_corr_pyramid_bwd),
    TS_PLAN_OP(ts_flow_corr_pyramid_fwd),   TS_PLAN_OP(ts_flow_corr_lookup_fwd),
    TS_PLAN_OP(ts_flow_corr_lookup_bwd),    TS_PLAN_OP(ts_flow_corr_pyramid_bwd),
    TS_PLAN_OP(ts_flow_metrics_fwd),        TS_PLAN_OP(ts_flow_render_fwd),         TS_PLAN_OP(ts_flow_u16_decode_fwd),
    TS_PLAN_OP(ts_spp3d_pool_fwd),          TS_PLAN_OP(ts_spp3d_pool_bwd),
    TS_PLAN_OP(ts_spp3d_expand_fwd),        TS_PLAN_OP(ts_spp3d_expand_bwd),        TS_PLAN_OP(ts_depth_sum3_fwd),
    TS_PLAN_OP(ts_bn_small_train_bwd),
};

struct Call {
  const Entry* op;
  unsigned long long w[kMaxWords];
};

__global__ void __launch_bounds__(256)
copy_rows_kernel(const float* __restrict__ src, float* __restrict__ dst, long long rows, long long row_elems,
                 long long src_pitch, long long dst_pitch) {
  const long long n = rows * row_elems;
  for (long long i = static_cast<long long>(blockIdx.x) * blockDim.x + threadIdx.x; i < n;
       i += static_cast<long long>(gridDim.x) * blockDim.x) {
    const long long r = i / row_elems, c = i - r * row_elems;
    dst[r * dst_pitch + c] = src[r * src_pitch + c];
  }
}

__global__ void __launch_bounds__(256)
copy_rows4_kernel(const float4* __restrict__ src, float4* __restrict__ dst, long long row_quads, long long src_pitch_q,
                  long long dst_pitch_q) {
  const float4* s = src + blockIdx.y * src_pitch_q;
  float4* d = dst + blockIdx.y * dst_pitch_q;
  for (long long i = static_cast<long long>(blockIdx.x) * blockDim.x + threadIdx.x; i < row_quads;
       i += static_cast<long long>(gridDim.x) * blockDim.x)
    d[i] = s[i];
}

}

struct ts_plan {
  std::vector<Call> calls;
};

extern "C" ts_plan* ts_plan_create(void) { return new (std::nothrow) ts_plan(); }

extern "C" void ts_plan_destroy(ts_plan* plan) { delete plan; }

extern "C" int ts_plan_length(const ts_plan* plan) { return plan ? static_cast<int>(plan->calls.size()) : -1; }

extern "C" int ts_plan_add_call(ts_plan* plan, const char* name, const unsigned long long* words, int n_words) {
  TS_REQUIRE_PTR(plan); TS_REQUIRE_PTR(name);
  TS_REQUIRE(n_words >= 0 && n_words <= kMaxWords, TS_ERR_SHAPE, "plan: %d argument words", n_words);
  TS_REQUIRE(n_words == 0 || words != nullptr, TS_ERR_NULL, "plan: words is NULL");
  for (const Entry& e : kTable) {
    if (std::strcmp(e.name, name) != 0) continue;
    TS_REQUIRE(e.nargs == n_words, TS_ERR_SHAPE, "plan: %s takes %d arguments, got %d", name, e.nargs, n_words);
    Call c;
    c.op = &e;
    std::memset(c.w, 0, sizeof(c.w));
    if (n_words) std::memcpy(c.w, words, sizeof(unsigned long long) * n_words);
    plan->calls.push_back(c);
    return TS_OK;
  }
  return ts::fail(TS_ERR_UNSUPPORTED, "plan: %s is not a launching entry point", name);
}

extern "C" int ts_plan_run(ts_plan* plan) {
  TS_REQUIRE_PTR(plan);
  for (const Call& c : plan->calls) {
    const int rc = c.op->thunk(c.w);
    if (rc != TS_OK) return rc;
  }
  return TS_OK;
}

extern "C" int ts_stream_fork(void* from_stream, void* to_stream) {
  constexpr int kRing = 64;
  constexpr int kMaxDev = 16;
  struct Ring { hipEvent_t ev[kRing]; int made = 0, next = 0; };
  static thread_local Ring rings[kMaxDev];
  int dev = 0;
  hipError_t e = hipGetDevice(&dev);
  if (e != hipSuccess) return ts::fail(static_cast<int>(e), "stream_fork: %s", hipGetErrorString(e));
  TS_REQUIRE(dev >= 0 && dev < kMaxDev, TS_ERR_UNSUPPORTED, "stream_fork: device %d", dev);
  Ring& r = rings[dev];
  if (r.made < kRing && r.next == r.made) {
    e = hipEventCreateWithFlags(&r.ev[r.made], hipEventDisableTiming);
    if (e != hipSuccess) return ts::fail(static_cast<int>(e), "stream_fork: %s", hipGetErrorString(e));
    ++r.made;
  }
  hipEvent_t ev = r.ev[r.next];
  r.next = (r.next + 1) % kRing;
  e = hipEventRecord(ev, ts::as_stream(from_stream));
  if (e == hipSuccess) e = hipStreamWaitEvent(ts::as_stream(to_stream), ev, 0);
  if (e != hipSuccess) return ts::fail(static_cast<int>(e), "stream_fork: %s", hipGetErrorString(e));
  return TS_OK;
}

namespace {
hipEvent_t g_slot[256];
bool g_slot_made[256];
bool g_slot_recorded[256];
std::mutex g_slot_lock;
}

extern "C" int ts_event_record(int slot, void* stream) {
  TS_REQUIRE(slot >= 0 && slot < 256, TS_ERR_SHAPE, "event_record: slot %d", slot);
  std::lock_guard<std::mutex> hold(g_slot_lock);
  if (!g_slot_made[slot]) {
    hipError_t e = hipEventCreateWithFlags(&g_slot[slot], hipEventDisableTiming);
    if (e != hipSuccess) return ts::fail(static_cast<int>(e), "event_record: %s", hipGetErrorString(e));
    g_slot_made[slot] = true;
  }
  hipError_t e = hipEventRecord(g_slot[slot], ts::as_stream(stream));
  if (e != hipSuccess) return ts::fail(static_cast<int>(e), "event_record: %s", hipGetErrorString(e));
  g_slot_recorded[slot] = true;
  return TS_OK;
}

extern "C" int ts_event_wait(int slot, void* stream) {
  TS_REQUIRE(slot >= 0 && slot < 256, TS_ERR_SHAPE, "event_wait: slot %d", slot);
  std::lock_guard<std::mutex> hold(g_slot_lock);
  if (!g_slot_recorded[slot]) return TS_OK;
  hipError_t e = hipStreamWaitEvent(ts::as_stream(stream), g_slot[slot], 0);
  if (e != hipSuccess) return ts::fail(static_cast<int>(e), "event_wait: %s", hipGetErrorString(e));
  return TS_OK;
}

namespace {
__global__ void __launch_bounds__(256)
channel_splice_kernel(const float* __restrict__ first, const float* __restrict__ second, float* __restrict__ out, int C, int mc,
                      long long N, long long fb, long long sb, long long ob) {
  const int c = blockIdx.y, b = blockIdx.z;
  const float* src = c < mc ? (first ? first + b * fb + static_cast<long long>(c) * N : nullptr) : second + b * sb + static_cast<long long>(c) * N;
  float* dst = out + b * ob + static_cast<long long>(c) * N;
  for (long long i = static_cast<long long>(blockIdx.x) * blockDim.x + threadIdx.x; i < N; i += static_cast<long long>(gridDim.x) * blockDim.x)
    dst[i] = src ? src[i] : 0.f;
}
}

extern "C" int ts_channel_splice_fwd(const float* first, const float* second, float* out, int B, int C, int mc, long long N,
                                     long long first_bstride, long long second_bstride, long long out_bstride, void* stream) {
  TS_REQUIRE(B > 0 && C > 0 && N > 0 && mc >= 0 && mc <= C && B <= 65535 && C <= 65535, TS_ERR_SHAPE, "channel_splice: bad size");
  TS_REQUIRE_PTR(second); TS_REQUIRE_PTR(out);
  long long blocks = (N + 255) / 256;
  if (blocks > 64) blocks = 64;
  hipLaunchKernelGGL(channel_splice_kernel, dim3(static_cast<unsigned>(blocks), C, B), dim3(256), 0, ts::as_stream(stream), first, second,
                     out, C, mc, N, first_bstride, second_bstride, out_bstride);
  return ts::launched("channel_splice_kernel");
}

extern "C" int ts_copy_rows_fwd(const float* src, float* dst, long long rows, long long row_elems, long long src_pitch,
                                long long dst_pitch, void* stream) {
  TS_REQUIRE(rows > 0 && row_elems > 0 && src_pitch >= row_elems && dst_pitch >= row_elems, TS_ERR_SHAPE,
             "copy_rows: bad geometry");
  TS_REQUIRE_PTR(src); TS_REQUIRE_PTR(dst);
  if (rows <= 65535 && row_elems % 4 == 0 && src_pitch % 4 == 0 && dst_pitch % 4 == 0 &&
      (reinterpret_cast<uintptr_t>(src) | reinterpret_cast<uintptr_t>(dst)) % 16 == 0) {
    const long long rq = row_elems / 4;
    long long bx = (rq + 255) / 256;
    const long long cap = (8192 + rows - 1) / rows;
    if (bx > cap) bx = cap;
// ... 11 lines not shown
```

temporalstereo_amd/csrc/ts_common.hpp:

```cpp
#pragma once
#include <hip/hip_runtime.h>

#include <cstdarg>
#include <cstdint>
#include <cstdio>
#include <cstdlib>
#include <type_traits>

#include "../../include/ts_hip.h"

#define TS_ABI_VERSION 18

namespace ts {

char* err_buf();
int fail(int code, const char* fmt, ...);

inline hipStream_t as_stream(void* s) { return reinterpret_cast<hipStream_t>(s); }

inline bool aligned16(const void* p) { return (reinterpret_cast<uintptr_t>(p) & 15u) == 0; }

inline size_t round_up(size_t v, size_t a) { return (v + a - 1) / a * a; }

inline int launched(const char* what) {
  hipError_t e = hipGetLastError();
  if (e != hipSuccess) return fail(static_cast<int>(e), "%s: %s", what, hipGetErrorString(e));
  return TS_OK;
}

template <class F>
inline void dispatch_bool(bool b, F&& f) {
  if (b) f(std::true_type{});
  else f(std::false_type{});
}

inline long long env_ll(const char* name, long long dflt) { const char* e = getenv(name); return e ? atoll(e) : dflt; }
inline bool env_not_zero(const char* name) { const char* e = getenv(name); return !(e && e[0] == '0'); }

constexpr int kWave = 64;
constexpr int kNumCU = 256;
constexpr int kNumXCD = 8;

}

#define TS_REQUIRE_PTR(p)                                                     \
  do {                                                                        \
    if ((p) == nullptr) return ts::fail(TS_ERR_NULL, "%s is NULL", #p);       \
  } while (0)
#define TS_REQUIRE_ALIGNED(p)                                                          \
  do {                                                                                 \
    if (!ts::aligned16(p)) return ts::fail(TS_ERR_ALIGN, "%s not 16-byte aligned", #p); \
  } while (0)
#define TS_REQUIRE(cond, code, ...)                       \
  do {                                                    \
    if (!(cond)) return ts::fail((code), __VA_ARGS__);    \
  } while (0)
```

Before: 1619.

## Fold decoder depth convs, shortcut, upsample and add into one kernel

In the hourglass decoder, the (3,1,1) depth conv of the main path and the shortcut's depth conv are merged with the trilinear depth upsample and the residual add-plus-activation into a single implicit-GEMM launch over concatenated channels. Per-output-depth weights fold the linear interpolation and the BN scales into the conv weights on device, and are rebuilt when the plan tape replays. This removes the intermediate depth-conv outputs and the separate resize_add_act pass over full-resolution volumes. In exchange it keeps a weight array per output depth and adds complexity to the kernel's channel-segment logic. It is on by default via TS_HG_FOLD.

```diff
diff --git a/include/ts_hip.h b/include/ts_hip.h
--- a/include/ts_hip.h
+++ b/include/ts_hip.h
@@ -53,6 +53,13 @@
                           int padding, int transposed, int act, float act_param,
                           long long in_bstride, long long in_cstride, long long in2_bstride, long long in2_cstride,
                           long long out_bstride, long long out_cstride, void* stream);
+int ts_conv3d_d_fold_supported(int CinA, int CinB, int Din, int Dout, int Hu, int Wu, int H, int W, int k);
+int ts_conv3d_d_fold_weights(const float* w_c, const float* w_s, const float* scale_c, const float* scale_s,
+                             const float* shift_c, const float* shift_s, float* w_fold, float* shift, int CinA, int CinB, int Cout, int Din, int Dout, void* stream);
+int ts_conv3d_d_fold_fwd(const float* u, const float* v, const float* w_fold, const float* shift, float* y,
+                         int B, int CinA, int CinB, int Cout, int Din, int Dout, int Hu, int Wu, int H, int W, int k,
+                         int act, long long u_bstride, long long u_cstride, long long v_bstride, long long v_cstride,
+                         long long out_bstride, long long out_cstride, void* stream);
 int ts_conv3d_hw_x6_split_supported(int Cin, int Csplit, int Cout, int W, int dilation);
 int ts_conv3d_hw_x6_split_fwd(const float* x, const float* x2, const void* w6, const float* scale, const float* shift, float* y,
                               int B, int Cin, int Csplit, int Cout, int D, int H, int W, int dilation, int act, float act_param,
diff --git a/temporalstereo_amd/_lib.py b/temporalstereo_amd/_lib.py
--- a/temporalstereo_amd/_lib.py
+++ b/temporalstereo_amd/_lib.py
@@ -29,6 +29,9 @@
                                [c_f32p, ctypes.c_longlong, c_ptr, c_size, c_ptr]),
     "ts_conv3d_d_split_supported": (c_int, [c_int] * 2),
     "ts_conv3d_d_split_fwd": (c_int, [c_f32p] * 6 + [c_int] * 13 + [c_float] + [ctypes.c_longlong] * 6 + [c_ptr]),
+    "ts_conv3d_d_fold_supported": (c_int, [c_int] * 9),
+    "ts_conv3d_d_fold_weights": (c_int, [c_f32p] * 8 + [c_int] * 5 + [c_ptr]),
+    "ts_conv3d_d_fold_fwd": (c_int, [c_f32p] * 5 + [c_int] * 12 + [ctypes.c_longlong] * 6 + [c_ptr]),
     "ts_conv3d_hw_x6_split_supported": (c_int, [c_int] * 5),
     "ts_conv3d_hw_x6_split_fwd": (c_int, [c_f32p, c_f32p, c_ptr, c_f32p, c_f32p, c_f32p] + [c_int] * 9 + [c_float] + [ctypes.c_longlong] * 6 +
                                   [c_f32p, ctypes.c_longlong, c_ptr, c_size, c_ptr]),
@@ -191,7 +194,7 @@
 }
 
 _QUERIES = frozenset(n for n in SIGNATURES if n.endswith("_bytes") or n.startswith("ts_plan_") or
-                     n.endswith("_split_supported") or
+                     n.endswith("_split_supported") or n == "ts_conv3d_d_fold_supported" or
                      n in ("ts_version", "ts_last_error_string", "ts_conv_cout_pad", "ts_conv3d_hw_x6_supported", "ts_conv3d_hw_x6s_supported", "ts_peer_max_floats", "ts_peer_max_ranks",
                            "ts_peer_alloc", "ts_peer_open", "ts_peer_close", "ts_peer_free", "ts_peer_status", "ts_peer_status_async",
                            "ts_peer_set_timeout_ms", "ts_peer_reset", "ts_bn_set_small_elems",
diff --git a/temporalstereo_amd/aggregation/native.py b/temporalstereo_amd/aggregation/native.py
--- a/temporalstereo_amd/aggregation/native.py
+++ b/temporalstereo_amd/aggregation/native.py
@@ -126,6 +126,7 @@
         self.layouts = []
         self.folds = []
         self.splits = []
+        self.derived = []
         self.eps = None
         self.unsupported = []
         self._tables = None
@@ -203,6 +204,8 @@
             else:
                 _lib.check(L.ts_conv3d_hw_x6s_weight_split(f.w.data_ptr(), f.w6s.data_ptr(), f.cin, f.cout, f.w.shape[2], mode, _stream()),
                            "ts_conv3d_hw_x6s_weight_split")
+        for step, key in self.derived:
+            step._make(key)
 
 
 _TAPE = None
@@ -580,9 +583,63 @@
         if c0.kernel_size != (1, 3, 3) or c0.padding[1] != self.dil or c1.stride[0] != self.stride:
             raise NotImplementedError("separable conv outside the (1,3,3)+(k,1,1) family: %r" % (mod,))
 
+    def hw(self, x, addend=None):
+        return conv_hw(x, self.f0, self.stride, self.dil, self.transposed, addend=addend)
+
+    def d(self, y, out=None):
+        return conv_d(y, self.f1, self.k, self.stride, self.dil, self.pad_d, self.transposed, out=out)
+
     def __call__(self, x, out=None, addend=None):
-        y = conv_hw(x, self.f0, self.stride, self.dil, self.transposed, addend=addend)
-        return conv_d(y, self.f1, self.k, self.stride, self.dil, self.pad_d, self.transposed, out=out)
+        return self.d(self.hw(x, addend=addend), out=out)
+
+
+HG_FOLD = os.environ.get("TS_HG_FOLD", "1") != "0"
+
+
+class FoldedStep:
+
+    def __init__(self, c, s):
+        self.c, self.s = c, s
+        self.made = {}
+        self._tape = _TAPE
+
+    def takes(self, u_dims, out_dims):
+        c, s = self.c, self.s
+        if c.k != s.k or s.stride != 1 or s.dil != 1 or s.pad_d != 1 or c.f1.act != ACT_NONE or s.f1.act != ACT_NONE or c.f1.cout != s.f1.cout:
+            return False
+        return bool(_lib._real_lib().ts_conv3d_d_fold_supported(c.f1.cin, s.f1.cin, u_dims[0], out_dims[0], u_dims[1], u_dims[2],
+                                                                out_dims[1], out_dims[2], c.k))
+
+    def _make(self, key):
+        c, s = self.c.f1, self.s.f1
+        w, shift = self.made[key]
+        _lib.check(_lib._real_lib().ts_conv3d_d_fold_weights(c.w.data_ptr(), s.w.data_ptr(), c.scale.data_ptr(), s.scale.data_ptr(),
+                                                             c.shift.data_ptr(), s.shift.data_ptr(), w.data_ptr(), shift.data_ptr(),
+                                                             c.cin, s.cin, c.cout, key[0], key[1], _stream()), "ts_conv3d_d_fold_weights")
+
+    def arrays(self, Din, Dout):
+        key = (Din, Dout)
+        if key not in self.made:
+            c, s = self.c.f1, self.s.f1
+            self.made[key] = (torch.empty((Dout, c.cin + s.cin, 3, c.w.shape[2]), device=c.w.device, dtype=torch.float32),
+                              torch.empty_like(c.shift))
+            self._make(key)
+            if self._tape is not None:
+                self._tape.derived.append((self, key))
+        return self.made[key]
+
+    def __call__(self, u, v):
+        B, Ca, Din, Hu, Wu = u.shape
+        _, Cb, D, H, W = v.shape
+        w, shift = self.arrays(Din, D)
+        out = torch.empty((B, self.c.f1.cout, D, H, W), device=u.device, dtype=torch.float32)
+        ub, uc = _strides5(u)
+        vb, vc = _strides5(v)
+        ob, oc = _strides5(out)
+        rc = _lib.lib().ts_conv3d_d_fold_fwd(_lib.ptr(u), _lib.ptr(v), _lib.ptr(w), _lib.ptr(shift), _lib.ptr(out), B, Ca, Cb,
+                                             self.c.f1.cout, Din, D, Hu, Wu, H, W, self.c.k, ACT_SILU, ub, uc, vb, vc, ob, oc, _stream())
+        _lib.check(rc, "ts_conv3d_d_fold_fwd")
+        return out
 
 
 class Hourglass:
@@ -592,17 +649,27 @@
         self.c5, self.c6 = SepConv(mod.conv5, True), SepConv(mod.conv6, True)
         self.s5, self.s6 = SepConv(mod.shortcut5), SepConv(mod.shortcut6)
         self.c4.f1.act = ACT_SILU
+        self.fold5, self.fold6 = FoldedStep(self.c5, self.s5), FoldedStep(self.c6, self.s6)
+
+    @staticmethod
+    def _half(n):
+        return (n - 1) // 2 + 1
 
     def __call__(self, x):
         pre = self.c2(self.c1(x))
+        dx, dp = tuple(x.shape[-3:]), tuple(pre.shape[-3:])
+        dq = tuple(self._half(n) for n in dp)
+        fold5 = HG_FOLD and self.fold5.takes((dq[0], 2 * dq[1], 2 * dq[2]), dp)
+        fold6 = HG_FOLD and self.fold6.takes((dp[0], 2 * dp[1], 2 * dp[2]), dx)
         br = Branch("hourglass")
         with br:
-            s6 = self.s6(x)
-            s5 = self.s5(pre)
-        out = self.c5(self.c4(self.c3(pre)))
+            s6 = self.s6.hw(x) if fold6 else self.s6(x)
+            s5 = self.s5.hw(pre) if fold5 else self.s5(pre)
+        out = self.c5.hw(self.c4(self.c3(pre)))
         br.join()
-        out = resize_add_act(out, s5, pre.shape[-3:])
-        return resize_add_act(self.c6(out), s6, x.shape[-3:])
+        out = self.fold5(out, s5) if fold5 else resize_add_act(self.c5.d(out), s5, dp)
+        out = self.c6.hw(out)
+        return self.fold6(out, s6) if fold6 else resize_add_act(self.c6.d(out), s6, dx)
 
 
 class Heads:
diff --git a/temporalstereo_amd/csrc/conv3d.hip b/temporalstereo_amd/csrc/conv3d.hip
--- a/temporalstereo_amd/csrc/conv3d.hip
+++ b/temporalstereo_amd/csrc/conv3d.hip
@@ -11,6 +11,20 @@
 
 
 
+
+__host__ __device__ __forceinline__ void fold_src(float sd, int od, int D, int& e0, int& e1, float& l1) {
+  const float s = sd * static_cast<float>(od);
+  e0 = static_cast<int>(s);
+  e1 = e0 + ((e0 < 2 * D - 1) ? 1 : 0);
+  l1 = s - static_cast<float>(e0);
+}
+__host__ __device__ __forceinline__ int fold_first_plane(float sd, int od, int D) {
+  int e0, e1;
+  float l1;
+  fold_src(sd, od, D, e0, e1, l1);
+  return e0 >> 1;
+}
+inline float fold_scale(int D, int Do) { return Do > 1 ? static_cast<float>(2 * D - 1) / static_cast<float>(Do - 1) : 0.f; }
 
 template <int MODE, int KT, int ST, int DL, int TP = 256>
 struct Geom {
@@ -26,12 +40,13 @@
 };
 
 
-template <int CB, int MODE, int KT, int ST, int DL, int NC, int PR = 0, int PF = 0, int TP = 256>
+template <int CB, int MODE, int KT, int ST, int DL, int NC, int PR = 0, int PF = 0, int TP = 256, int FOLD = 0>
 __global__ void __launch_bounds__(256)
 ig_conv_kernel(const float* __restrict__ x, const float* __restrict__ w, const float* __restrict__ scale,
                const float* __restrict__ shift, float* __restrict__ y, const IG p) {
   extern __shared__ __attribute__((aligned(16))) float lds[];
   static_assert(!PR || (MODE == MODE_HW && KT == 9 && ST == 1 && CB == 1 && NC >= 8), "row pairing: stride-1 (1,3,3), Cout <= 8");
+  static_assert(!FOLD || (MODE == MODE_D && KT == 3 && CB == 1), "folded decoder step: the (3,1,1) form");
   static_assert(TP == 256 || (TP == 64 && (MODE == MODE_D || MODE == MODE_HWT || (MODE == MODE_HW && !PR))), "64-pixel tiles: not the row-paired form");
   using G = Geom<MODE, KT, ST, DL, TP>;
   constexpr int WP = (CB * 16) | 16;
@@ -71,7 +86,17 @@
   const unsigned HW = static_cast<unsigned>(p.H) * p.W;
 
   int plane_id[NTR], plane_wt[NTR], ntaps = KT;
-  if (MODE == MODE_D) {
+  int plane_id2[FOLD ? NTR : 1];
+  if constexpr (FOLD) {
+    const int m = fold_first_plane(p.fold_sd, od, p.D);
+#pragma unroll
+    for (int t = 0; t < NTR; ++t) {
+      const int ia = m + t, ib = od - 1 + t;
+      plane_id[t] = (t < 2 && ia < p.D) ? ia : -1;
+      plane_id2[t] = (ib >= 0 && ib < p.Do) ? ib : -1;
+      plane_wt[t] = t;
+    }
+  } else if (MODE == MODE_D) {
     if (p.transposed) {
       ntaps = 0;
       if ((od & 1) == 0) { plane_id[0] = od >> 1; plane_wt[0] = 1; ntaps = 1; }
@@ -93,12 +118,14 @@
   const int px0 = (MODE == MODE_D) ? bx * TP : 0;
 
   unsigned goff[RQ];
+  unsigned goff2[FOLD ? RQ : 1];
   int loff[RQ];
   if (MODE == MODE_D) {
 #pragma unroll
     for (int t = 0; t < NTR; ++t) {
       const unsigned px = px0 + 4u * (threadIdx.x & 63u);
       goff[t] = (plane_id[t] >= 0 && px < HW) ? (static_cast<unsigned>(plane_id[t]) * HW + px) * 4u : kOOB;
+      if constexpr (FOLD) goff2[t] = (plane_id2[t] >= 0 && px < HW) ? (static_cast<unsigned>(plane_id2[t]) * HW + px) * 4u : kOOB;
       loff[t] = t * 256 + 4 * static_cast<int>(threadIdx.x & 63u);
     }
   } else {
@@ -115,6 +142,7 @@
   }
   constexpr int NI64 = (MODE == MODE_D && TP == 64) ? (NC * NTR + 15) / 16 : 1;
   unsigned go64[NI64];
+  unsigned go64b[FOLD ? NI64 : 1];
   int lo64[NI64], ch64[NI64];
   if constexpr (MODE == MODE_D && TP == 64) {
 #pragma unroll
@@ -122,11 +150,15 @@
       const int r = static_cast<int>(threadIdx.x >> 4) + 16 * i;
       const bool ok = r < NC * NTR;
       const int c = r / NTR, t = r - c * NTR;
-      int pid = -1;
-#pragma unroll
-      for (int u = 0; u < NTR; ++u) pid = (u == t) ? plane_id[u] : pid;
+      int pid = -1, pid2 = -1;
+#pragma unroll
+      for (int u = 0; u < NTR; ++u) {
+        pid = (u == t) ? plane_id[u] : pid;
+        if constexpr (FOLD) pid2 = (u == t) ? plane_id2[u] : pid2;
+      }
       const unsigned px = px0 + 4u * (threadIdx.x & 15u);
       go64[i] = (ok && pid >= 0 && px < HW) ? (static_cast<unsigned>(pid) * HW + px) * 4u : kOOB;
+      if constexpr (FOLD) go64b[i] = (ok && pid2 >= 0 && px < HW) ? (static_cast<unsigned>(pid2) * HW + px) * 4u : kOOB;
       ch64[i] = ok ? c : 0;
       lo64[i] = ok ? c * chan_elems + t * TP + 4 * static_cast<int>(threadIdx.x & 15u) : G::chan_raw;
     }
@@ -151,7 +183,7 @@
   }
   const __amdgpu_buffer_rsrc_t xr = ig_rsrc(x + static_cast<long long>(b) * p.in_bstride, p.in_bytes);
   const __amdgpu_buffer_rsrc_t xr2 = ig_rsrc(p.x2 + static_cast<long long>(b) * p.in2_bstride, p.in2_bytes);
-  const __amdgpu_buffer_rsrc_t wr = ig_rsrc(w, p.w_bytes);
+  const __amdgpu_buffer_rsrc_t wr = ig_rsrc(FOLD ? w + static_cast<size_t>(od) * p.Cin * KT * p.coutp : w, p.w_bytes);
   const unsigned cstride_b = static_cast<unsigned>(p.in_cstride) * 4u, cstride2_b = static_cast<unsigned>(p.in2_cstride) * 4u;
   const unsigned wstride_b = static_cast<unsigned>(KT * p.coutp) * 4u;
 
@@ -197,18 +229,25 @@
   auto fetch = [&](auto set, int c0) {
     constexpr int S = decltype(set)::value;
     const ChunkBase cbs = chunk_base(c0, p.csplit, xr, xr2, cstride_b, cstride2_b);
+    [[maybe_unused]] const bool seg_b = FOLD && c0 >= p.csplit;
     if constexpr (VD64) {
 #pragma unroll
       for (int i = 0; i < NI64; ++i) {
         const unsigned chb = static_cast<unsigned>(min(c0 + ch64[i], p.Cin - 1) - cbs.c_first) * cbs.cstride_b;
-        rin64[S][i] = __builtin_amdgcn_raw_buffer_load_b128(cbs.rsrc, go64[i] == kOOB ? kOOB : go64[i] + chb, 0, 0);
+        unsigned go = go64[i];
+        if constexpr (FOLD) go = seg_b ? go64b[i] : go;
+        rin64[S][i] = __builtin_amdgcn_raw_buffer_load_b128(cbs.rsrc, go == kOOB ? kOOB : go + chb, 0, 0);
       }
     } else if constexpr (VD) {
 #pragma unroll
       for (int ic = 0; ic < NCQ; ++ic) {
         const unsigned so = static_cast<unsigned>(min(c0 + wave_u + 4 * ic, p.Cin - 1) - cbs.c_first) * cbs.cstride_b;
 #pragma unroll
-        for (int t = 0; t < NTR; ++t) rin4[S][ic][t] = __builtin_amdgcn_raw_buffer_load_b128(cbs.rsrc, goff[t], so, 0);
+        for (int t = 0; t < NTR; ++t) {
+          unsigned go = goff[t];
+          if constexpr (FOLD) go = seg_b ? goff2[t] : go;
+          rin4[S][ic][t] = __builtin_amdgcn_raw_buffer_load_b128(cbs.rsrc, go, so, 0);
+        }
       }
     } else {
 #pragma unroll
@@ -243,6 +282,7 @@
 #pragma unroll
     for (int q = 0; q < RWN; ++q) *reinterpret_cast<u32x4*>(w_tile + wl[q]) = rw[S][q];
   };
+  [[maybe_unused]] int fold_nt = 3;
   auto mma = [&]() {
 #pragma unroll 1
   for (int c8 = 0; c8 < (NC >= 8 ? NC / 8 : 1); ++c8) {
@@ -301,7 +341,7 @@
     } else {
 #pragma unroll
       for (int t = 0; t < NTR; ++t) {
-        if (t >= ntaps) continue;
+        if (FOLD ? t >= fold_nt : t >= ntaps) continue;
         const float* wt = wt0 + (plane_wt[t] * NC) * WP;
 #pragma unroll
         for (int cq = 0; cq < 2; ++cq) {
@@ -320,6 +360,7 @@
     }
   }
   };
+  auto segment_taps = [&](int c0) { if constexpr (FOLD) fold_nt = c0 < p.csplit ? 2 : 3; };
   using S0 = std::integral_constant<int, 0>;
   using S1 = std::integral_constant<int, NSET - 1>;
   fetch(S0{}, kbeg);
@@ -330,12 +371,14 @@
       commit(S0{});
       __syncthreads();
       if (c0 + 2 * NC < kend) fetch(S0{}, c0 + 2 * NC);
+      segment_taps(c0);
       mma();
       if (c0 + NC < kend) {
         __syncthreads();
         commit(S1{});
         __syncthreads();
         if (c0 + 3 * NC < kend) fetch(S1{}, c0 + 3 * NC);
+        segment_taps(c0 + NC);
         mma();
       }
     }
@@ -345,6 +388,7 @@
       commit(S0{});
       __syncthreads();
       if (c0 + NC < kend) fetch(S0{}, c0 + NC);
+      segment_taps(c0);
       mma();
     }
   }
@@ -687,7 +731,7 @@
 const bool g_small_over_pairing = ts::env_ll("TS_CONV_SMALL_OVER_PAIRING", 1) != 0;
 const bool g_row_pairing = ts::env_not_zero("TS_CONV_ROW_PAIRING");
 
-template <int CB, int MODE, int KT, int ST, int DL, int NC, int PR = 0, int PF = 0, int TP = 256>
+template <int CB, int MODE, int KT, int ST, int DL, int NC, int PR = 0, int PF = 0, int TP = 256, int FOLD = 0>
 int launch_one(const float* x, const float* w, const float* scale, const float* shift, float* y, const IG& p,
                dim3 grid, hipStream_t st) {
   using G = Geom<MODE, KT, ST, DL, TP>;
@@ -695,7 +739,7 @@
   constexpr int KTW = PR ? 12 : KT;
   constexpr size_t lds = (static_cast<size_t>(NC) * G::chan_elems + static_cast<size_t>(KTW) * NC * WP + 4) * sizeof(float);
   static_assert(lds <= 160 * 1024, "ig_conv_kernel: tile does not fit the LDS");
-  auto kern = &ig_conv_kernel<CB, MODE, KT, ST, DL, NC, PR, PF, TP>;
+  auto kern = &ig_conv_kernel<CB, MODE, KT, ST, DL, NC, PR, PF, TP, FOLD>;
   if (lds > 64 * 1024) {
     static bool raised = false;
     if (!raised) {
@@ -851,6 +895,7 @@
   p.in_bytes = static_cast<unsigned>(in_b); p.w_bytes = static_cast<unsigned>(w_b);
   p.out_bytes = p.part_bytes = 0;
   p.x2 = nullptr; p.csplit = 0x7fffffff; p.in2_bstride = p.in2_cstride = 0; p.in2_bytes = 0;
+  p.fold_sd = 0.f;
   return true;
 }
 
@@ -1700,6 +1745,132 @@
                      act_param, in_bstride, in_cstride, out_bstride, out_cstride, 0, stream, &sp);
 }
 
+namespace {
+
+__global__ void __launch_bounds__(256)
+fold_weights_kernel(const float* __restrict__ wc, const float* __restrict__ ws, const float* __restrict__ scale_c,
+                    const float* __restrict__ scale_s, const float* __restrict__ shift_c, const float* __restrict__ shift_s,
+                    float* __restrict__ out, float* __restrict__ shift, int CinA, int CinB, int coutp, int D, int Do, float sd) {
+  if (blockIdx.x == 0 && static_cast<int>(threadIdx.x) < coutp) shift[threadIdx.x] = shift_c[threadIdx.x] + shift_s[threadIdx.x];
+  const unsigned per = static_cast<unsigned>(CinA + CinB) * 3u * static_cast<unsigned>(coutp);
+  const unsigned n = per * static_cast<unsigned>(Do);
+  for (unsigned i = blockIdx.x * blockDim.x + threadIdx.x; i < n; i += gridDim.x * blockDim.x) {
+    const int od = static_cast<int>(i / per);
+    unsigned r = i - static_cast<unsigned>(od) * per;
+    const int co = static_cast<int>(r % static_cast<unsigned>(coutp)); r /= static_cast<unsigned>(coutp);
+    const int t = static_cast<int>(r % 3u), ci = static_cast<int>(r / 3u);
+    float v;
+    if (ci >= CinA) v = ws[(static_cast<size_t>(ci - CinA) * 3 + t) * coutp + co] * scale_s[co];
+    else {
+      int e[2];
+      float l1;
+      fold_src(sd, od, D, e[0], e[1], l1);
+      const double bw[2] = {1.0 - static_cast<double>(l1), static_cast<double>(l1)};
+      const int plane = (e[0] >> 1) + t;
+      const float* wrow = wc + static_cast<size_t>(ci) * 3 * coutp + co;
+      double acc = 0.0;
+#pragma unroll
+      for (int s = 0; s < 2; ++s) {
+        if ((e[s] & 1) == 0) { if (plane == (e[s] >> 1)) acc += bw[s] * wrow[coutp]; }
+        else {
+          if (plane == ((e[s] - 1) >> 1)) acc += bw[s] * wrow[2 * coutp];
+          if (plane == ((e[s] + 1) >> 1) && plane < D) acc += bw[s] * wrow[0];
+        }
+      }
+      v = static_cast<float>(acc * static_cast<double>(scale_c[co]));
+    }
+    out[i] = v;
+  }
+}
+
+bool fold_shape_ok(int CinA, int CinB, int Din, int Dout, int Hu, int Wu, int H, int W, int k) {
+  return CinA > 0 && CinB > 0 && Din > 0 && Dout > 0 && H > 0 && W > 0 && Hu == H && Wu == W && k == 3 && Dout <= 2 * Din &&
+         CinA % 8 == 0;
+}
+
+template <int TP>
+int launch_fold_nc(long long wgs, const float* x, const float* w, const float* shift, float* y, const IG& p, dim3 grid, hipStream_t st) {
+  using G = Geom<MODE_D, 3, 1, 1, TP>;
+  constexpr size_t per_ch = (static_cast<size_t>(G::chan_elems) + 3 * 16) * sizeof(float);
+  constexpr size_t lds_cu = 160 * 1024;
+  const size_t per_cu = static_cast<size_t>((wgs + ts::kNumCU - 1) / ts::kNumCU);
+  const int max_nc = g_chunk_cap;
+  auto fits = [&](int nc) { return nc <= max_nc && (nc * per_ch + 16) * per_cu <= lds_cu && p.kspan >= nc && p.csplit % nc == 0; };
+  if (fits(32)) return launch_one<1, MODE_D, 3, 1, 1, 32, 0, 0, TP, 1>(x, w, nullptr, shift, y, p, grid, st);
+  if (fits(16)) return launch_one<1, MODE_D, 3, 1, 1, 16, 0, 0, TP, 1>(x, w, nullptr, shift, y, p, grid, st);
+  if (wgs < g_pf_max_wgs && p.kspan > 8) return launch_one<1, MODE_D, 3, 1, 1, 8, 0, 1, TP, 1>(x, w, nullptr, shift, y, p, grid, st);
+  return launch_one<1, MODE_D, 3, 1, 1, 8, 0, 0, TP, 1>(x, w, nullptr, shift, y, p, grid, st);
+}
+
+}
+
+extern "C" int ts_conv3d_d_fold_supported(int CinA, int CinB, int Din, int Dout, int Hu, int Wu, int H, int W, int k) {
+  return fold_shape_ok(CinA, CinB, Din, Dout, Hu, Wu, H, W, k) ? 1 : 0;
+}
+
+extern "C" int ts_conv3d_d_fold_weights(const float* w_c, const float* w_s, const float* scale_c, const float* scale_s,
+                                        const float* shift_c, const float* shift_s, float* w_fold, float* shift,
+                                        int CinA, int CinB, int Cout, int Din, int Dout, void* stream) {
+  TS_REQUIRE(CinA > 0 && CinB > 0 && Cout > 0 && Din > 0 && Dout > 0, TS_ERR_SHAPE, "conv3d_d_fold_weights: non-positive size");
+  TS_REQUIRE(Dout <= 2 * Din, TS_ERR_UNSUPPORTED, "conv3d_d_fold_weights: Dout=%d > 2 Din=%d", Dout, 2 * Din);
+  TS_REQUIRE_PTR(w_c); TS_REQUIRE_PTR(w_s); TS_REQUIRE_PTR(scale_c); TS_REQUIRE_PTR(scale_s); TS_REQUIRE_PTR(shift_c); TS_REQUIRE_PTR(shift_s);
+  TS_REQUIRE_PTR(w_fold); TS_REQUIRE_PTR(shift);
+  const int bucket = cout_bucket(Cout);
+  TS_REQUIRE(bucket > 0 && bucket <= 256, TS_ERR_UNSUPPORTED, "conv3d_d_fold_weights: Cout=%d", Cout);
+  const unsigned long long n = static_cast<unsigned long long>(Dout) * (CinA + CinB) * 3ull * bucket;
+  TS_REQUIRE(n < 0x7fffffffull / 4, TS_ERR_UNSUPPORTED, "conv3d_d_fold_weights: array of 2 GiB or more");
+  const unsigned blocks = (n + 255) / 256 < 1024 ? static_cast<unsigned>((n + 255) / 256) : 1024u;
+  hipLaunchKernelGGL(fold_weights_kernel, dim3(blocks), dim3(256), 0, ts::as_stream(stream), w_c, w_s, scale_c, scale_s, shift_c, shift_s, w_fold, shift,
+                     CinA, CinB, bucket, Din, Dout, fold_scale(Din, Dout));
+  return ts::launched("fold_weights_kernel");
+}
+
+extern "C" int ts_conv3d_d_fold_fwd(const float* u, const float* v, const float* w_fold, const float* shift, float* y,
+                                    int B, int CinA, int CinB, int Cout, int Din, int Dout, int Hu, int Wu, int H, int W, int k,
+                                    int act, long long u_bstride, long long u_cstride, long long v_bstride, long long v_cstride,
+                                    long long out_bstride, long long out_cstride, void* stream) {
+  TS_REQUIRE(B > 0 && CinA > 0 && CinB > 0 && Cout > 0 && Din > 0 && Dout > 0 && Hu > 0 && Wu > 0 && H > 0 && W > 0, TS_ERR_SHAPE,
+             "conv3d_d_fold: non-positive size");
+  TS_REQUIRE(fold_shape_ok(CinA, CinB, Din, Dout, Hu, Wu, H, W, k), TS_ERR_UNSUPPORTED,
+             "conv3d_d_fold: needs the same H, W on both inputs (%dx%d, %dx%d), k=%d == 3, Dout=%d <= 2 Din=%d, CinA=%d %% 8 == 0", Hu, Wu,
+             H, W, k, Dout, 2 * Din, CinA);
+  TS_REQUIRE(act >= 0 && act <= 2, TS_ERR_SHAPE, "conv3d_d_fold: unknown activation");
+  TS_REQUIRE(Dout <= 65535, TS_ERR_SHAPE, "conv3d_d_fold: bad output depth");
+  TS_REQUIRE_PTR(u); TS_REQUIRE_PTR(v); TS_REQUIRE_PTR(w_fold); TS_REQUIRE_PTR(shift); TS_REQUIRE_PTR(y);
+  const int Cin = CinA + CinB;
+  IG p;
+  p.Cin = Cin; p.Cout = Cout; p.coutp = cout_bucket(Cout); p.D = Din; p.H = H; p.W = W; p.Do = Dout; p.Ho = H; p.Wo = W;
+  p.stride = 1; p.dil = 1; p.pad = 1; p.k = 3; p.transposed = 0;
+  p.act = act; p.act_param = 0.f;
+  p.in_bstride = u_bstride; p.in_cstride = u_cstride; p.out_bstride = out_bstride; p.out_cstride = out_cstride;
+  p.tiles_x = 1; p.ksplit = 1; p.kspan = Cin; p.partial = nullptr; p.B = B;
+  p.addend = nullptr; p.add_bstride = 0; p.add_cstride = 0; p.add_dstride = 0;
+  const unsigned long long hw = static_cast<unsigned long long>(H) * W;
+  const unsigned long long bu = (static_cast<unsigned long long>(CinA - 1) * u_cstride + Din * hw) * 4ull;
+  const unsigned long long bv = (static_cast<unsigned long long>(CinB - 1) * v_cstride + Dout * hw) * 4ull;
+  const unsigned long long bo = (static_cast<unsigned long long>(Cout - 1) * out_cstride + Dout * hw) * 4ull;
+  const unsigned long long bw = static_cast<unsigned long long>(Cin) * 3ull * p.coutp * 4ull;
+  TS_REQUIRE(u_cstride >= 0 && v_cstride >= 0 && out_cstride >= 0 && bu < 0x7fffffffull && bv < 0x7fffffffull && bo < 0x7fffffffull &&
+                 bw * Dout < 0x7fffffffull, TS_ERR_UNSUPPORTED, "conv3d_d_fold: a batch element spans 2 GiB or more");
+  p.in_bytes = static_cast<unsigned>(bu); p.in2_bytes = static_cast<unsigned>(bv); p.out_bytes = static_cast<unsigned>(bo);
+  p.part_bytes = 0; p.w_bytes = static_cast<unsigned>(bw);
+  p.x2 = v; p.csplit = CinA; p.in2_bstride = v_bstride; p.in2_cstride = v_cstride;
+  p.fold_sd = fold_scale(Din, Dout);
+  p.co_groups = (Cout + 15) / 16;
+  static const int xcd = ts::env_not_zero("TS_CONV_XCD") ? 1 : 0;
+  p.xcd = xcd;
+  hipStream_t st = ts::as_stream(stream);
+  static const long long small = ts::env_ll("TS_CONV_D_SMALL_WGS", 256);
+  const int tiles = static_cast<int>((hw + 255) / 256);
+  const long long wgs = static_cast<long long>(tiles) * Dout * B * p.co_groups;
+  if (wgs <= small) {
+    const dim3 grid64(static_cast<unsigned>((hw + 63) / 64), Dout, B * p.co_groups);
+    return launch_fold_nc<64>(4 * wgs, u, w_fold, shift, y, p, grid64, st);
+  }
+  const dim3 grid(tiles, Dout, B * p.co_groups);
+  return launch_fold_nc<256>(wgs, u, w_fold, shift, y, p, grid, st);
+}
+
 extern "C" int ts_conv3d_d_bwd_data(const float* dy, const float* w_b, float* dx, int B, int Cin, int Cout, int Din, int H,
                                     int W, int k, int stride, int dilation, int padding, int transposed,
                                     long long dy_bstride, long long dy_cstride, long long dx_bstride, long long dx_cstride,
diff --git a/temporalstereo_amd/csrc/conv_common.hpp b/temporalstereo_amd/csrc/conv_common.hpp
--- a/temporalstereo_amd/csrc/conv_common.hpp
+++ b/temporalstereo_amd/csrc/conv_common.hpp
@@ -54,6 +54,7 @@
   int csplit;
   long long in2_bstride, in2_cstride;
   unsigned in2_bytes;
+  float fold_sd;
 };
 
 struct ChunkBase {
diff --git a/temporalstereo_amd/csrc/plan.hip b/temporalstereo_amd/csrc/plan.hip
--- a/temporalstereo_amd/csrc/plan.hip
+++ b/temporalstereo_amd/csrc/plan.hip
@@ -98,6 +98,7 @@
     TS_PLAN_OP(ts_spp3d_pool_fwd),          TS_PLAN_OP(ts_spp3d_pool_bwd),
     TS_PLAN_OP(ts_spp3d_expand_fwd),        TS_PLAN_OP(ts_spp3d_expand_bwd),        TS_PLAN_OP(ts_depth_sum3_fwd),
     TS_PLAN_OP(ts_bn_small_train_bwd),
+    TS_PLAN_OP(ts_conv3d_d_fold_fwd),       TS_PLAN_OP(ts_conv3d_d_fold_weights),
 };
 
 struct Call {
diff --git a/temporalstereo_amd/csrc/ts_common.hpp b/temporalstereo_amd/csrc/ts_common.hpp
--- a/temporalstereo_amd/csrc/ts_common.hpp
+++ b/temporalstereo_amd/csrc/ts_common.hpp
@@ -9,7 +9,7 @@
 
 #include "../../include/ts_hip.h"
 
-#define TS_ABI_VERSION 18
+#define TS_ABI_VERSION 19
 
 namespace ts {
 
```

New measurement: 1624 (median of 5 runs). No clear change (+0.3%).
